# tabahi/WebSpeechAnalyzer

Measured on AMD Instinct MI355X. Metric: 53-feat frames/sec, higher is better.
Workload: dtype f32 front end / f64 tracker; 1 GPU; 1024 clips x 10 s @16 kHz mono per GPU, 1024-pt FFT, 25 ms hop, Segment Features (level 5); parallelism=1 GPU, batches_in_flight=6, streams=3

## Files before the change

webspeechanalyzer_amd/csrc/api.hip:

```cpp
#include <algorithm>
#include <cmath>
#include <cstdio>
#include <cstdlib>
#include <cstring>
#include <string>
#include <vector>
#include <map>
#include <mutex>
#include <system_error>
#include <thread>
#include "host_plan.hpp"

using namespace wsa;

thread_local std::string wsa_api::g_create_error;
using wsa_api::fail;

struct wsa_batch {
    wsa_ctx* ctx = nullptr;
    uint32_t n_clips = 0;
    double fs = 0;
    std::vector<uint32_t> n_samples, n_frames, frame_off;
    uint32_t total_frames = 0, max_frames = 0, max_samples = 0;
    DevArena mem;
    FeDev fe;
    Derived D;
    BackEnd be;
    int n_waves = 0;
    uint32_t *d_n_frames = nullptr, *d_frame_off = nullptr, *d_spec = nullptr;
    uint2* d_order = nullptr;
    uint2* d_redo = nullptr;
    char* d_pool = nullptr; double* d_span_hdr = nullptr; bool split = false; size_t pool_bpf = 0;
    hipStream_t up_stream[8] = {}; hipEvent_t up_event[8] = {}, up_start = nullptr; bool up_ready = false;
    int16_t* d_i16 = nullptr; uint64_t i16_cap = 0; uint64_t* d_i16_off = nullptr; uint32_t *d_i16_ch = nullptr, *d_i16_ns = nullptr;
    std::vector<uint64_t> h_i16_off; std::vector<uint32_t> h_i16_ch;
    bool pair = false;
    bool published = false;
    Tuning tune;
    uint32_t* d_span_hist = nullptr; uint2* d_span_key = nullptr;
    float* d_pcm_own = nullptr;
    bool rs_on = false; double fs_in = 0; std::vector<uint32_t> n_samples_in; uint32_t max_samples_in = 0;
    uint32_t *d_rs_n_in = nullptr, *d_rs_n_out = nullptr; float *d_rs_table = nullptr, *d_rs_pcm = nullptr; uint64_t rs_stride = 0;
    bool rs_mixed = false; RsMixedPlan rs_plan; RsClass* d_rs_cls = nullptr; uint32_t* d_rs_clip_class = nullptr; RsWork* d_rs_work = nullptr;
    bool counters_clean = false, end_clears = false, capturing = false, ever_captured = false;
    TrackGather trk;
    std::vector<int32_t> h_trk_seg; std::vector<uint32_t> h_seg_count;
    uint32_t res_utt = 0;
    double* d_trace = nullptr;
    uint32_t* h_totals = nullptr;
    uint32_t* h_totals_dev = nullptr;
    hipEvent_t ev[5] = {nullptr, nullptr, nullptr, nullptr, nullptr};
    bool timing = true, ran = false, full_table = false;
    uint32_t reruns = 0;
    uint32_t res_rows = 0, res_segs = 0, res_flags = 0;
    const uint32_t* spec_in_use = nullptr;
    wsa_cls* cls = nullptr;
    wsa_ecls* ecls = nullptr;
    int cls_last = 0;
};

namespace wsa {
Tuning Tuning::from_env() {
    Tuning t;
    { const char* on = std::getenv("WSA_TUNING_ENV"); if (!on || on[0] != '1') return t; }
    auto num = [](const char* name, int dflt) { const char* e = std::getenv(name); return e && *e ? std::atoi(e) : dflt; };
    t.dbg = num("WSA_DBG", 0);
    t.no_pair = std::getenv("WSA_NO_PAIR") != nullptr; t.no_split = std::getenv("WSA_NO_SPLIT") != nullptr; t.no_quad = std::getenv("WSA_NO_QUAD") != nullptr; t.quad = std::getenv("WSA_QUAD") != nullptr; t.no_fuse = std::getenv("WSA_NO_FUSE") != nullptr;
    t.fe_fat = std::getenv("WSA_FE_FAT") != nullptr; t.peaks_lanes = std::getenv("WSA_PEAKS_LANES") != nullptr;
    t.full_table = num("WSA_FULL_TABLE", -1);
    t.tracker_wpc = num("WSA_TRACKER_WPC", 0); t.fin_wpc = num("WSA_FIN_WPC", 0); t.fpw = num("WSA_FPW", 0);
    t.fe_wg_per_cu = num("WSA_FE_WGS", 0); t.fe_no_queue = std::getenv("WSA_FE_NO_QUEUE") != nullptr; t.peaks_wpc = num("WSA_PEAKS_WPC", 0); t.peaks_w = num("WSA_PEAKS_W", 0); t.upload_threads = num("WSA_UPLOAD_THREADS", 0);
    t.rs_s = num("WSA_RS_S", 0); t.rs_j = num("WSA_RS_J", 0); t.rs_c = num("WSA_RS_C", 0); t.rs_one_launch = std::getenv("WSA_RS_ONE_LAUNCH") != nullptr;
    return t;
}
__global__ void pcm_i16_to_f32_kernel(const int16_t* in, const uint64_t* off, const uint32_t* ch, const uint32_t* ns, float* out, uint64_t stride) {
    const uint32_t c = blockIdx.y;
    const uint32_t n = ns[c], k = ch[c];
    const int16_t* src = in + off[c];
    float* dst = out + (uint64_t)c * stride;
    for (uint32_t i = blockIdx.x * blockDim.x + threadIdx.x; i < n; i += gridDim.x * blockDim.x) dst[i] = (float)src[(uint64_t)i * k] * (1.0f / 32768.0f);
}
__global__ void batch_publish_kernel(const uint32_t* totals, const uint32_t* counters, uint32_t* host) {
    if (threadIdx.x == 0) {
        host[0] = totals[0]; host[1] = totals[1]; host[2] = counters[1]; host[3] = totals[3];
        __threadfence_system();
    }
}
__global__ void batch_clear_kernel(uint32_t* counters, uint32_t* totals, uint32_t* span_hist) {
    if (threadIdx.x < 16) counters[threadIdx.x] = 0;
    if (threadIdx.x < 4) totals[threadIdx.x] = 0;
    if (span_hist) for (int b = threadIdx.x; b < SPAN_BUCKETS; b += blockDim.x) span_hist[b] = 0;
}
}

extern "C" {

int wsa_abi_version(void) { return WSA_ABI_VERSION; }

void wsa_config_default(wsa_config* c) {
    c->spec_type = 1; c->output_level = 4; c->f_min = 50; c->f_max = 4000; c->N_fft_bins = 256; c->N_mel_bins = 128;
    c->window_width = 25; c->window_step = 25; c->pause_length = 200; c->min_seg_length = 50; c->auto_noise_gate = 1;
    c->voiced_max_dB = 100; c->voiced_min_dB = 10; c->pre_norm_gain = 1000; c->high_f_emph = 0;
}

const char* wsa_last_error(const wsa_ctx* ctx) { return ctx ? ctx->err.c_str() : wsa_api::g_create_error.c_str(); }

wsa_status wsa_create(const wsa_config* cfg, int32_t device, wsa_ctx** out) {
    if (!cfg || !out) return fail(nullptr, WSA_ERR_INVALID, "null argument");
    *out = nullptr;
    int n = 0;
    if (hipGetDeviceCount(&n) != hipSuccess || n <= 0) return fail(nullptr, WSA_ERR_NO_DEVICE, "no HIP device visible (libwsa has no CPU path)");
    if (device < 0 || device >= n) return fail(nullptr, WSA_ERR_INVALID, "device ordinal out of range");
    hipDeviceProp_t prop;
    if (hipGetDeviceProperties(&prop, device) != hipSuccess) return fail(nullptr, WSA_ERR_NO_DEVICE, "hipGetDeviceProperties failed");
    if (std::strncmp(prop.gcnArchName, "gfx950", 6) != 0)
        return fail(nullptr, WSA_ERR_NO_DEVICE, std::string("libwsa is built for gfx950 only; device is ") + prop.gcnArchName);
    const int lv = cfg->output_level;
    if (!(lv == 1 || lv == 2 || lv == 3 || lv == 4 || lv == 5 || lv == 10 || lv == 11 || lv == 12 || lv == 13))
        return fail(nullptr, WSA_ERR_INVALID, "output_level must be 1, 2 (spectrum frames only), 3, 4, 5, 10, 11, 12 or 13");
    if (!(cfg->window_step > 0) || !(cfg->window_width > 0)) return fail(nullptr, WSA_ERR_INVALID, "window_width / window_step must be positive");
    wsa_ctx* c = new wsa_ctx();
    c->cfg = *cfg; c->device = device; c->n_cu = prop.multiProcessorCount;
    *out = c;
    return WSA_OK;
}

void wsa_destroy(wsa_ctx* ctx) { delete ctx; }

wsa_status wsa_geometry_for(const wsa_ctx* ctx, double fs, wsa_geometry* out) {
    if (!ctx || !out) return WSA_ERR_INVALID;
    FePlanHost p; std::string err;
    if (!build_fe_plan(ctx->cfg, fs, p, err)) return fail(const_cast<wsa_ctx*>(ctx), WSA_ERR_INVALID, err);
    out->nfft = p.nfft; out->win = p.win; out->hop = p.hop; out->bands = p.bands; out->kmax = p.kmax;
    return WSA_OK;
}

wsa_status wsa_bins_hz(const wsa_ctx* ctx, double fs, double* out, int32_t n) {
    if (!ctx || !out) return WSA_ERR_INVALID;
    FePlanHost p; std::string err;
    if (!build_fe_plan(ctx->cfg, fs, p, err)) return fail(const_cast<wsa_ctx*>(ctx), WSA_ERR_INVALID, err);
    if (n < p.bands) return fail(const_cast<wsa_ctx*>(ctx), WSA_ERR_INVALID, "bins_hz buffer too small");
    for (int i = 0; i < p.bands; i++) out[i] = p.bins_hz[i];
    return WSA_OK;
}

void wsa_batch_destroy(wsa_batch* b) {
    if (!b) return;
    (void)hipSetDevice(b->ctx->device);
    if (b->d_i16) (void)hipFree(b->d_i16);
    for (auto& st : b->up_stream) if (st) (void)hipStreamDestroy(st);
    for (auto& e : b->up_event) if (e) (void)hipEventDestroy(e);
    if (b->up_start) (void)hipEventDestroy(b->up_start);
    for (auto& e : b->ev) if (e) (void)hipEventDestroy(e);
    wsa_cls_free(b->cls);
    wsa_ecls_free(b->ecls);
    delete b;
}

static wsa_status batch_create_impl(wsa_ctx* ctx, uint32_t n_clips, const uint32_t* n_samples, double fs, const uint32_t* n_samples_in, double fs_in, wsa_batch** out, const double* fs_in_each = nullptr) {
    if (!ctx || !out || (n_clips && !n_samples)) return fail(ctx, WSA_ERR_INVALID, "null argument");
    *out = nullptr;
    HIP_TRY(ctx, hipSetDevice(ctx->device));
    wsa_batch* b = new wsa_batch();
    b->ctx = ctx; b->n_clips = n_clips; b->fs = fs;
    b->tune = Tuning::from_env();
    std::string err;
    const FeDev::Refusal refused = b->fe.build(ctx->cfg, fs, b->tune.fe_fat, err);
    if (refused == FeDev::BAD_FFT) err = "unsupported FFT length: NFFT = the smallest of {2^k, 3 * 2^k} >= max(window, fs * N_fft_bins / f_max) must lie in 256 .. 8192 or be 3 * 2^k up to 12288";
    if (refused == FeDev::LDS) err += ": shorten the window or lower f_max / N_fft_bins";
    if (refused != FeDev::OK) { delete b; return fail(ctx, WSA_ERR_INVALID, err); }
    const FePlanHost& P = b->fe.plan;
    b->n_samples.assign(n_samples, n_samples + n_clips);
    b->n_frames.resize(n_clips); b->frame_off.resize(n_clips + 1);
    uint64_t tot = 0;
    for (uint32_t i = 0; i < n_clips; i++) {
        const uint32_t ns = n_samples[i];
        const uint32_t nf = ns < (uint32_t)P.win ? 0u : (ns - (uint32_t)P.win) / (uint32_t)P.hop + 1u;
        b->n_frames[i] = nf; b->frame_off[i] = (uint32_t)tot; tot += nf;
        if (nf > b->max_frames) b->max_frames = nf;
        if (ns > b->max_samples) b->max_samples = ns;
    }
    if (tot * CAND_CAP > 0xfffffff0ull) { delete b; return fail(ctx, WSA_ERR_INVALID, "batch has too many frames"); }
    b->frame_off[n_clips] = (uint32_t)tot; b->total_frames = (uint32_t)tot;

    const Derived& D = b->D = Derived(ctx->cfg, P.bands);
    BackEnd& B = b->be;
    B.n = n_clips;
    B.set_caps(D, P.bands, b->max_frames);
    B.seg_cap = (int)b->max_frames / D.period + 2;
    B.row_cap = D.syllable_rows ? (int)b->max_frames / 2 + 2 : B.seg_cap;
    b->pair = !D.raw_tracks && P.bands <= 128 && !b->tune.no_pair;
    b->pool_bpf = tracker_pool_bpf();
    b->split = b->pair && !b->tune.no_split && (size_t)b->total_frames * b->pool_bpf <= ((size_t)48 << 30);
    const size_t budget = (size_t)(b->pair ? 16 : 8) << 30;
    size_t waves = budget / ((b->be.ws_stride ? b->be.ws_stride : 1) * (b->pair ? 2 : 1));
    size_t wpc = 16;
    if (b->tune.tracker_wpc >= 1 && b->tune.tracker_wpc <= 32) wpc = (size_t)b->tune.tracker_wpc;
    const size_t want = (size_t)ctx->n_cu * wpc;
    if (waves > want) waves = want;
    if (waves > (size_t)n_clips * (size_t)b->be.seg_cap) waves = (size_t)n_clips * (size_t)b->be.seg_cap;
    if (b->pair && waves > ((size_t)n_clips * (size_t)b->be.seg_cap + 1) / 2 && n_clips * (size_t)b->be.seg_cap > 256) waves = ((size_t)n_clips * (size_t)b->be.seg_cap + 1) / 2;
    if (waves < 1) waves = 1;
    b->n_waves = (int)waves;

    DevArena& A = b->mem;
    const size_t spans = (size_t)n_clips * B.seg_cap;
    bool ok = b->fe.upload(A) && A.upload(&b->d_n_frames, b->n_frames) && A.upload(&b->d_frame_off, b->frame_off) && A.alloc(&b->d_spec, (size_t)b->total_frames * P.bands);
    if (ok && D.level > 2 && b->split) {
        size_t free_b = 0, total_b = 0;
        const size_t pool_bytes = (size_t)b->total_frames * b->pool_bpf;
        const bool room = hipMemGetInfo(&free_b, &total_b) != hipSuccess || free_b > pool_bytes + ((size_t)2 << 30);
        if (!(room && A.alloc(&b->d_pool, pool_bytes) && A.alloc(&b->d_span_hdr, spans * 8))) {
            (void)hipGetLastError();
            b->split = false; b->d_pool = nullptr; b->d_span_hdr = nullptr;
        }
    }
    ok = ok && B.alloc(A, D, b->total_frames, false) && A.alloc(&B.d_counters, 16);
    if (D.level > 2)
        ok = ok && A.alloc(&B.d_ws, B.ws_stride * (size_t)b->n_waves * (b->pair && !b->split ? 2 : 1)) && A.alloc(&b->d_redo, spans) && A.alloc(&b->d_order, spans)
                && A.alloc(&b->d_span_hist, (size_t)SPAN_BUCKETS) && A.alloc(&b->d_span_key, spans)
                && (!D.raw_tracks || (A.alloc(&B.d_trk_pts, ((size_t)b->total_frames + 1) * 64 * 2) && A.alloc(&B.d_trk_rank, ((size_t)b->total_frames + 1) * 64)))
                && (D.level != 12 || A.alloc(&B.d_coef_ws, (size_t)b->total_frames * 8));
    ok = ok && A.pin(&b->h_totals, &b->h_totals_dev, 8);
    for (auto& e : b->ev) if (ok) ok = hipEventCreate(&e) == hipSuccess;
    if (b->tune.full_table >= 0) b->full_table = b->tune.full_table != 0;
    if (ok && n_samples_in) {
        b->rs_on = true; b->fs_in = fs_in; b->n_samples_in.assign(n_samples_in, n_samples_in + n_clips);
        for (uint32_t i = 0; i < n_clips; i++) if (n_samples_in[i] > b->max_samples_in) b->max_samples_in = n_samples_in[i];
        b->rs_stride = ((uint64_t)b->max_samples + 3u) & ~3ull;
        ok = A.upload(&b->d_rs_n_in, b->n_samples_in) && A.upload(&b->d_rs_n_out, b->n_samples) && b->mem.alloc(&b->d_rs_pcm, (size_t)n_clips * b->rs_stride + 4);
        if (ok && fs_in_each) {
            b->rs_mixed = true;
            if (!plan_resample_mixed(n_clips, b->n_samples.data(), fs_in_each, fs, b->rs_plan, err)) { wsa_batch_destroy(b); return fail(ctx, WSA_ERR_INVALID, err); }
            RsMixedPlan& M = b->rs_plan;
            ok = A.upload(&b->d_rs_table, M.tables) && A.upload(&b->d_rs_cls, M.cls) && A.upload(&b->d_rs_clip_class, M.clip_class) && A.upload(&b->d_rs_work, M.work);
            std::vector<float>().swap(M.tables); std::vector<RsWork>().swap(M.work);
        } else if (ok) {
            std::vector<float> K0, K; build_resample_table(fs_in, fs, K0); resample_table_image(K0, K);
            ok = A.upload(&b->d_rs_table, K);
        }
    }
    if (!ok) {
        const std::string m = std::string("device allocation failed: ") + hipGetErrorString(hipGetLastError());
        wsa_batch_destroy(b);
        return fail(ctx, WSA_ERR_HIP, m);
    }
    *out = b;
    return WSA_OK;
}

wsa_status wsa_batch_create(wsa_ctx* ctx, uint32_t n_clips, const uint32_t* n_samples, double fs, wsa_batch** out) {
    return batch_create_impl(ctx, n_clips, n_samples, fs, nullptr, 0, out);
}

uint64_t wsa_resample_length(uint64_t n_in, double fs_in, double fs_out) { return fs_in > 0 && fs_out > 0 ? resample_length(n_in, fs_in, fs_out) : 0; }

wsa_status wsa_batch_create_resampled(wsa_ctx* ctx, uint32_t n_clips, const uint32_t* n_samples_in, double fs_in, double fs_out, wsa_batch** out) {
    if (!ctx || !out || (n_clips && !n_samples_in)) return fail(ctx, WSA_ERR_INVALID, "null argument");
    if (const wsa_status st = check_rates(ctx, &fs_in, 1, fs_out, nullptr); st != WSA_OK) return st;
    std::vector<uint32_t> n_out(n_clips);
    for (uint32_t i = 0; i < n_clips; i++) {
        const uint64_t n = resample_length(n_samples_in[i], fs_in, fs_out);
        if (n > 0xfffffff0ull) return fail(ctx, WSA_ERR_INVALID, "a converted clip would exceed 2^32 samples");
        n_out[i] = (uint32_t)n;
    }
    return batch_create_impl(ctx, n_clips, n_out.data(), fs_out, n_samples_in, fs_in, out);
}

wsa_status wsa_batch_create_mixed(wsa_ctx* ctx, uint32_t n_clips, const uint32_t* n_samples_in, const double* fs_in, double fs_out, wsa_batch** out) {
    if (!ctx || !out || (n_clips && (!n_samples_in || !fs_in))) return fail(ctx, WSA_ERR_INVALID, n_clips && ctx && out && !fs_in ? "null argument: fs_in holds one rate per clip (clip 0 has none)" : "null argument");
    if (const wsa_status st = check_rates(ctx, fs_in, n_clips, fs_out, "clip"); st != WSA_OK) return st;
    std::vector<uint32_t> n_out(n_clips);
    for (uint32_t i = 0; i < n_clips; i++) {
        const uint64_t n = resample_length(n_samples_in[i], fs_in[i], fs_out);
        if (n > 0xfffffff0ull) return fail(ctx, WSA_ERR_INVALID, "a converted clip would exceed 2^32 samples (clip " + std::to_string(i) + ")");
        n_out[i] = (uint32_t)n;
    }
    return batch_create_impl(ctx, n_clips, n_out.data(), fs_out, n_samples_in, 0, out, fs_in);
}

wsa_status wsa_batch_get_info(const wsa_batch* b, wsa_batch_info* o) {
    if (!b || !o) return WSA_ERR_INVALID;
    o->n_clips = b->n_clips; o->n_frames_total = b->total_frames; o->max_frames_per_clip = b->max_frames; o->bands = (uint32_t)b->fe.plan.bands;
    o->rows_cap = b->n_clips * (uint32_t)b->be.row_cap; o->segments_cap = b->n_clips * (uint32_t)b->be.seg_cap; o->workspace_bytes = b->mem.dev_bytes;
    return WSA_OK;
}

static wsa_status run_backend_stages(wsa_batch* b, const uint32_t* d_spec, bool skip_peaks, hipStream_t s) {
    wsa_ctx* ctx = b->ctx;
    const Derived& D = b->D;
    const BackEnd& B = b->be;
    b->published = false;
    if (D.level <= 2) return WSA_OK;
    const int dbg = b->tune.dbg;
    {
        hipStream_t cs = s;
        uint32_t* counters = B.d_counters + 4;
        PkParams pk; pk.spec = d_spec; pk.rec = B.rec; pk.total_frames = b->total_frames; pk.bands = b->fe.plan.bands;
        pk.flags = B.d_counters + 1; pk.dbg = (b->tune.dbg >> 20) & 0xff; pk.lanes_only = b->tune.peaks_lanes ? 1 : 0;
        pk.wpc = b->tune.peaks_wpc; pk.round_bins = b->tune.peaks_w;
        if (!skip_peaks) launch_peaks(pk, cs);
        GateParams g;
        B.fill(g, D);
        g.n_frames = b->d_n_frames; g.frame_off = b->d_frame_off; g.trace = b->d_trace; g.dbg = dbg; g.prio = 1;
        const bool ordered = !(dbg & 8192);
        g.span_hist = ordered ? b->d_span_hist : nullptr; g.span_key = b->d_span_key;
        launch_gate(g, cs);
        TrParams t;
        B.fill(t, D);
        t.frame_off = b->d_frame_off; t.trace = b->d_trace; t.dbg = dbg;
        t.order = ordered ? b->d_order : nullptr; t.redo = b->d_redo; t.redo_count = counters + 2;
        t.fin_waves = b->tune.fin_wpc >= 1 && b->tune.fin_wpc <= 32 ? ctx->n_cu * b->tune.fin_wpc : 0;
        t.quad = b->split && !b->tune.no_quad && (b->tune.quad || b->total_frames >= 1200000u) ? 1 : 0;
        t.quad_waves = (int)std::min<size_t>((size_t)b->n_waves, ((size_t)b->n_clips * (size_t)B.seg_cap + 3) / 4 + 1);
        t.pool = b->split ? b->d_pool : nullptr; t.pool_bpf = (uint32_t)b->pool_bpf; t.span_hdr = b->split ? b->d_span_hdr : nullptr;
        if (t.order) launch_span_order(t, b->d_span_hist, b->d_span_key, b->d_order, counters, cs);
        if (b->timing) HIP_TRY(ctx, hipEventRecord(b->ev[2], s));
        launch_tracker(t, b->n_waves, b->full_table, b->pair, cs);
    }
    if (b->timing) HIP_TRY(ctx, hipEventRecord(b->ev[3], s));
    CompactParams cp;
    B.fill(cp, D);
    cp.clip_rows = B.d_clip_rows; cp.flags = B.d_counters + 1; cp.fused = b->tune.no_fuse ? 0 : 1;
    cp.host = D.tail_kernel ? nullptr : b->h_totals_dev;
    b->published = compact_is_fused(cp) && cp.host != nullptr;
    const bool self_clear = b->published && !b->capturing;
    cp.clr_counters = self_clear ? B.d_counters : nullptr; cp.clr_hist = self_clear ? b->d_span_hist : nullptr;
    b->end_clears = self_clear;
    launch_compact(cp, s);
    if (D.level == 11) {
        UttParams u;
        B.fill(u, b->d_frame_off);
        launch_utterance(u, s);
    }
    if (D.level == 12) {
        CoefParams q;
        B.fill(q, b->d_frame_off);
        q.total_frames = b->total_frames;
        launch_coeffs(q, b->n_clips * (uint32_t)B.row_cap, s);
    }
    HIP_TRY(ctx, hipGetLastError());
    return WSA_OK;
}

static wsa_status run_impl(wsa_batch* b, const float* d_pcm, uint64_t stride, const uint32_t* d_spec_in, bool fe, bool be, hipStream_t s) {
    wsa_ctx* ctx = b->ctx;
    HIP_TRY(ctx, hipSetDevice(ctx->device));
    {
        hipStreamCaptureStatus cap = hipStreamCaptureStatusNone;
        if (s && hipStreamIsCapturing(s, &cap) != hipSuccess) { (void)hipGetLastError(); cap = hipStreamCaptureStatusNone; }
        b->capturing = cap != hipStreamCaptureStatusNone;
        if (b->capturing) b->ever_captured = true;
    }
    if (!b->counters_clean || b->ever_captured) hipLaunchKernelGGL(batch_clear_kernel, dim3(1), dim3(256), 0, s, b->be.d_counters, b->be.d_totals, b->d_span_hist);
    b->counters_clean = false; b->end_clears = false;
    if (b->timing) HIP_TRY(ctx, hipEventRecord(b->ev[0], s));
    const uint32_t* spec = d_spec_in ? d_spec_in : b->d_spec;
    if (fe) {
        if (!d_pcm && b->total_frames) return fail(ctx, WSA_ERR_INVALID, "null PCM pointer");
        if (stride < (b->rs_on ? b->max_samples_in : b->max_samples) && b->n_clips > 1) return fail(ctx, WSA_ERR_INVALID, "clip_stride smaller than the longest clip");
        if (b->rs_mixed) {
            RsMixedParams r; r.in = d_pcm; r.stride_in = stride; r.out = b->d_rs_pcm; r.stride_out = b->rs_stride; r.n_in = b->d_rs_n_in; r.n_out = b->d_rs_n_out;
            r.tables = b->d_rs_table; r.cls = b->d_rs_cls; r.clip_class = b->d_rs_clip_class; r.work = b->d_rs_work;
            launch_resample_mixed(r, b->rs_plan, !b->tune.rs_one_launch, s);
            HIP_TRY(ctx, hipGetLastError());
            d_pcm = b->d_rs_pcm; stride = b->rs_stride;
        } else if (b->rs_on) {
            RsParams r; r.in = d_pcm; r.stride_in = stride; r.out = b->d_rs_pcm; r.stride_out = b->rs_stride;
            r.n_in = b->d_rs_n_in; r.n_out = b->d_rs_n_out; r.table = b->d_rs_table; r.ratio = b->fs_in / b->fs; r.S = b->tune.rs_s > 0 ? b->tune.rs_s : resample_stride(b->fs_in, b->fs);
            r.J = b->tune.rs_j > 0 ? b->tune.rs_j : resample_outputs_per_lane(r.S, r.ratio); r.span = resample_span(r.ratio, r.S, r.J); r.chunks = b->tune.rs_c > 0 ? b->tune.rs_c : 1;
            launch_resample(r, b->n_clips, b->max_samples, s);
            HIP_TRY(ctx, hipGetLastError());
            d_pcm = b->d_rs_pcm; stride = b->rs_stride;
        }
        FeParams p;
        b->fe.fill(p, b->tune.fe_fat);
        p.pcm = d_pcm; p.clip_stride = stride; p.n_frames = b->d_n_frames; p.frame_off = b->d_frame_off; p.spec = b->d_spec;
        p.frames_per_wave = b->tune.fpw > 0 ? b->tune.fpw : 25; p.wg_per_cu = b->tune.fe_wg_per_cu;
        p.queue = b->tune.fe_no_queue ? nullptr : b->be.d_counters + 8; p.n_cu = b->ctx->n_cu;
        launch_frontend(p, (int)b->n_clips, (int)b->max_frames, b->fe.plan.R, b->fe.plan.three, s);
        HIP_TRY(ctx, hipGetLastError());
    }
    if (b->timing) HIP_TRY(ctx, hipEventRecord(b->ev[1], s));
    if (be) {
        const wsa_status st = run_backend_stages(b, spec, false, s);
        if (st != WSA_OK) return st;
    } else if (b->timing) { HIP_TRY(ctx, hipEventRecord(b->ev[2], s)); HIP_TRY(ctx, hipEventRecord(b->ev[3], s)); }
    if (!(be && b->published)) hipLaunchKernelGGL(batch_publish_kernel, dim3(1), dim3(64), 0, s, b->be.d_totals, b->be.d_counters, b->h_totals_dev);
    if (b->timing) HIP_TRY(ctx, hipEventRecord(b->ev[4], s));
    b->ran = true; b->spec_in_use = spec;
    b->counters_clean = be && b->end_clears && !b->capturing;
    return WSA_OK;
}

int wsa_debug_batch_counters(wsa_batch* b, uint32_t* out16) {
    if (!b || !out16) return WSA_ERR_INVALID;
    return hipMemcpy(out16, b->be.d_counters, 16 * sizeof(uint32_t), hipMemcpyDeviceToHost) == hipSuccess ? WSA_OK : WSA_ERR_HIP;
}

wsa_status wsa_batch_run(wsa_batch* b, const float* d_pcm, uint64_t clip_stride, void* stream) {
    if (!b) return WSA_ERR_INVALID;
    return run_impl(b, d_pcm, clip_stride, nullptr, true, true, reinterpret_cast<hipStream_t>(stream));
}
wsa_status wsa_batch_run_frontend(wsa_batch* b, const float* d_pcm, uint64_t clip_stride, void* stream) {
    if (!b) return WSA_ERR_INVALID;
    return run_impl(b, d_pcm, clip_stride, nullptr, true, false, reinterpret_cast<hipStream_t>(stream));
}
wsa_status wsa_batch_run_backend(wsa_batch* b, const uint32_t* d_spectra, void* stream) {
    if (!b || !d_spectra) return WSA_ERR_INVALID;
    return run_impl(b, nullptr, 0, d_spectra, false, true, reinterpret_cast<hipStream_t>(stream));
}

}
static std::mutex g_slab_mu;
static std::map<uintptr_t, size_t> g_slabs;
static bool slab_of(const void* p, uintptr_t* base, size_t* size) {
    std::lock_guard<std::mutex> lk(g_slab_mu);
    auto it = g_slabs.upper_bound(reinterpret_cast<uintptr_t>(p));
    if (it == g_slabs.begin()) return false;
    --it;
    if (reinterpret_cast<uintptr_t>(p) >= it->first + it->second) return false;
    *base = it->first; *size = it->second;
    return true;
}
template <typename DST, typename SRC, typename LEN>
static wsa_status upload_clips(wsa_batch* b, uint32_t n, DST dst, SRC src, LEN bytes, hipStream_t s) {
    wsa_ctx* ctx = b->ctx;
    uint64_t total = 0;
    for (uint32_t i = 0; i < n; i++) total += bytes(i);
    constexpr int UP_MAX = 8;
    int UP_THREADS = 3;
    if (b->tune.upload_threads >= 1 && b->tune.upload_threads <= UP_MAX) UP_THREADS = b->tune.upload_threads;
    {
        bool pinned = n > 0;
        std::vector<uintptr_t> slab_end(n, 0);
        for (uint32_t i = 0; i < n && pinned; i++) {
            if (!bytes(i)) continue;
            uintptr_t base = 0; size_t size = 0;
            if (slab_of(src(i), &base, &size)) { slab_end[i] = base + size; continue; }
            hipPointerAttribute_t at;
            if (hipPointerGetAttributes(&at, src(i)) != hipSuccess) { (void)hipGetLastError(); pinned = false; }
            else pinned = at.type == hipMemoryTypeHost;
        }
        if (pinned) {
            uint32_t i = 0;
            while (i < n) {
                const char* s0 = reinterpret_cast<const char*>(src(i)); char* d0 = reinterpret_cast<char*>(dst(i));
                size_t len = bytes(i); uint32_t j = i + 1;
                while (slab_end[i] && j < n && reinterpret_cast<const char*>(src(j)) == s0 + len && reinterpret_cast<char*>(dst(j)) == d0 + len
                       && reinterpret_cast<uintptr_t>(s0) + len + bytes(j) <= slab_end[i]) { len += bytes(j); j++; }
                if (len) HIP_TRY(ctx, hipMemcpyAsync(d0, s0, len, hipMemcpyHostToDevice, s));
                i = j;
            }
            return WSA_OK;
        }
    }
    if (n < 16 || total < ((uint64_t)32 << 20) || UP_THREADS == 1) {
        for (uint32_t i = 0; i < n; i++) if (bytes(i)) HIP_TRY(ctx, hipMemcpyAsync(dst(i), src(i), bytes(i), hipMemcpyHostToDevice, s));
        return WSA_OK;
    }
    if (!b->up_ready) {
        for (int t = 0; t < UP_MAX; t++) { HIP_TRY(ctx, hipStreamCreateWithFlags(&b->up_stream[t], hipStreamNonBlocking)); HIP_TRY(ctx, hipEventCreateWithFlags(&b->up_event[t], hipEventDisableTiming)); }
        HIP_TRY(ctx, hipEventCreateWithFlags(&b->up_start, hipEventDisableTiming));
        b->up_ready = true;
    }
    HIP_TRY(ctx, hipEventRecord(b->up_start, s));
    hipError_t err[UP_MAX];
    std::thread th[UP_MAX];
    uint32_t first_[UP_MAX + 1]; first_[0] = 0;
    { uint64_t acc = 0; int t = 1; for (uint32_t i = 0; i < n && t < UP_THREADS; i++) { acc += bytes(i); if (acc >= total * t / UP_THREADS) first_[t++] = i + 1; } while (t <= UP_THREADS) first_[t++] = n; }
    first_[UP_THREADS] = n;
    int started = 0;
    for (int t = 0; t < UP_THREADS; t++) {
        err[t] = hipSuccess;
        try {
        th[t] = std::thread([&, t]() {
            hipError_t e = hipSetDevice(ctx->device);
            if (e == hipSuccess) e = hipStreamWaitEvent(b->up_stream[t], b->up_start, 0);
            for (uint32_t i = first_[t]; i < first_[t + 1] && e == hipSuccess; i++) if (bytes(i)) e = hipMemcpyAsync(dst(i), src(i), bytes(i), hipMemcpyHostToDevice, b->up_stream[t]);
            if (e == hipSuccess) e = hipEventRecord(b->up_event[t], b->up_stream[t]);
            err[t] = e;
        });
        } catch (const std::system_error&) { break; }
        started++;
    }
    for (int t = 0; t < started; t++) th[t].join();
    hipError_t first = hipSuccess;
    for (int t = started; t < UP_THREADS && first == hipSuccess; t++)
        for (uint32_t i = first_[t]; i < first_[t + 1] && first == hipSuccess; i++) if (bytes(i)) first = hipMemcpyAsync(dst(i), src(i), bytes(i), hipMemcpyHostToDevice, s);
    for (int t = 0; t < started; t++) {
        if (err[t] != hipSuccess) { if (first == hipSuccess) first = err[t]; (void)hipStreamSynchronize(b->up_stream[t]); }
        else { const hipError_t e = hipStreamWaitEvent(s, b->up_event[t], 0); if (e != hipSuccess && first == hipSuccess) first = e; }
    }
    HIP_TRY(ctx, first);
    return WSA_OK;
}

extern "C" {
wsa_status wsa_batch_run_host(wsa_batch* b, const float* const* pcm, void* stream) {
    if (!b || (!pcm && b->n_clips)) return WSA_ERR_INVALID;
    wsa_ctx* ctx = b->ctx;
    hipStream_t s = reinterpret_cast<hipStream_t>(stream);
    HIP_TRY(ctx, hipSetDevice(ctx->device));
    const std::vector<uint32_t>& ns_host = b->rs_on ? b->n_samples_in : b->n_samples;
    const uint64_t stride = ((b->rs_on ? b->max_samples_in : b->max_samples) + 3u) & ~3ull;
    if (!b->d_pcm_own && !b->mem.alloc(&b->d_pcm_own, (size_t)b->n_clips * stride)) return fail(ctx, WSA_ERR_HIP, "PCM staging allocation failed");
    {
        const wsa_status st = upload_clips(b, b->n_clips, [&](uint32_t i) { return b->d_pcm_own + (size_t)i * stride; }, [&](uint32_t i) { return pcm[i]; },
                                           [&](uint32_t i) { return (size_t)ns_host[i] * sizeof(float); }, s);
        if (st != WSA_OK) return st;
    }
    return run_impl(b, b->d_pcm_own, stride, nullptr, true, true, s);
}

wsa_status wsa_batch_run_host_i16(wsa_batch* b, const int16_t* const* pcm, const uint32_t* channels, void* stream) {
    if (!b || (!pcm && b->n_clips)) return WSA_ERR_INVALID;
    wsa_ctx* ctx = b->ctx;
    hipStream_t s = reinterpret_cast<hipStream_t>(stream);
    HIP_TRY(ctx, hipSetDevice(ctx->device));
    const std::vector<uint32_t>& ns_host = b->rs_on ? b->n_samples_in : b->n_samples;
    const uint64_t stride = ((b->rs_on ? b->max_samples_in : b->max_samples) + 3u) & ~3ull;
    if (!b->d_pcm_own && !b->mem.alloc(&b->d_pcm_own, (size_t)b->n_clips * stride)) return fail(ctx, WSA_ERR_HIP, "PCM staging allocation failed");
    std::vector<uint64_t> off(b->n_clips + 1, 0); std::vector<uint32_t> ch(b->n_clips ? b->n_clips : 1, 1u);
    for (uint32_t i = 0; i < b->n_clips; i++) {
        ch[i] = channels ? channels[i] : 1u;
        if (ch[i] < 1 || ch[i] > 64) return fail(ctx, WSA_ERR_INVALID, "channels must be 1 .. 64");
        off[i + 1] = off[i] + (((uint64_t)ns_host[i] * ch[i] + 3u) & ~3ull);
    }
    if (off[b->n_clips] > b->i16_cap) {
        if (b->d_i16) { (void)hipFree(b->d_i16); b->d_i16 = nullptr; b->i16_cap = 0; }
        HIP_TRY(ctx, hipMalloc(reinterpret_cast<void**>(&b->d_i16), (size_t)off[b->n_clips] * sizeof(int16_t) + 16));
        b->i16_cap = off[b->n_clips];
    }
    if (!b->d_i16_off) {
        if (!b->mem.alloc(&b->d_i16_off, (size_t)b->n_clips + 1) || !b->mem.alloc(&b->d_i16_ch, (size_t)b->n_clips + 1) || !b->mem.alloc(&b->d_i16_ns, (size_t)b->n_clips + 1))
            return fail(ctx, WSA_ERR_HIP, "int16 staging allocation failed");
    }
    b->h_i16_off = off; b->h_i16_ch = ch;
    HIP_TRY(ctx, hipMemcpyAsync(b->d_i16_off, b->h_i16_off.data(), ((size_t)b->n_clips + 1) * sizeof(uint64_t), hipMemcpyHostToDevice, s));
    HIP_TRY(ctx, hipMemcpyAsync(b->d_i16_ch, b->h_i16_ch.data(), (size_t)(b->n_clips ? b->n_clips : 1) * sizeof(uint32_t), hipMemcpyHostToDevice, s));
    HIP_TRY(ctx, hipMemcpyAsync(b->d_i16_ns, ns_host.data(), (size_t)b->n_clips * sizeof(uint32_t), hipMemcpyHostToDevice, s));
    {
        const wsa_status st = upload_clips(b, b->n_clips, [&](uint32_t i) { return b->d_i16 + off[i]; }, [&](uint32_t i) { return pcm[i]; },
                                           [&](uint32_t i) { return (size_t)ns_host[i] * ch[i] * sizeof(int16_t); }, s);
        if (st != WSA_OK) return st;
    }
    if (b->n_clips) {
        const uint32_t mx = b->rs_on ? b->max_samples_in : b->max_samples;
        hipLaunchKernelGGL(pcm_i16_to_f32_kernel, dim3((mx + 1023) / 1024 ? (mx + 1023) / 1024 : 1, b->n_clips), dim3(256), 0, s, b->d_i16, b->d_i16_off, b->d_i16_ch, b->d_i16_ns, b->d_pcm_own, stride);
        HIP_TRY(ctx, hipGetLastError());
    }
    return run_impl(b, b->d_pcm_own, stride, nullptr, true, true, s);
}

static wsa_status fetch_totals(wsa_batch* b, hipStream_t s) {
    wsa_ctx* ctx = b->ctx;
    if (!b->ran) return fail(ctx, WSA_ERR_INVALID, "no run on this batch yet");
    {
        HIP_TRY(ctx, hipSetDevice(ctx->device));
        HIP_TRY(ctx, hipStreamSynchronize(s));
        const volatile uint32_t* ht = b->h_totals;
        b->res_rows = ht[0]; b->res_segs = ht[1]; b->res_flags = ht[2]; b->res_utt = ht[3];
        if (b->res_flags & 2u) {
            b->full_table = true; b->reruns++;
            hipLaunchKernelGGL(batch_clear_kernel, dim3(1), dim3(256), 0, s, b->be.d_counters, b->be.d_totals, b->d_span_hist);
            const bool tm = b->timing; b->timing = false;
            const wsa_status st = run_backend_stages(b, b->spec_in_use, true, s);
            b->timing = tm;
            if (st != WSA_OK) return st;
            if (!b->published) hipLaunchKernelGGL(batch_publish_kernel, dim3(1), dim3(64), 0, s, b->be.d_totals, b->be.d_counters, b->h_totals_dev);
            HIP_TRY(ctx, hipStreamSynchronize(s));
            b->res_rows = ht[0]; b->res_segs = ht[1]; b->res_flags = ht[2]; b->res_utt = ht[3];
        }
    }
    if (b->res_flags & 1u) return fail(ctx, WSA_ERR_CAPACITY, "a device-side arena overflowed; results are invalid");
    return WSA_OK;
}

wsa_status wsa_host_alloc(wsa_ctx* ctx, uint64_t bytes, void** out) {
    if (!ctx || !out) return WSA_ERR_INVALID;
    *out = nullptr;
    HIP_TRY(ctx, hipSetDevice(ctx->device));
    HIP_TRY(ctx, hipHostMalloc(out, bytes ? (size_t)bytes : 1, hipHostMallocPortable));
    { std::lock_guard<std::mutex> lk(g_slab_mu); g_slabs[reinterpret_cast<uintptr_t>(*out)] = bytes ? (size_t)bytes : 1; }
    return WSA_OK;
}
void wsa_host_free(void* p) {
    if (!p) return;
    { std::lock_guard<std::mutex> lk(g_slab_mu); g_slabs.erase(reinterpret_cast<uintptr_t>(p)); }
    (void)hipHostFree(p);
}

wsa_status wsa_queue_create(wsa_ctx* ctx, void** stream) {
    if (!ctx || !stream) return WSA_ERR_INVALID;
    *stream = nullptr;
    HIP_TRY(ctx, hipSetDevice(ctx->device));
    hipStream_t s = nullptr;
    HIP_TRY(ctx, hipStreamCreateWithFlags(&s, hipStreamNonBlocking));
    *stream = s;
    return WSA_OK;
}
wsa_status wsa_queue_synchronize(wsa_ctx* ctx, void* stream) {
    if (!ctx) return WSA_ERR_INVALID;
    HIP_TRY(ctx, hipSetDevice(ctx->device));
    HIP_TRY(ctx, hipStreamSynchronize(reinterpret_cast<hipStream_t>(stream)));
    return WSA_OK;
}
void wsa_queue_destroy(wsa_ctx* ctx, void* stream) {
    if (!stream) return;
    if (ctx) (void)hipSetDevice(ctx->device);
    (void)hipStreamDestroy(reinterpret_cast<hipStream_t>(stream));
}

void wsa_batch_view_internal(wsa_batch* b, wsa_batch_view* v) {
    v->ctx = b->ctx; v->level = b->ctx->cfg.output_level; v->n_clips = b->n_clips; v->rows_cap = b->n_clips * (uint32_t)b->be.row_cap;
    v->d_meta = b->be.d_meta; v->d_feat = b->be.d_feat; v->d_row_off = b->be.d_row_off; v->reruns = b->reruns; v->cls = &b->cls; v->ecls = &b->ecls; v->cls_last = &b->cls_last;
}
wsa_status wsa_batch_fetch_internal(wsa_batch* b, hipStream_t s) { return fetch_totals(b, s); }

wsa_ctx* wsa_batch_ctx_internal(const wsa_batch* b) { return b ? b->ctx : nullptr; }

wsa_status wsa_batch_result(wsa_batch* b, void* stream, wsa_device_result* o) {
    if (!b || !o) return WSA_ERR_INVALID;
    const wsa_status st = fetch_totals(b, reinterpret_cast<hipStream_t>(stream));
    o->n_clips = b->n_clips; o->n_rows = b->res_rows; o->n_segments = b->res_segs; o->n_frames_total = b->total_frames;
    o->status_flags = b->res_flags;
    o->d_row_meta = b->be.d_meta; o->d_row_feat = b->be.d_feat; o->d_segments = b->be.d_seg; o->d_clip_row_off = b->be.d_row_off; o->d_clip_seg_off = b->be.d_seg_off;
    o->d_spectra = b->spec_in_use; o->d_clip_frame_off = b->d_frame_off; o->d_formants = b->be.d_formants;
    o->n_utterance_rows = b->be.d_utt_feat ? b->res_utt : 0; o->d_utt_meta = b->be.d_utt_meta; o->d_utt_feat = b->be.d_utt_feat; o->d_clip_utt_off = b->be.d_utt_off;
    return st;
}

wsa_status wsa_batch_copy_rows(wsa_batch* b, void* stream, int32_t* row_meta, double* row_feat, uint32_t rows_cap,
                               int32_t* segments, uint32_t seg_cap, uint32_t* clip_row_off, uint32_t* clip_seg_off) {
    if (!b) return WSA_ERR_INVALID;
    wsa_ctx* ctx = b->ctx;
    hipStream_t s = reinterpret_cast<hipStream_t>(stream);
    const wsa_status st = fetch_totals(b, s);
    if (st != WSA_OK) return st;
    if ((row_meta || row_feat) && rows_cap < b->res_rows) return fail(ctx, WSA_ERR_INVALID, "row buffer too small");
    if (segments && seg_cap < b->res_segs) return fail(ctx, WSA_ERR_INVALID, "segment buffer too small");
    if (row_meta && b->res_rows) HIP_TRY(ctx, hipMemcpyAsync(row_meta, b->be.d_meta, (size_t)b->res_rows * 8 * sizeof(int32_t), hipMemcpyDefault, s));
    if (row_feat && b->res_rows) HIP_TRY(ctx, hipMemcpyAsync(row_feat, b->be.d_feat, (size_t)b->res_rows * WSA_NFEAT * sizeof(double), hipMemcpyDefault, s));
    if (segments && b->res_segs) HIP_TRY(ctx, hipMemcpyAsync(segments, b->be.d_seg, (size_t)b->res_segs * 4 * sizeof(int32_t), hipMemcpyDefault, s));
    if (clip_row_off) HIP_TRY(ctx, hipMemcpyAsync(clip_row_off, b->be.d_row_off, ((size_t)b->n_clips + 1) * sizeof(uint32_t), hipMemcpyDefault, s));
    if (clip_seg_off) HIP_TRY(ctx, hipMemcpyAsync(clip_seg_off, b->be.d_seg_off, ((size_t)b->n_clips + 1) * sizeof(uint32_t), hipMemcpyDefault, s));
    HIP_TRY(ctx, hipStreamSynchronize(s));
    return WSA_OK;
}

wsa_status wsa_batch_copy_spectra(wsa_batch* b, void* stream, uint32_t* spectra, uint64_t cap_words, uint32_t* clip_frame_off) {
    if (!b) return WSA_ERR_INVALID;
    wsa_ctx* ctx = b->ctx;
    hipStream_t s = reinterpret_cast<hipStream_t>(stream);
    if (!b->ran) return fail(ctx, WSA_ERR_INVALID, "no run on this batch yet");
    if (spectra && !b->spec_in_use) return fail(ctx, WSA_ERR_INVALID, "the u32 frames of this run were not stored: call wsa_batch_keep_spectra(batch, 1) before the run");
    const uint64_t words = (uint64_t)b->total_frames * (uint32_t)b->fe.plan.bands;
    if (spectra && cap_words < words) return fail(ctx, WSA_ERR_INVALID, "spectra buffer too small");
    HIP_TRY(ctx, hipSetDevice(ctx->device));
    if (spectra && words) HIP_TRY(ctx, hipMemcpyAsync(spectra, b->spec_in_use, words * sizeof(uint32_t), hipMemcpyDefault, s));
    if (clip_frame_off) std::memcpy(clip_frame_off, b->frame_off.data(), ((size_t)b->n_clips + 1) * sizeof(uint32_t));
    HIP_TRY(ctx, hipStreamSynchronize(s));
    return WSA_OK;
}

wsa_status wsa_batch_copy_utterance(wsa_batch* b, void* stream, int32_t* utt_meta, double* utt_feat, uint32_t cap_rows, uint32_t* clip_utt_off) {
    if (!b) return WSA_ERR_INVALID;
    wsa_ctx* ctx = b->ctx;
    hipStream_t s = reinterpret_cast<hipStream_t>(stream);
    if (!b->be.d_utt_feat) return fail(ctx, WSA_ERR_INVALID, "no utterance features: output_level must be 11");
    const wsa_status st = fetch_totals(b, s);
    if (st != WSA_OK) return st;
    if ((utt_meta || utt_feat) && cap_rows < b->res_utt) return fail(ctx, WSA_ERR_INVALID, "utterance buffer too small");
    if (utt_meta && b->res_utt) HIP_TRY(ctx, hipMemcpyAsync(utt_meta, b->be.d_utt_meta, (size_t)b->res_utt * 4 * sizeof(int32_t), hipMemcpyDefault, s));
    if (utt_feat && b->res_utt) HIP_TRY(ctx, hipMemcpyAsync(utt_feat, b->be.d_utt_feat, (size_t)b->res_utt * WSA_NUTT * sizeof(double), hipMemcpyDefault, s));
    if (clip_utt_off) HIP_TRY(ctx, hipMemcpyAsync(clip_utt_off, b->be.d_utt_off, ((size_t)b->n_clips + 1) * sizeof(uint32_t), hipMemcpyDefault, s));
    HIP_TRY(ctx, hipStreamSynchronize(s));
    return WSA_OK;
}

wsa_status wsa_batch_copy_formants(wsa_batch* b, void* stream, float* formants, uint64_t cap_frames) {
    if (!b || !formants) return WSA_ERR_INVALID;
    wsa_ctx* ctx = b->ctx;
    hipStream_t s = reinterpret_cast<hipStream_t>(stream);
    if (!b->ran || !b->be.d_formants) return fail(ctx, WSA_ERR_INVALID, "no formant frames: output_level must be 4, 10, 11 or 12 and the batch must have run");
    if (cap_frames < b->total_frames) return fail(ctx, WSA_ERR_INVALID, "formant buffer too small");
    HIP_TRY(ctx, hipSetDevice(ctx->device));
    if (b->total_frames) HIP_TRY(ctx, hipMemcpyAsync(formants, b->be.d_formants, (size_t)b->total_frames * 9 * sizeof(float), hipMemcpyDefault, s));
    HIP_TRY(ctx, hipStreamSynchronize(s));
    return WSA_OK;
}


static wsa_status fetch_track_tables(wsa_batch* b, hipStream_t s) {
    wsa_ctx* ctx = b->ctx;
    if (!b->be.d_trk_seg) return fail(ctx, WSA_ERR_INVALID, "no raw tracks: output_level must be 3");
    const wsa_status st = fetch_totals(b, s);
    if (st != WSA_OK) return st;
    b->h_trk_seg.resize((size_t)b->n_clips * b->be.seg_cap * 4); b->h_seg_count.resize(b->n_clips);
    if (b->n_clips) {
        HIP_TRY(ctx, hipMemcpyAsync(b->h_trk_seg.data(), b->be.d_trk_seg, b->h_trk_seg.size() * sizeof(int32_t), hipMemcpyDefault, s));
        HIP_TRY(ctx, hipMemcpyAsync(b->h_seg_count.data(), b->be.d_seg_count, b->h_seg_count.size() * sizeof(uint32_t), hipMemcpyDefault, s));
        HIP_TRY(ctx, hipStreamSynchronize(s));
    }
    return WSA_OK;
}

static void batch_track_list(wsa_batch* b) {
    b->trk.begin();
    for (uint32_t c = 0; c < b->n_clips; c++)
        for (uint32_t k = 0; k < b->h_seg_count[c]; k++) b->trk.add(&b->h_trk_seg[((size_t)c * b->be.seg_cap + k) * 4], 0);
}

wsa_status wsa_batch_tracks_info(wsa_batch* b, void* stream, wsa_tracks_info* out) {
    if (!b || !out) return WSA_ERR_INVALID;
    const wsa_status st = fetch_track_tables(b, reinterpret_cast<hipStream_t>(stream));
    if (st != WSA_OK) return st;
    batch_track_list(b);
    out->n_segments = b->trk.segments(); out->n_points = b->trk.n_points; out->n_ranked = b->trk.n_ranked;
    return WSA_OK;
}

wsa_status wsa_batch_copy_tracks(wsa_batch* b, void* stream, uint64_t* seg_off, int32_t* points, uint64_t cap_points, int32_t* ranked, uint64_t cap_ranked) {
    if (!b || !seg_off || !points || !ranked) return WSA_ERR_INVALID;
    wsa_ctx* ctx = b->ctx;
    hipStream_t s = reinterpret_cast<hipStream_t>(stream);
    const wsa_status st = fetch_track_tables(b, s);
    if (st != WSA_OK) return st;
    TrackGather& G = b->trk;
    batch_track_list(b);
    if (G.n_points > cap_points || G.n_ranked > cap_ranked) return fail(ctx, WSA_ERR_INVALID, "track buffers too small");
    G.offsets(seg_off);
    if (const wsa_status gs = G.run(ctx, 1ull << 63, b->be.d_trk_pts, b->be.d_trk_rank, points, ranked, s); gs != WSA_OK) return gs;
    HIP_TRY(ctx, hipStreamSynchronize(s));
    return WSA_OK;
}

wsa_status wsa_batch_copy_pcm(wsa_batch* b, void* stream, float* pcm, uint64_t stride) {
    if (!b || !pcm) return WSA_ERR_INVALID;
    wsa_ctx* ctx = b->ctx;
    hipStream_t s = reinterpret_cast<hipStream_t>(stream);
    if (!b->rs_on || !b->ran) return fail(ctx, WSA_ERR_INVALID, "no converted PCM: the batch must come from wsa_batch_create_resampled / wsa_batch_create_mixed and must have run");
    if (stride < b->max_samples) return fail(ctx, WSA_ERR_INVALID, "stride smaller than the longest converted clip");
    HIP_TRY(ctx, hipSetDevice(ctx->device));
    for (uint32_t i = 0; i < b->n_clips; i++)
        if (b->n_samples[i]) HIP_TRY(ctx, hipMemcpyAsync(pcm + (size_t)i * stride, b->d_rs_pcm + (size_t)i * b->rs_stride, (size_t)b->n_samples[i] * sizeof(float), hipMemcpyDefault, s));
    HIP_TRY(ctx, hipStreamSynchronize(s));
    return WSA_OK;
}

wsa_status wsa_batch_stage_ms(wsa_batch* b, float out[4]) {
    if (!b || !out) return WSA_ERR_INVALID;
    wsa_ctx* ctx = b->ctx;
    if (!b->ran || !b->timing) return fail(ctx, WSA_ERR_INVALID, "no timed run on this batch");
    HIP_TRY(ctx, hipEventSynchronize(b->ev[4]));
    for (int i = 0; i < 4; i++) HIP_TRY(ctx, hipEventElapsedTime(&out[i], b->ev[i], b->ev[i + 1]));
    return WSA_OK;
}

wsa_status wsa_batch_enable_trace(wsa_batch* b, int32_t on) {
    if (!b) return WSA_ERR_INVALID;
    if (on && !b->d_trace) {
        HIP_TRY(b->ctx, hipSetDevice(b->ctx->device));
        const size_t rows = b->total_frames ? b->total_frames : 1;
        if (!b->mem.alloc(&b->d_trace, rows * 12)) return fail(b->ctx, WSA_ERR_HIP, "trace allocation failed");
        HIP_TRY(b->ctx, hipMemset(b->d_trace, 0, rows * 12 * sizeof(double)));
    }
    if (!on) b->d_trace = nullptr;
    return WSA_OK;
}

wsa_status wsa_batch_copy_trace(wsa_batch* b, void* stream, double* out, uint64_t cap_rows) {
    if (!b || !out) return WSA_ERR_INVALID;
    wsa_ctx* ctx = b->ctx;
    hipStream_t s = reinterpret_cast<hipStream_t>(stream);
    if (!b->d_trace || !b->ran) return fail(ctx, WSA_ERR_INVALID, "trace not enabled or no run yet");
    if (cap_rows < b->total_frames) return fail(ctx, WSA_ERR_INVALID, "trace buffer too small");
    if (b->total_frames) HIP_TRY(ctx, hipMemcpyAsync(out, b->d_trace, (size_t)b->total_frames * 12 * sizeof(double), hipMemcpyDefault, s));
    HIP_TRY(ctx, hipStreamSynchronize(s));
    return WSA_OK;
}

wsa_status wsa_batch_keep_spectra(wsa_batch* b, int32_t on) {
    if (!b) return WSA_ERR_INVALID;
    (void)on;
    return WSA_OK;
}

wsa_status wsa_batch_backend_reruns(const wsa_batch* b, uint32_t* out) {
    if (!b || !out) return WSA_ERR_INVALID;
    *out = b->reruns;
    return WSA_OK;
}

wsa_status wsa_batch_enable_timing(wsa_batch* b, int32_t on) {
    if (!b) return WSA_ERR_INVALID;
    b->timing = on != 0;
    return WSA_OK;
}

}
```

webspeechanalyzer_amd/csrc/gate.hip:

```cpp
#include "wsa_internal.hpp"
#include "wave_ops.hpp"
#include "jsmath_device.hpp"
#include "gate_floor.hpp"

#pragma clang diagnostic ignored "-Winline-asm"

namespace wsa {


template <bool ST>
__global__ __launch_bounds__(64) void gate_kernel_t(GateParams p) {
    const int lane = threadIdx.x;
    for (uint32_t clip = p.clip0 + blockIdx.x; clip < p.clip0 + p.n_clips; clip += gridDim.x) {
        const uint32_t nfr = p.n_frames[clip];
        const uint32_t foff = ST ? clip * p.ring : p.frame_off[clip];
        const uint32_t fmask = ST ? p.ring - 1 : 0xffffffffu;
        int32_t* seg_i = p.seg_i + (uint64_t)clip * p.seg_cap * 8;
        double* seg_d = p.seg_d + (uint64_t)clip * p.seg_cap * 2;

        int cur_frame = 0, no_fm = 0, c_ci = 0, c_started = -1;
        double ctx_max = p.ctx_max0, floor_ = p.floor0, last_max = p.ctx_max0, last_floor = p.floor0;
        double gw = 0, gT = 0, gk = 0;
        int nseg = 0, span_begin = 0, cuts = 0;
        bool overflow = false;
        double* st = ST ? p.state + (uint64_t)clip * GATE_STATE : nullptr;
        if (ST) {
            cur_frame = (int)st[0]; no_fm = (int)st[1]; c_ci = (int)st[2]; c_started = (int)st[3];
            ctx_max = st[4]; floor_ = st[5]; last_max = st[6]; last_floor = st[7]; gw = st[8]; gT = st[9]; gk = st[10];
            span_begin = (int)st[11]; cuts = (int)st[12];
        }
        const uint32_t fbase = (uint32_t)cur_frame;

        auto finalize = [&](int e_arg, int f_end) __attribute__((always_inline)) {
            const int len = e_arg - no_fm;
            if (!((double)len > p.min_frames && c_started >= 2)) return;
            if (nseg >= p.seg_cap) { overflow = true; return; }
            if (lane == 0) {
                int32_t* sg = seg_i + 8 * nseg;
                sg[SEG_START] = cur_frame - len; sg[SEG_LEN] = len; sg[SEG_FBEGIN] = span_begin; sg[SEG_FEND] = f_end;
                sg[SEG_CCI] = c_ci; sg[SEG_FLAG] = p.level == 3 ? 1 : 0; sg[SEG_NROWS] = 0; sg[SEG_ROW0] = 0;
                seg_d[2 * nseg] = ctx_max; seg_d[2 * nseg + 1] = floor_;
                if (!ST && p.span_hist) {
                    const uint32_t bkt = (uint32_t)(SPAN_BUCKETS - 1) - min((uint32_t)(f_end - span_begin), (uint32_t)(SPAN_BUCKETS - 1));
                    p.span_key[(uint64_t)clip * p.seg_cap + nseg] = make_uint2(bkt, atomicAdd(&p.span_hist[bkt], 1u));
                }
            }
            nseg++;
        };
        bool gate_reset = false;
        auto noise_gate = [&](double h) __attribute__((always_inline)) {
            gw++;
            if (h > ctx_max || (gw > 40 && h > 2 * floor_)) {
                if (h >= ctx_max) { gw = 0; last_max = ctx_max = h; }
                else if (h > last_max / 100) { ctx_max -= trunc(ctx_max / 8); gw = 35; }
                const double y = ctx_max, t = jsm::log10(y);
                double v;
                if (t > 7) v = trunc(jsm::pow_pos(10, t - 3) / 20);
                else if (t > 6) v = trunc(jsm::pow_pos(10, t - 3) / 2);
                else if (t > 4) v = trunc(jsm::pow_pos(10, t - 2) / 2);
                else if (t > 2) v = trunc(jsm::pow_pos(10, t / 3));
                else if (t > 1) v = trunc(y / 10);
                else v = 1;
                floor_ = v; last_floor = v;
                if (gk > 0 && gT / gk < 30 * v) { c_ci = 0; c_started = 0; no_fm = 0; gate_reset = true; gk = 0; gT = 0; }
                gT += ctx_max; gk += 1;
            } else if (floor_ > 10 && floor_ > last_floor / 10 && gw > 20) {
                floor_ -= trunc(last_floor / 20);
                if (floor_ < 10) floor_ = 10;
            }
        };

        constexpr int GF = 4;
        const uint32_t fend = fbase + nfr;
        auto load_hdr_blk = [&](uint32_t blk, uint4& h) __attribute__((always_inline)) {
            const uint32_t f = min(blk + (uint32_t)lane, fend - 1);
            h = p.rec.hdr[foff + (f & fmask)];
        };
        auto load_ent = [&](uint32_t f, int n, uint32_t cbase, uint32_t& w) __attribute__((always_inline)) {
            w = 0u;
            if (f < fend && lane < n) w = p.rec.amp[cbase + (uint32_t)lane];
        };
        uint4 hd = make_uint4(0u, 0u, 0u, 0u), hd2 = hd;
        uint32_t e_ent[GF], x_ent[GF];
        if (nfr > 0) {
            load_hdr_blk(fbase, hd);
#pragma unroll
            for (int k = 0; k < GF; k++) load_ent(fbase + k, (read_lane_i32((int)hd.y, k) >> 8) & 0xff, (uint32_t)read_lane_i32((int)hd.w, k), e_ent[k]);
        }
        for (uint32_t blk = fbase; blk < fend; blk += 64) {
          if (blk + 64 < fend) load_hdr_blk(blk + 64, hd2);
          int o_info = -1, o_span = 0; double o_v = 0, o_fl = 0;
          const int nblk = (int)min(64u, fend - blk);
          for (int j0 = 0; j0 < nblk; j0 += GF) {
#pragma unroll
            for (int k = 0; k < GF; k++) {
                const int jn = j0 + GF + k;
                const int ny = jn < 64 ? read_lane_i32((int)hd.y, jn & 63) : read_lane_i32((int)hd2.y, jn & 63);
                const uint32_t nb = (uint32_t)(jn < 64 ? read_lane_i32((int)hd.w, jn & 63) : read_lane_i32((int)hd2.w, jn & 63));
                load_ent(blk + (uint32_t)jn, (ny >> 8) & 0xff, nb, x_ent[k]);
            }
#pragma unroll
            for (int k = 0; k < GF; k++) {
            const int jf = j0 + k;
            if (jf >= nblk) break;
            const uint32_t f = blk + (uint32_t)jf;
            const int hnw = read_lane_i32((int)hd.y, jf);
            const int ncand = (hnw >> 8) & 0xff;
            const double g = (double)(hnw & 0xff) * 4294967296.0 + (double)(uint32_t)read_lane_i32((int)hd.x, jf);
            const uint32_t amp = e_ent[k];

            cur_frame++;
            const int t_idx = c_ci;
            const double v = floor_;
            const bool acc = lane < ncand && (double)amp > v;
            const int n = __popcll(__ballot(acc));
            const double d = wave_sum_int40(acc ? (uint64_t)amp : 0ull);
            const uint32_t mx = (uint32_t)read_lane_i32((int)hd.z, jf);
            double h = 2 * v; int pbin = 0;
            if (n > 0 && (double)mx > h) { h = mx; pbin = (hnw >> 16) & 0xff; }
            bool reset_before_acc = false;
            if (c_started < 0) {
                const bool r_gt4 = p.auto_gate ? (d > h && h * (n - 1) > 4 * (d - h)) : ((d > h ? h * (n - 1) / (d - h) : 0) > 4);
                if (n > 0 && pbin > 7 && pbin < p.max_voiced_bin && n > 4 && r_gt4) {
                    c_ci = 0; c_started = 0; no_fm = 0; reset_before_acc = true; span_begin = (int)f;
                } else no_fm++;
            }
            bool do_reset = false;
            int info = -1;
            if (c_started >= 0) {
                if (n == 0 || pbin < 7 || pbin >= p.max_voiced_bin || (n > 3 && g - d > 0 && 10 * d < g - d)) {
                    no_fm++;
                    if (c_started < 2) c_started--;
                    else if ((double)no_fm >= p.breaker) { finalize(c_ci + 1, (int)f + 1); do_reset = true; }
                    else if (p.auto_gate) { gate_reset = false; noise_gate(h); if (gate_reset) span_begin = (int)f + 1; }
                } else {
                    if (p.auto_gate) { gate_reset = false; noise_gate(h); if (gate_reset) { reset_before_acc = true; span_begin = (int)f; } }
                    info = t_idx | (reset_before_acc ? (1 << 30) : 0);
                    if (c_started < 2) c_started++; else no_fm = 0;
                }
            }
            if (lane == jf) { o_info = info; o_v = v; o_fl = floor_; o_span = span_begin; }
            if (lane == 0) {
                if (!ST && p.trace && !(p.dbg & 16)) {
                    double* tr = p.trace + ((uint64_t)foff + f) * 12;
                    tr[0] = c_ci; tr[1] = c_started; tr[2] = no_fm; tr[3] = ctx_max; tr[4] = floor_; tr[5] = n; tr[6] = pbin;
                    tr[7] = h; tr[8] = d; tr[9] = g; tr[10] = 0; tr[11] = 0;
                }
            }
            c_ci++;
            if (do_reset) { c_ci = 0; c_started = -1; no_fm = 0; span_begin = (int)f + 1; }
            if (ST && c_started >= 0 && f + 1 - (uint32_t)span_begin + p.step_frames > p.ring) {
                finalize(c_ci, (int)f + 1);
                c_ci = 0; c_started = 1; no_fm = 0; span_begin = (int)f + 1; cuts++;
            }
            }
#pragma unroll
            for (int k = 0; k < GF; k++) e_ent[k] = x_ent[k];
          }
          if (lane < nblk) {
              const uint32_t fi = foff + ((blk + (uint32_t)lane) & fmask);
              p.fr_info[fi] = o_info; p.fr_v[fi] = o_v; p.fr_fl[fi] = o_fl;
              if (ST && p.fr_span) p.fr_span[fi] = o_span;
          }
          hd = hd2;
        }
        if (!ST || (p.ctl[clip] & 2u)) {
            finalize(c_ci, (int)fend);
            c_ci = 0; c_started = 1; no_fm = 0; span_begin = (int)fend;
        }
        if (ST && lane == 0) {
            st[0] = cur_frame; st[1] = no_fm; st[2] = c_ci; st[3] = c_started; st[4] = ctx_max; st[5] = floor_; st[6] = last_max;
            st[7] = last_floor; st[8] = gw; st[9] = gT; st[10] = gk; st[11] = span_begin; st[12] = cuts;
        }
        if (lane == 0) {
            p.seg_count[clip] = (uint32_t)nseg; p.clip_rows[clip] = 0;
            if (nseg > 0) atomicMax(&p.counters[0], (uint32_t)nseg);
            if (overflow) atomicOr(&p.shared[1], 1u);
        }
    }
}

template <bool TRACE>
__global__ __launch_bounds__(64) void gate_kernel_auto(GateParams p) {
    constexpr int GS = 16;
    __shared__ uint32_t s_amp[64 * GS];
    static_assert(CAND_CAP == 64 && GS % 4 == 0, "one LDS row per frame, one lane per candidate");
    if (p.prio) __builtin_amdgcn_s_setprio(3);
    const int lane = threadIdx.x;
    const int br_i = p.breaker >= 2147483647.0 ? 2147483647 : (int)ceil(p.breaker);
    const int maxvb = p.max_voiced_bin;
    const bool want_trace = TRACE && p.trace && !(p.dbg & 16);
    const uint64_t lt_l = lanemask_lt(lane);
    for (uint32_t clip = p.clip0 + blockIdx.x; clip < p.clip0 + p.n_clips; clip += gridDim.x) {
        const uint32_t nfr = p.n_frames[clip];
        const uint32_t foff = p.frame_off[clip];
        int32_t* seg_i = p.seg_i + (uint64_t)clip * p.seg_cap * 8;
        double* seg_d = p.seg_d + (uint64_t)clip * p.seg_cap * 2;
        int no_fm = 0, c_ci = 0, c_started = -1, gw = 0;
        uint32_t ctx_max = (uint32_t)p.ctx_max0, floor_ = (uint32_t)p.floor0, last_max = ctx_max;
        uint32_t dec20 = floor_ / 20u, thr_b = max(10u, floor_ / 10u);
        uint64_t gT = 0; uint32_t gk = 0;
        int nseg = 0, span_begin = 0;
        bool overflow = false;

        auto finalize = [&](int e_arg, int f_end, int cur_frame) __attribute__((always_inline)) {
            const int len = e_arg - no_fm;
            if (!((double)len > p.min_frames && c_started >= 2)) return;
            if (nseg >= p.seg_cap) { overflow = true; return; }
            if (lane == 0) {
                int32_t* sg = seg_i + 8 * nseg;
                sg[SEG_START] = cur_frame - len; sg[SEG_LEN] = len; sg[SEG_FBEGIN] = span_begin; sg[SEG_FEND] = f_end;
                sg[SEG_CCI] = c_ci; sg[SEG_FLAG] = p.level == 3 ? 1 : 0; sg[SEG_NROWS] = 0; sg[SEG_ROW0] = 0;
                seg_d[2 * nseg] = (double)ctx_max; seg_d[2 * nseg + 1] = (double)floor_;
                if (p.span_hist) {
                    const uint32_t bkt = (uint32_t)(SPAN_BUCKETS - 1) - min((uint32_t)(f_end - span_begin), (uint32_t)(SPAN_BUCKETS - 1));
                    p.span_key[(uint64_t)clip * p.seg_cap + nseg] = make_uint2(bkt, atomicAdd(&p.span_hist[bkt], 1u));
                }
            }
            nseg++;
        };
        uint4 stg[GS / 4];
        auto stage_load = [&](uint32_t blk, const uint4& hdr_of_lane) __attribute__((always_inline)) {
            const int c0 = 4 * (lane & (GS / 4 - 1));
#pragma unroll
            for (int i = 0; i < GS / 4; i++) {
                const int row = (256 / GS) * i + (lane / (GS / 4));
                const int nc = (__builtin_amdgcn_ds_bpermute(row << 2, (int)hdr_of_lane.y) >> 8) & 0xff;
                uint4 w = make_uint4(0u, 0u, 0u, 0u);
                if (blk + (uint32_t)row < nfr && c0 < nc) w = *reinterpret_cast<const uint4*>(p.rec.amp + ((uint64_t)(foff + blk + (uint32_t)row)) * CAND_CAP + c0);
                if (c0 + 1 >= nc) w.y = 0u;
                if (c0 + 2 >= nc) w.z = 0u;
                if (c0 + 3 >= nc) w.w = 0u;
                stg[i] = w;
            }
        };
        auto stage_store = [&]() __attribute__((always_inline)) {
#pragma unroll
            for (int i = 0; i < GS / 4; i++) *reinterpret_cast<uint4*>(&s_amp[((256 / GS) * i + (lane / (GS / 4))) * GS + 4 * (lane & (GS / 4 - 1))]) = stg[i];
        };
        uint4 hd = make_uint4(0u, 0u, 0u, 0u), hd2 = hd;
        if (nfr > 0) {
            hd = p.rec.hdr[foff + min((uint32_t)lane, nfr - 1)];
            stage_load(0, hd);
            stage_store();
        }
        for (uint32_t blk = 0; blk < nfr; blk += 64) {
            wsync();
            if (blk + 64 < nfr) { hd2 = p.rec.hdr[foff + min(blk + 64 + (uint32_t)lane, nfr - 1)]; stage_load(blk + 64, hd2); }
            const int mxbin_l = (int)((hd.y >> 16) & 0xffu);
            const uint32_t flags_l = ((mxbin_l < 7 || mxbin_l >= maxvb) ? 1u : 0u)
                                   | (11ull * (uint64_t)hd.z < (((uint64_t)(hd.y & 0xffu) << 32) | hd.x) ? 2u : 0u)
                                   | ((mxbin_l > 7 && mxbin_l < maxvb) ? 4u : 0u);
            int o_info = -1; uint32_t o_fl = 0;
            const uint32_t floor_in = floor_;
            const int nblk = (int)min(64u, nfr - blk);
#pragma clang diagnostic push
#pragma clang diagnostic ignored "-Winline-asm"
            auto put = [&](int j_, int info_) __attribute__((always_inline)) {
                asm volatile("s_mov_b32 m0, %2\n\tv_writelane_b32 %0, %3, m0\n\tv_writelane_b32 %1, %4, m0" : "+v"(o_info), "+v"(o_fl) : "s"(j_), "s"(info_), "s"(floor_) : "m0");
            };
#pragma clang diagnostic pop
            auto amp_row = [&](int j_) __attribute__((always_inline)) -> uint32_t {
                uint32_t a = lane < GS ? s_amp[j_ * GS + lane] : 0u;
                const int nc = (read_lane_i32((int)hd.y, j_) >> 8) & 0xff;
                if (nc > GS) a = lane < nc ? p.rec.amp[((uint64_t)(foff + blk) + (uint32_t)j_) * CAND_CAP + (uint32_t)lane] : 0u;
                return a;
            };
            auto count_accepted = [&](int j_) __attribute__((always_inline)) -> int {
                return __popcll(__ballot(amp_row(j_) > floor_));
            };
            for (int j = 0; j < nblk; j++) {
                if (!TRACE) {
                    if (c_started >= 2) {
                        for (; j < nblk; j++) {
                            {
                                const int k = lane - j;
                                const int d0 = max(20 - gw, 0);
                                const uint32_t room = floor_ > thr_b ? floor_ - thr_b : 0u;
                                const int S = __popcll(__ballot((uint64_t)(uint32_t)lane * (uint64_t)dec20 < (uint64_t)room));
                                const uint32_t lo10 = S > 0 ? 10u : 0u;
                                const int sk = min(max(k - d0, 0), S), sk1 = min(max(k + 1 - d0, 0), S);
                                const uint32_t fk = max(floor_ - (uint32_t)sk * dec20, lo10), fk1 = max(floor_ - (uint32_t)sk1 * dec20, lo10);
                                const uint32_t mxl = hd.z, v2 = fk << 1;
                                const bool strong = mxl > v2, voiced = strong && !(flags_l & 1u);
                                const uint64_t run_m = ~0ull << j;
                                const uint64_t prev = __ballot(voiced) & run_m & lt_l;
                                const int nofm_b = prev ? lane - 64 + __clzll((long long)prev) : no_fm + k;
                                const bool ex = max(mxl, v2) > ctx_max
                                             || (strong && gw + k >= 40)
                                             || (voiced && (flags_l & 2u))
                                             || (!voiced && nofm_b >= br_i - 1);
                                const uint64_t exm = __ballot(ex) & run_m;
                                const int E = min(exm ? __ffsll((long long)exm) - 1 : 64, nblk);
                                if (E > j) {
                                    if (k >= 0 && lane < E) { o_info = voiced ? c_ci + k : -1; o_fl = fk1; }
                                    floor_ = (uint32_t)read_lane_i32((int)fk1, E - 1);
                                    no_fm = read_lane_i32(voiced ? 0 : nofm_b + 1, E - 1);
                                    c_ci += E - j; gw += E - j; j = E;
                                }
                                if (j >= nblk) break;
                            }
                            const uint32_t mx_ = (uint32_t)read_lane_i32((int)hd.z, j), fl_ = (uint32_t)read_lane_i32((int)flags_l, j);
                            const bool strong_ = mx_ > 2u * floor_;
                            const uint32_t h_ = max(mx_, 2u * floor_);
                            bool unv_;
                            if (strong_ && !(fl_ & 1u)) {
                                if ((fl_ & 2u) && count_accepted(j) > 3) break;
                                unv_ = false;
                            } else {
                                if (no_fm + 1 >= br_i) break;
                                unv_ = true;
                            }
                            if (h_ > ctx_max || (gw >= 40 && strong_)) {
                                uint32_t nctx = ctx_max, nlast = last_max; int ngw = gw + 1;
                                if (h_ >= ctx_max) { ngw = 0; nlast = nctx = h_; }
                                else if (100ull * (uint64_t)h_ > (uint64_t)last_max) { nctx -= nctx >> 3; ngw = 35; }
                                const uint32_t nv = (uint32_t)__builtin_amdgcn_readfirstlane((int)floor_law(nctx));
                                if (gk >= (1u << 20) || (gk > 0 && gT < 30ull * (uint64_t)nv * (uint64_t)gk)) break;
                                ctx_max = nctx; last_max = nlast; gw = ngw;
                                floor_ = nv; dec20 = nv / 20u; thr_b = max(10u, nv / 10u);
                                gT += nctx; gk += 1;
                            } else {
                                gw++;
                                if (gw > 20 && floor_ > thr_b) floor_ = max(floor_ - dec20, 10u);
                            }
                            put(j, unv_ ? -1 : c_ci);
                            no_fm = unv_ ? no_fm + 1 : 0;
                            c_ci++;
                        }
                    } else if (c_started < 0) {
                        for (; j < nblk; j++) {
                            {
                                const uint64_t exm = __ballot(hd.z > 2u * floor_ && (flags_l & 4u)) & (~0ull << j);
                                const int E = min(exm ? __ffsll((long long)exm) - 1 : 64, nblk);
                                if (E > j) {
                                    if (lane >= j && lane < E) { o_info = -1; o_fl = floor_; }
                                    no_fm += E - j; c_ci += E - j; j = E;
                                }
                                if (j >= nblk) break;
                            }
                            const uint32_t mx_ = (uint32_t)read_lane_i32((int)hd.z, j), fl_ = (uint32_t)read_lane_i32((int)flags_l, j);
                            if (mx_ > 2u * floor_ && (fl_ & 4u) && count_accepted(j) > 4) break;
                            put(j, -1);
                            no_fm++; c_ci++;
                        }
                    }
                    if (j >= nblk) break;
                }
                const uint32_t f = blk + (uint32_t)j;
                const uint32_t amp = amp_row(j);
                const uint32_t mx = (uint32_t)read_lane_i32((int)hd.z, j);
                const uint32_t v = floor_;
                const int n = __popcll(__ballot(amp > v));
                const bool strong = mx > 2u * v;
                const uint32_t h = strong ? mx : 2u * v;
                int info = -1;
                {
                    const uint32_t hx = (uint32_t)read_lane_i32((int)hd.x, j), hy = (uint32_t)read_lane_i32((int)hd.y, j);
                    const uint64_t g = ((uint64_t)(hy & 0xffu) << 32) | hx;
                    const int pbin = strong ? (int)((hy >> 16) & 0xffu) : 0;
                    const int t_idx = c_ci;
                    uint64_t d = 0; bool have_d = false;
                    auto exact_d = [&]() __attribute__((always_inline)) {
                        if (have_d) return;
                        const uint32_t a = amp > v ? amp : 0u;
                        d = ((uint64_t)wave_sum_u32(a >> 20) << 20) + (uint64_t)wave_sum_u32(a & 0xfffffu);
                        have_d = true;
                    };
                    if (want_trace) exact_d();
                    bool reset_before_acc = false;
                    if (c_started < 0) {
                        bool start = false;
                        if (n > 4 && pbin > 7 && pbin < maxvb) { exact_d(); start = d > (uint64_t)h && (uint64_t)h * (uint64_t)(n - 1) > 4ull * (d - (uint64_t)h); }
                        if (start) { c_ci = 0; c_started = 0; no_fm = 0; reset_before_acc = true; span_begin = (int)f; }
                        else no_fm++;
                    }
                    bool do_reset = false, gate_reset = false;
                    auto noise_gate = [&]() __attribute__((always_inline)) {
                        gw++;
                        if (h > ctx_max || (gw > 40 && h > 2u * floor_)) {
                            if (h >= ctx_max) { gw = 0; last_max = ctx_max = h; }
                            else if (100ull * (uint64_t)h > (uint64_t)last_max) { ctx_max -= ctx_max >> 3; gw = 35; }
                            const uint32_t nv = (uint32_t)__builtin_amdgcn_readfirstlane((int)floor_law(ctx_max));
                            floor_ = nv; dec20 = nv / 20u; thr_b = max(10u, nv / 10u);
                            const bool below = gk < (1u << 20) ? gT < 30ull * (uint64_t)nv * (uint64_t)gk : (double)gT / (double)gk < 30.0 * (double)nv;
                            if (gk > 0 && below) { c_ci = 0; c_started = 0; no_fm = 0; gate_reset = true; gk = 0; gT = 0; }
                            gT += ctx_max; gk += 1;
                        } else if (floor_ > thr_b && gw > 20) {
                            floor_ = max(floor_ - dec20, 10u);
                        }
                    };
                    if (c_started >= 0) {
                        bool unv = n == 0 || pbin < 7 || pbin >= maxvb;
                        if (!unv && n > 3 && 11ull * (uint64_t)mx < g) { exact_d(); unv = 11ull * d < g; }
                        if (unv) {
                            no_fm++;
                            if (c_started < 2) c_started--;
                            else if (no_fm >= br_i) { finalize(c_ci + 1, (int)f + 1, (int)f + 1); do_reset = true; }
                            else { noise_gate(); if (gate_reset) span_begin = (int)f + 1; }
                        } else {
                            noise_gate();
                            if (gate_reset) { reset_before_acc = true; span_begin = (int)f; }
                            info = t_idx | (reset_before_acc ? (1 << 30) : 0);
                            if (c_started < 2) c_started++; else no_fm = 0;
                        }
                    }
                    if (want_trace && lane == 0) {
                        double* tr = p.trace + ((uint64_t)foff + f) * 12;
                        tr[0] = c_ci; tr[1] = c_started; tr[2] = no_fm; tr[3] = (double)ctx_max; tr[4] = (double)floor_; tr[5] = n; tr[6] = pbin;
                        tr[7] = (double)h; tr[8] = (double)d; tr[9] = (double)g; tr[10] = 0; tr[11] = 0;
                    }
                    c_ci++;
                    if (do_reset) { c_ci = 0; c_started = -1; no_fm = 0; span_begin = (int)f + 1; }
                }
                put(j, info);
            }
            const uint32_t o_sh = (uint32_t)__builtin_amdgcn_ds_bpermute(((lane - 1) & 63) << 2, (int)o_fl);
            if (lane < nblk) {
                const uint32_t fi = foff + blk + (uint32_t)lane;
                const uint32_t o_v = lane == 0 ? floor_in : o_sh;
                p.fr_info[fi] = o_info; p.fr_v[fi] = (double)o_v; p.fr_fl[fi] = (double)o_fl;
            }
            wsync();
            if (blk + 64 < nfr) stage_store();
            hd = hd2;
        }
        finalize(c_ci, (int)nfr, (int)nfr);
        if (lane == 0) {
            p.seg_count[clip] = (uint32_t)nseg; p.clip_rows[clip] = 0;
            if (nseg > 0) atomicMax(&p.counters[0], (uint32_t)nseg);
            if (overflow) atomicOr(&p.shared[1], 1u);
        }
        wsync();
    }
}

__global__ void stream_prepare_kernel(double* state, int32_t* carry, int32_t* tr_state, const uint32_t* ctl, uint32_t n, double ctx_max0, double floor0) {
    const uint32_t s = blockIdx.x * blockDim.x + threadIdx.x;
    if (s >= n || !(ctl[s] & 1u)) return;
    double* st = state + (uint64_t)s * GATE_STATE;
    st[0] = 0; st[1] = 0; st[2] = 0; st[3] = -1; st[4] = ctx_max0; st[5] = floor0; st[6] = ctx_max0; st[7] = floor0;
    st[8] = 0; st[9] = 0; st[10] = 0; st[11] = 0; st[12] = 0;
    for (int i = 0; i < CARRY_WORDS; i++) carry[(uint64_t)s * CARRY_WORDS + i] = 0;
    if (tr_state) {
        int32_t* t = tr_state + (uint64_t)s * TR_STATE_WORDS;
        t[0] = 0; t[1] = 0; t[2] = 0; t[3] = -1; t[4] = 0; t[5] = -2; t[8] = 0; t[9] = 0; t[10] = 0; t[11] = 0;
    }
}

void launch_gate(const GateParams& p, hipStream_t s) {
    if (p.n_clips == 0) return;
    if (p.auto_gate && p.strided && !(p.dbg & 2048)) {
        if ((p.trace && !(p.dbg & 16)) || (p.dbg & 4096)) hipLaunchKernelGGL(gate_kernel_auto<true>, dim3(p.n_clips), dim3(64), 0, s, p);
        else hipLaunchKernelGGL(gate_kernel_auto<false>, dim3(p.n_clips), dim3(64), 0, s, p);
    }
    else hipLaunchKernelGGL(gate_kernel_t<false>, dim3(p.n_clips), dim3(64), 0, s, p);
}

void launch_stream_prepare(double* state, int32_t* carry, int32_t* tr_state, const uint32_t* ctl, uint32_t n, double ctx_max0, double floor0, hipStream_t s) {
    if (n == 0) return;
    hipLaunchKernelGGL(stream_prepare_kernel, dim3((n + 255) / 256), dim3(256), 0, s, state, carry, tr_state, ctl, n, ctx_max0, floor0);
}

void launch_gate_stream(const GateParams& p, hipStream_t s) {
    if (p.n_clips == 0) return;
    hipLaunchKernelGGL(gate_kernel_t<true>, dim3(p.n_clips), dim3(64), 0, s, p);
}

}
```

webspeechanalyzer_amd/csrc/tracker.hip:

```cpp
#include <type_traits>
#include "wsa_internal.hpp"
#include "jsmath_device.hpp"
#include "wave_ops.hpp"
#include "tracker_score.hpp"
#include "tracker_features.hpp"

#ifdef WSA_TUNING
#define WSA_TUNE(bits_) (p.dbg & (bits_))
#else
#define WSA_TUNE(bits_) false
#endif

namespace wsa {

constexpr int MAXC = 64;
constexpr int AC_MAX = 320;
constexpr int PAIR_AC = 64;
constexpr int PAIR_GSZ = 4384;
constexpr int QUAD_AC = 38;
constexpr int QUAD_GSZ = 2496;
constexpr int AC_FAST = 140;

struct Ws {
    int32_t *tr_len, *tr_slot, *tr_rank;
    double *tr_sumE, *tr_sumEbin;
    int4* pt;
    int4* ptx;
    int32_t* pt_key;
    int32_t *d_p0, *d_p1, *d_gen;
    float *fr, *sm1;
    double *dB, *Aev;
    int32_t *q_idx, *sorted; double* q_mb;
};

__host__ __device__ inline size_t align16(size_t x) { return (x + 15) & ~(size_t)15; }

__host__ __device__ __forceinline__ Ws carve_ws(char* base, int T, int P, int F, int PX, size_t* bytes) {
    Ws w;
    size_t o = 0;
#define WSA_CARVE(field, type, count) do { w.field = reinterpret_cast<type*>(base + o); \
        o = align16(o + sizeof(type) * (size_t)(count)); } while (0)
    WSA_CARVE(tr_len, int32_t, T); WSA_CARVE(tr_slot, int32_t, T); WSA_CARVE(tr_rank, int32_t, T);
    WSA_CARVE(tr_sumE, double, T); WSA_CARVE(tr_sumEbin, double, T);
    WSA_CARVE(pt, int4, P); WSA_CARVE(ptx, int4, PX); WSA_CARVE(pt_key, int32_t, P);
    WSA_CARVE(d_p0, int32_t, F + 2); WSA_CARVE(d_p1, int32_t, F + 2); WSA_CARVE(d_gen, int32_t, F + 2);
    WSA_CARVE(fr, float, (size_t)(F + 2) * 9); WSA_CARVE(sm1, float, F + 2);
    WSA_CARVE(dB, double, (size_t)3 * (F + 2)); WSA_CARVE(Aev, double, (size_t)3 * (F + 2));
    WSA_CARVE(q_idx, int32_t, T); WSA_CARVE(sorted, int32_t, T); WSA_CARVE(q_mb, double, T);
#undef WSA_CARVE
    if (bytes) *bytes = o;
    return w;
}

constexpr int GW_MAX = 32;
static_assert(GW_MAX <= MAXC, "a frame's new tracks / points (one per lane of its span's group) fit the MAXC per frame that tracker_pool_bpf gives a span region");
size_t tracker_pool_bpf() { size_t b = 0; (void)carve_ws(nullptr, MAXC, MAXC, 1, 0, &b); return align16(b) + 256; }
size_t tracker_ws_bytes(int tcap, int pcap, int fcap, bool raw_tracks) { size_t b = 0; (void)carve_ws(nullptr, tcap, pcap, fcap, raw_tracks ? pcap : 0, &b); return align16(b) + 256; }

template <int AC, bool RAW, bool ST, bool PAIR = false, int SPLIT = 0, int GW = 32>
__device__ __forceinline__ void tracker_body(const TrParams& p) {
    constexpr int SCRATCH = MAXC * (4 + 4 + 8 + 8) + 64 * 8 + MAXC * 8 + MAXC * 4;
    constexpr int LDS_ONE = AC * 52 + SCRATCH;
    constexpr int LDS_ALL = (PAIR && GW == 16 && 4 * QUAD_GSZ > LDS_ONE) ? 4 * QUAD_GSZ : LDS_ONE;
    __shared__ __attribute__((aligned(16))) unsigned char s_big[LDS_ALL];
    static_assert((AC * 52) % 16 == 0, "the scratch arrays start 16-byte aligned");
    double* const s_plo = reinterpret_cast<double*>(s_big + AC * 52);
    double* const s_phi = s_plo + MAXC;
    unsigned long long* const s_best = reinterpret_cast<unsigned long long*>(s_phi + MAXC);
    uint32_t* const s_pk = reinterpret_cast<uint32_t*>(s_best + MAXC);
    uint32_t* const s_amp = s_pk + MAXC;
    int32_t* const s_pr_j = reinterpret_cast<int32_t*>(s_amp + MAXC);
    int32_t* const s_pr_o = s_pr_j + 64;
    int32_t* const s_asg = s_pr_o + 64;
    double* const a_vel = reinterpret_cast<double*>(s_big);
    double* const a_sumE = a_vel + AC;
    double* const a_sumEbin = a_sumE + AC;
    unsigned long long* const a_mmask = reinterpret_cast<unsigned long long*>(a_sumEbin + AC);
    int32_t* const a_last_frame = reinterpret_cast<int32_t*>(a_mmask + AC);
    int32_t* const a_len = a_last_frame + AC;
    int32_t* const a_gid = a_len + AC;
    uint32_t* const a_bins = reinterpret_cast<uint32_t*>(a_gid + AC);
    uint32_t* const a_amp = a_bins + AC;
    constexpr int FRCAP = (AC * 52 - AC * 16) / 40;
    static_assert(FRCAP <= FEAT_LDS_MAX, "finalize_fast hands formant_features_lds every span that fits the block");
    double* const f_qmb = reinterpret_cast<double*>(s_big);
    int32_t* const f_qidx = reinterpret_cast<int32_t*>(f_qmb + AC);
    int32_t* const f_sorted = f_qidx + AC;
    float* const f_fr = reinterpret_cast<float*>(f_sorted + AC);
    float* const f_sm = f_fr + FRCAP * 9;

    const int lane = threadIdx.x;
    Ws W = carve_ws(SPLIT ? p.pool : p.ws + (uint64_t)blockIdx.x * (PAIR ? 2 : 1) * p.ws_stride, p.tcap, p.pcap, p.fcap, RAW ? p.pcap : 0, nullptr);
    int gen = 0;
    int vz; asm volatile("v_mov_b32 %0, 0" : "=v"(vz));
    int aev_stride = p.fcap + 2;
    if (!ST && !SPLIT) { for (int d = lane; d < p.fcap + 2; d += 64) W.d_gen[d] = 0; }
    if (PAIR && !SPLIT) { const Ws W1 = carve_ws(p.ws + ((uint64_t)blockIdx.x * 2 + 1) * p.ws_stride, p.tcap, p.pcap, p.fcap, 0, nullptr); for (int d = lane; d < p.fcap + 2; d += 64) W1.d_gen[d] = 0; }
    wsync();

    uint32_t item = (!ST && p.order) ? 0u : blockIdx.x;
    bool gen_once = false;
    for (;;) {
        uint32_t k_seg = 0, clip = 0;
        uint64_t pair_idx = 0; uint32_t pair_total = 0;
        if (ST) { if (gen_once) break; gen_once = true; clip = blockIdx.x; k_seg = 0; }
        else if (SPLIT == 2) {
            const uint32_t total = p.counters[p.order_cnt];
            const uint64_t idx = (uint64_t)item * gridDim.x + blockIdx.x;
            if (idx >= total) break;
            item++;
            const uint2 e = p.order[idx];
            clip = e.x; k_seg = e.y;
        }
        else if (PAIR) {
            pair_total = p.counters[p.order_cnt];
            const uint32_t npairs = (pair_total + (uint32_t)(64 / GW) - 1u) / (uint32_t)(64 / GW), W_ = gridDim.x, r = item;
            if ((uint64_t)r * W_ >= npairs) break;
            item++;
            pair_idx = (uint64_t)r * W_ + ((r & 1u) ? W_ - 1u - blockIdx.x : blockIdx.x);
            if (pair_idx >= npairs) continue;
        }
        else if (p.order) {
            const uint32_t total = p.counters[p.order_cnt], W_ = gridDim.x, r = item;
            if ((uint64_t)r * W_ >= total) break;
            item++;
            const uint64_t idx = (uint64_t)r * W_ + ((r & 1u) ? W_ - 1u - blockIdx.x : blockIdx.x);
            if (idx >= total) continue;
            const uint2 e = p.order[idx];
            clip = e.x; k_seg = e.y;
        } else {
            k_seg = item / p.n_clips; clip = item - k_seg * p.n_clips;
            if (k_seg >= p.counters[0]) break;
            item += gridDim.x;
            if (k_seg >= p.seg_count[clip]) continue;
        }
        int my_seg = (int)k_seg;
        int32_t* sg = p.seg_i + ((uint64_t)clip * p.seg_cap + my_seg) * 8;
        int start = 0, len = 0, c_ci = 0; uint32_t f_begin = 0, f_end = 0; double ctx_max = 0, floor_ = 0;
        if (!ST && !PAIR) {
            start = sg[SEG_START]; len = sg[SEG_LEN]; c_ci = sg[SEG_CCI];
            f_begin = (uint32_t)sg[SEG_FBEGIN]; f_end = (uint32_t)sg[SEG_FEND];
            ctx_max = p.seg_d[((uint64_t)clip * p.seg_cap + my_seg) * 2];
            floor_ = p.seg_d[((uint64_t)clip * p.seg_cap + my_seg) * 2 + 1];
        }
        uint32_t foff = p.frame_off[clip];

        const unsigned long long tk0 = (WSA_TUNE(16)) ? __builtin_readcyclecounter() : 0ull;
        unsigned long long tk1 = tk0;
        double accG = 0, accL = 0;
        auto acc_totals = [&](double& S, double& C) __attribute__((always_inline)) { C = wave_sum_f64(accL); S = accG - C; };
        int n_tr = 0, n_pt = 0, n_act = 0, stale_d = -1, stale_p1 = 0;
        bool overflow = false, act_overflow = false;
        if (!ST) gen++;

        unsigned long long ph[4] = {0, 0, 0, 0};
        unsigned long long acp[5] = {0, 0, 0, 0, 0}, act = 0;
#define WSA_ACP(k_) do { if (WSA_TUNE(512)) { const unsigned long long now_ = __builtin_readcyclecounter(); acp[k_] += now_ - act; act = now_; } } while (0)

        auto take_rows = [&](int n) __attribute__((always_inline)) -> long long {
            uint32_t r0 = 0;
            if (lane == 0) r0 = atomicAdd(&p.clip_rows[clip], (uint32_t)n);
            r0 = (uint32_t)read_lane_i32((int)r0, 0);
            if ((uint64_t)r0 + (uint32_t)n > p.row_cap) { overflow = true; return -1; }
            return (long long)clip * p.row_cap + r0;
        };

        constexpr int BIG = LDS_ALL;
        auto finalize_fast_impl = [&](auto GFR) __attribute__((always_inline)) -> bool {
            constexpr bool G = decltype(GFR)::value;
            const int off_u = (int)align16((size_t)2 * n_tr);
            const int rank_bytes = 16 * n_tr, fr_bytes = G ? 0 : (int)align16((size_t)40 * len);
            const int off_pt = off_u + fr_bytes;
            const bool pe_lds = !G && off_pt + 12 * n_pt <= BIG;
            const int ppb = pe_lds ? 12 : 4;
            if (n_tr > 8000 || n_pt > 60000 || off_u + rank_bytes > BIG || off_pt + ppb * n_pt > BIG || off_pt + FEAT_SCRATCH * 8 > BIG) return false;
            int16_t* const trk_key = reinterpret_cast<int16_t*>(s_big);
            double* const qmb = reinterpret_cast<double*>(s_big + off_u);
            int32_t* const qt = reinterpret_cast<int32_t*>(s_big + off_u + 8 * n_tr);
            int32_t* const srt = qt + n_tr;
            float* const fr = G ? W.fr : reinterpret_cast<float*>(s_big + off_u);
            float* const smv = G ? W.sm1 : fr + 9 * len;
            double* const pE = reinterpret_cast<double*>(s_big + off_pt);
            uint32_t* const pkb = reinterpret_cast<uint32_t*>(s_big + off_pt + (pe_lds ? 8 * n_pt : 0));
            auto energy_of = [&](int q) __attribute__((always_inline)) -> double { return pe_lds ? pE[q] : reinterpret_cast<const double*>(W.pt + q)[1]; };
            if (WSA_TUNE(16)) ph[0] = ph[1] = ph[2] = ph[3] = __builtin_readcyclecounter();
            int nq = 0;
            for (int base = 0; base < n_tr; base += 64) {
                const int t = base + lane;
                bool q = false; double mb = 0;
                if (t < n_tr) {
                    trk_key[t] = -1;
                    const int tl = W.tr_len[t]; const double sb = W.tr_sumEbin[t], se = W.tr_sumE[t];
                    if (tl >= 2) { mb = sb / se; q = mb >= 7; }
                }
                const uint64_t mask = __ballot(q);
                if (q) { const int pos = nq + __popcll(mask & lanemask_lt(lane)); qmb[pos] = mb; qt[pos] = t; }
                nq += __popcll(mask);
            }
            wsync();
            for (int base = 0; base < nq; base += 64) {
                const int qi = base + lane;
                if (qi < nq) {
                    const double mb = qmb[qi];
                    int rank = 0;
                    for (int u = 0; u < nq; u++) { const double o = qmb[u]; rank += (o < mb || (o == mb && u < qi)) ? 1 : 0; }
                    srt[rank] = qi;
                }
            }
            wsync();
            int n_part = 0;
            {
                double last = 0; int slot = 0; bool stopped = false;
                for (int base = 0; base < nq && !stopped; base += 64) {
                    const int r = base + lane;
                    double mb = 0; int t = 0;
                    if (r < nq) { const int qi = srt[r]; mb = qmb[qi]; t = qt[qi]; }
                    uint64_t todo = __ballot(r < nq);
                    int myslot = -1;
                    while (todo) {
                        const uint64_t jm = __ballot(((todo >> lane) & 1ull) && fabs(mb - last) > 20);
                        if (jm == 0ull) { if ((todo >> lane) & 1ull) myslot = slot; break; }
                        const int j = __ffsll((long long)jm) - 1;
                        if (((todo >> lane) & 1ull) && lane < j) myslot = slot;
                        last = __hiloint2double(__builtin_amdgcn_readlane(__double2hiint(mb), j), __builtin_amdgcn_readlane(__double2loint(mb), j));
                        slot++;
                        if (slot >= 3) { stopped = true; break; }
                        todo &= ~lanemask_lt(j);
                    }
                    if (myslot >= 0) trk_key[t] = (int16_t)((r << 2) | myslot);
                    n_part += __popcll(__ballot(myslot >= 0));
                }
            }
            wsync();
            const int off_tbl = (int)align16((size_t)off_pt + (size_t)ppb * (size_t)n_pt);
            const int tbl_bytes = 4 * (len + 1) + 2 * (len + 1) * n_part;
            const bool use_tbl = !G && n_part <= 32 && c_ci + 1 < 0x7fff && stale_d < 0x7fff && off_tbl + tbl_bytes <= BIG && !(p.dbg & 32768);
            uint32_t* const tblm = reinterpret_cast<uint32_t*>(s_big + off_tbl);
            uint16_t* const tbl = reinterpret_cast<uint16_t*>(tblm + len + 1);
            if (use_tbl) for (int q = lane; q <= len; q += 64) tblm[q] = 0u;
            wsync();
            bool bad = false;
            {
                int4 nxt4 = lane < n_pt ? W.pt[lane] : make_int4(0, 0, 0, 0);
                for (int q = lane; q < n_pt; q += 64) {
                    const int4 rec4 = nxt4;
                    if (q + 64 < n_pt) nxt4 = W.pt[q + 64];
                    const int key = trk_key[rec4.x];
                    if (pe_lds) pE[q] = __hiloint2double(rec4.w, rec4.z);
                    pkb[q] = ((uint32_t)rec4.y & 0x1ffffu) | ((key < 0 ? 0x7fffu : (uint32_t)key) << 17);
                    if (use_tbl && key >= 0) {
                        const int d = (int)((uint32_t)rec4.y >> 17);
                        if (d >= len) bad = true;
                        else {
                            const int row = (q < stale_p1 && stale_d >= 0) ? len : d;
                            tbl[row * n_part + (key >> 2)] = (uint16_t)(q + 1);
                            atomicOr(&tblm[row], 1u << (key >> 2));
                        }
                    }
                }
            }
            wsync();
            if (WSA_TUNE(16)) ph[0] = __builtin_readcyclecounter();
            if (!use_tbl) bad = false;
            for (int base = len; base <= (use_tbl ? -1 : c_ci + 1); base += 64) {
                const int d = base + lane;
                if (d <= c_ci + 1 && W.d_gen[d] == gen)
                    for (int q = W.d_p0[d]; q < W.d_p1[d]; q++) if ((pkb[q] >> 17) != 0x7fffu) bad = true;
            }
            if (stale_d >= len && lane == 0)
                for (int q = 0; q < stale_p1; q++) if ((pkb[q] >> 17) != 0x7fffu) bad = true;
            if (__ballot(bad) != 0ull) { if (lane == 0) { sg[SEG_FLAG] = -1; sg[SEG_NROWS] = 0; } return true; }
            if (use_tbl) {
                const uint32_t stale_m = tblm[len];
                float thr_f;
                { const double t0 = floor_ < 0 ? 0.0 : floor(floor_) + 1.0; thr_f = (float)(t0 > 256.0 ? 256.0 : t0); }
                for (int base = 0; base < ((WSA_TUNE(8)) ? 0 : len); base += 64) {
                    const int d = base + lane;
                    float* const row = fr + 9 * (d < len ? d : 0);
                    if (d < len) {
#pragma unroll
                        for (int q = 0; q < 9; q++) row[q] = 0.f;
                    }
                    float sm = 0.f;
                    auto apply = [&](int q) __attribute__((always_inline)) {
                        const uint32_t w = pkb[q];
                        int l = (int)((w >> 17) & 3u);
                        const double E = energy_of(q);
                        const float ff = (float)(w & 0xffu), cur = row[3 * l];
                        if (cur >= thr_f && cur < ff && l < 2) l++;
                        row[3 * l] = ff; row[3 * l + 1] = (float)E; row[3 * l + 2] = (float)((w >> 8) & 0x1ffu);
                        sm = (float)((double)sm + E);
                    };
                    const uint32_t m_main = d < len ? tblm[d] : 0u, m_st = (d < len && d == stale_d) ? stale_m : 0u;
                    uint32_t mm = m_main | m_st;
                    while (mm) {
                        const int r = __ffs((int)mm) - 1; mm &= mm - 1u;
                        if ((m_st >> r) & 1u) apply((int)tbl[len * n_part + r] - 1);
                        if ((m_main >> r) & 1u) apply((int)tbl[d * n_part + r] - 1);
                    }
                    if (d < len) smv[d] = sm;
                }
            } else
            for (int base = 0; base < ((WSA_TUNE(8)) ? 0 : len); base += 64) {
                const int d = base + lane;
                if (d < len) {
                    float f9[9];
#pragma unroll
                    for (int q = 0; q < 9; q++) f9[q] = 0.f;
                    float sm = 0.f;
                    const int a1 = (stale_d == d) ? stale_p1 : 0;
                    const int dg = W.d_gen[d], dp0 = W.d_p0[d], dp1 = W.d_p1[d];
                    const bool has_main = dg == gen;
                    const int b0 = has_main ? dp0 : 0, b1 = has_main ? dp1 : 0;
                    int last_key = -1;
                    for (;;) {
                        int best_key = 0x7fffffff, best_q = -1;
                        for (int q = 0; q < a1; q++) {
                            const uint32_t w = pkb[q];
                            const int key = (int)(((w >> 19) << 16) | (uint32_t)q);
                            if ((w >> 17) != 0x7fffu && key > last_key && key < best_key) { best_key = key; best_q = q; }
                        }
                        for (int q = b0; q < b1; q++) {
                            const uint32_t w = pkb[q];
                            const int key = (int)(((w >> 19) << 16) | (uint32_t)q);
                            if ((w >> 17) != 0x7fffu && key > last_key && key < best_key) { best_key = key; best_q = q; }
                        }
                        if (best_q < 0) break;
                        last_key = best_key;
                        const uint32_t w = pkb[best_q];
                        int l = (int)((w >> 17) & 3u);
                        const double f = w & 0xffu, wd = (w >> 8) & 0x1ffu, E = energy_of(best_q);
                        const float cur = l == 0 ? f9[0] : (l == 1 ? f9[3] : f9[6]);
                        if ((double)cur > floor_ && (double)cur < f && l < 2) l++;
                        const float ff = (float)f, Ef = (float)E, wf = (float)wd;
                        if (l == 0) { f9[0] = ff; f9[1] = Ef; f9[2] = wf; }
                        else if (l == 1) { f9[3] = ff; f9[4] = Ef; f9[5] = wf; }
                        else { f9[6] = ff; f9[7] = Ef; f9[8] = wf; }
                        sm = (float)((double)sm + E);
                    }
#pragma unroll
                    for (int q = 0; q < 9; q++) fr[9 * d + q] = f9[q];
                    smv[d] = sm;
                }
            }
            wsync();
            if (WSA_TUNE(16)) ph[1] = __builtin_readcyclecounter();
            if (p.formants && (p.level == 4 || p.level == 10)) {
                for (int q = lane; q < 9 * len; q += 64) { const int d = q / 9; p.formants[((uint64_t)foff + (((uint32_t)start + (uint32_t)d) & p.ring_mask)) * 9 + (uint32_t)(q - 9 * d)] = fr[q]; }
                if (p.sums) { for (int q = lane; q < len; q += 64) p.sums[(uint64_t)foff + (((uint32_t)start + (uint32_t)q) & p.ring_mask)] = smv[q]; }
            }
            double accS, accC; acc_totals(accS, accC);
            const double cs = accC / accS;
            const double lg_ctx = jsm::log10(ctx_max);
            double* const red = reinterpret_cast<double*>(s_big + off_pt);
            if (p.level == 4 || p.level == 5) {
                const long long r0 = take_rows(1);
                if (r0 < 0) return true;
                double* x = p.row_feat + (uint64_t)r0 * WSA_NFEAT;
                if (WSA_TUNE(16)) ph[2] = __builtin_readcyclecounter();
                if (p.level == 5) {
                    if (!(WSA_TUNE(4))) formant_features_lds(fr, len, ctx_max, x, lane, red, !G && len <= 15 && !(p.dbg & 65536), G || (p.dbg & 131072) != 0);
                    if (WSA_TUNE(16)) ph[3] = __builtin_readcyclecounter();
                    if (lane == 0) { x[0] = len; x[1] = sqrt((double)len); x[2] = cs; x[3] = lg_ctx; x[4] = floor_; }
                } else if (lane < WSA_NFEAT) x[lane] = 0;
                if (lane == 0) {
                    int32_t* m = p.row_meta + (uint64_t)r0 * 8;
                    m[0] = (int32_t)clip; m[1] = 0; m[2] = 0; m[3] = 0; m[4] = my_seg; m[5] = 0; m[6] = start; m[7] = len;
                    sg[SEG_FLAG] = 1; sg[SEG_NROWS] = 1; sg[SEG_ROW0] = (int32_t)r0;
                }
                return true;
            }
            int nsyl = 0, my_si = 0, my_sl = 0;
            {
                int si = -1, cc = 0, uu = 0;
                for (int base = 0; base < len; base += 64) {
                    const int dd = base + lane;
                    const float smq = dd < len ? smv[dd] : 0.f;
                    const int lim = min(64, len - base);
                    for (int j = 0; j < lim; j++) {
                        const int e2 = base + j;
                        const double v = __builtin_bit_cast(float, read_lane_i32(__builtin_bit_cast(int, smq), j));
                        if (v > floor_) { cc = 0; uu++; if (si < 0) si = e2; } else cc++;
                        if ((uu > 20 && cc > 0) || (uu > 10 && cc > 1) || (uu > 0 && cc > 4) || (e2 >= len - 1 && uu > 4)) {
                            const int t = e2 - cc;
                            if (t - si > 1) {
                                if (nsyl < 64) { if (lane == nsyl) { my_si = si; my_sl = t - si; } }
                                else if (lane == 0) { W.q_idx[2 * nsyl] = si; W.q_idx[2 * nsyl + 1] = t - si; }
                                nsyl++;
                                si = -1; uu = 0;
                            }
                        }
                    }
                }
            }
            wsync();
            long long r0 = 0;
            if (nsyl > 0) { r0 = take_rows(nsyl); if (r0 < 0) return true; }
            for (int k = 0; k < nsyl; k++) {
                const int si = k < 64 ? read_lane_i32(my_si, k) : W.q_idx[2 * k], sl = k < 64 ? read_lane_i32(my_sl, k) : W.q_idx[2 * k + 1];
                double* x = p.row_feat + (uint64_t)(r0 + k) * WSA_NFEAT;
                if (p.level == 13) {
                    if (!(WSA_TUNE(4))) formant_features_lds(fr + 9 * si, sl, ctx_max, x, lane, red, !G && sl <= 15 && !(p.dbg & 65536), G || (p.dbg & 131072) != 0);
                    if (lane == 0) { x[0] = sl; x[1] = sqrt((double)sl); x[2] = cs; x[3] = lg_ctx; x[4] = floor_; }
                } else if (lane < WSA_NFEAT) x[lane] = 0;
                if (lane == 0) {
                    int32_t* m = p.row_meta + (uint64_t)(r0 + k) * 8;
                    m[0] = (int32_t)clip; m[1] = 0; m[2] = si; m[3] = sl; m[4] = my_seg; m[5] = k; m[6] = start + si; m[7] = sl;
                }
            }
            if (lane == 0) { sg[SEG_FLAG] = nsyl > 0 ? 1 : 0; sg[SEG_NROWS] = nsyl; sg[SEG_ROW0] = (int32_t)r0; }
            return true;
        };
        auto finalize_fast = [&]() __attribute__((always_inline)) -> bool {
            if (finalize_fast_impl(std::false_type{})) return true;
            if constexpr (SPLIT == 2) { if (!(p.dbg & 262144)) return finalize_fast_impl(std::true_type{}); }
            return false;
        };
        auto finalize_slow = [&]() __attribute__((always_inline)) {
            if (WSA_TUNE(16)) ph[0] = ph[1] = ph[2] = ph[3] = __builtin_readcyclecounter();
            int nq = 0;
            for (int base = 0; base < n_tr; base += 64) {
                const int t = base + lane;
                bool q = false; double mb = 0;
                if (t < n_tr) {
                    W.tr_slot[t] = -1;
                    if (W.tr_len[t] >= 2) { mb = W.tr_sumEbin[t] / W.tr_sumE[t]; q = mb >= 7; }
                }
                const uint64_t mask = __ballot(q);
                if (q) { const int pos = nq + __popcll(mask & lanemask_lt(lane)); W.q_idx[pos] = t; W.q_mb[pos] = mb; }
                nq += __popcll(mask);
            }
            wsync();
            const bool q_lds = nq <= AC;
            double* qmb = W.q_mb; int32_t* qidx = W.q_idx; int32_t* sorted = W.sorted;
            if (q_lds) {
                for (int qi = lane; qi < nq; qi += 64) { f_qmb[qi] = W.q_mb[qi]; f_qidx[qi] = W.q_idx[qi]; }
                qmb = f_qmb; qidx = f_qidx; sorted = f_sorted;
                wsync();
            }
            for (int base = 0; base < nq; base += 64) {
                const int qi = base + lane;
                if (qi < nq) {
                    const double mb = qmb[qi];
                    int rank = 0;
                    for (int u = 0; u < nq; u++) { const double o = qmb[u]; rank += (o < mb || (o == mb && u < qi)) ? 1 : 0; }
                    sorted[rank] = qi;
                }
            }
            wsync();
            {
                double last = 0; int slot = 0; bool stopped = false;
                for (int base = 0; base < nq && !stopped; base += 64) {
                    const int r = base + lane;
                    double mb = 0; int t = 0;
                    if (r < nq) { const int qi = sorted[r]; mb = qmb[qi]; t = qidx[qi]; }
                    uint64_t todo = __ballot(r < nq);
                    int myslot = -1;
                    while (todo) {
                        const uint64_t jm = __ballot(((todo >> lane) & 1ull) && fabs(mb - last) > 20);
                        if (jm == 0ull) { if ((todo >> lane) & 1ull) myslot = slot; break; }
                        const int j = __ffsll((long long)jm) - 1;
                        if (((todo >> lane) & 1ull) && lane < j) myslot = slot;
                        last = __hiloint2double(__builtin_amdgcn_readlane(__double2hiint(mb), j), __builtin_amdgcn_readlane(__double2loint(mb), j));
                        slot++;
                        if (slot >= 3) { stopped = true; break; }
                        todo &= ~lanemask_lt(j);
                    }
                    if (myslot >= 0) W.tr_slot[t] = (r << 2) | myslot;
                }
            }
            wsync();
            {
                int t_nxt = lane < n_pt ? W.pt[lane].x : 0;
                for (int q = lane; q < n_pt; q += 64) {
                    const int t = t_nxt;
                    if (q + 64 < n_pt) t_nxt = W.pt[q + 64].x;
                    W.pt_key[q] = W.tr_slot[t];
                }
            }
            wsync();
            if (WSA_TUNE(16)) ph[0] = __builtin_readcyclecounter();
            bool bad = false;
            for (int base = len; base <= c_ci + 1; base += 64) {
                const int d = base + lane;
                if (d <= c_ci + 1 && W.d_gen[d] == gen)
                    for (int q = W.d_p0[d]; q < W.d_p1[d]; q++) if (W.pt_key[q] >= 0) bad = true;
            }
            if (stale_d >= len && lane == 0)
                for (int q = 0; q < stale_p1; q++) if (W.pt_key[q] >= 0) bad = true;
            if (__ballot(bad) != 0ull) { if (lane == 0) { sg[SEG_FLAG] = -1; sg[SEG_NROWS] = 0; } return; }
            float* const fr = len <= FRCAP ? f_fr : W.fr;
            float* const smv_ = len <= FRCAP ? f_sm : W.sm1;
            auto slow_features = [&](const float* f, int a, double* x) __attribute__((always_inline)) {
                if (len > FRCAP && a <= FEAT_LDS_MAX) formant_features_lds(f, a, ctx_max, x, lane, reinterpret_cast<double*>(s_big), false, true);
                else formant_features_wave(f, a, ctx_max, x, W.Aev, aev_stride, lane);
            };
            for (int base = 0; base < ((WSA_TUNE(8)) ? 0 : len); base += 64) {
                const int d = base + lane;
                if (d < len) {
                    float f9[9];
#pragma unroll
                    for (int q = 0; q < 9; q++) f9[q] = 0.f;
                    float sm = 0.f;
                    const int a0 = 0, a1 = (stale_d == d) ? stale_p1 : 0;
                    const bool has_main = W.d_gen[d] == gen;
                    const int b0 = has_main ? W.d_p0[d] : 0, b1 = has_main ? W.d_p1[d] : 0;
                    long long last_key = -1;
                    for (;;) {
                        long long best_key = 0x7fffffffffffffffLL; int best_q = -1;
                        for (int part = 0; part < 2; part++) {
                            const int q0 = part ? b0 : a0, q1 = part ? b1 : a1;
                            for (int q = q0; q < q1; q++) {
                                const int pk = W.pt_key[q];
                                if (pk < 0) continue;
                                const long long key = (long long)(pk >> 2) * (long long)(p.pcap + 1) + q;
                                if (key > last_key && key < best_key) { best_key = key; best_q = q; }
                            }
                        }
                        if (best_q < 0) break;
                        last_key = best_key;
                        int l = W.pt_key[best_q] & 3;
                        const int4 rec4 = W.pt[best_q];
                        const int bw = rec4.y;
                        const double f = bw & 0xff, wd = (bw >> 8) & 0x1ff, E = __hiloint2double(rec4.w, rec4.z);
                        const float cur = l == 0 ? f9[0] : (l == 1 ? f9[3] : f9[6]);
                        if ((double)cur > floor_ && (double)cur < f && l < 2) l++;
                        const float ff = (float)f, Ef = (float)E, wf = (float)wd;
                        if (l == 0) { f9[0] = ff; f9[1] = Ef; f9[2] = wf; }
                        else if (l == 1) { f9[3] = ff; f9[4] = Ef; f9[5] = wf; }
                        else { f9[6] = ff; f9[7] = Ef; f9[8] = wf; }
                        sm = (float)((double)sm + E);
                    }
#pragma unroll
                    for (int q = 0; q < 9; q++) fr[9 * d + q] = f9[q];
                    smv_[d] = sm;
                }
            }
            wsync();
            if (WSA_TUNE(16)) ph[1] = __builtin_readcyclecounter();
            if (p.formants && (p.level == 4 || p.level == 10)) {
                for (int q = lane; q < 9 * len; q += 64) { const int d = q / 9; p.formants[((uint64_t)foff + (((uint32_t)start + (uint32_t)d) & p.ring_mask)) * 9 + (uint32_t)(q - 9 * d)] = fr[q]; }
                if (p.sums) { for (int q = lane; q < len; q += 64) p.sums[(uint64_t)foff + (((uint32_t)start + (uint32_t)q) & p.ring_mask)] = smv_[q]; }
            }
            double accS, accC; acc_totals(accS, accC);
            const double cs = accC / accS;
            const double lg_ctx = jsm::log10(ctx_max);
            if (p.level == 4 || p.level == 5) {
                const long long r0 = take_rows(1);
                if (r0 < 0) return;
                double* x = p.row_feat + (uint64_t)r0 * WSA_NFEAT;
                if (WSA_TUNE(16)) ph[2] = __builtin_readcyclecounter();
                if (p.level == 5) {
                    if (!(WSA_TUNE(4))) slow_features(fr, len, x);
                    if (WSA_TUNE(16)) ph[3] = __builtin_readcyclecounter();
                    if (lane == 0) { x[0] = len; x[1] = sqrt((double)len); x[2] = cs; x[3] = lg_ctx; x[4] = floor_; }
                } else if (lane < WSA_NFEAT) x[lane] = 0;
                if (lane == 0) {
                    int32_t* m = p.row_meta + (uint64_t)r0 * 8;
                    m[0] = (int32_t)clip; m[1] = 0; m[2] = 0; m[3] = 0; m[4] = my_seg; m[5] = 0; m[6] = start; m[7] = len;
                    sg[SEG_FLAG] = 1; sg[SEG_NROWS] = 1; sg[SEG_ROW0] = (int32_t)r0;
                }
                return;
            }
            int nsyl = 0;
            {
                int si = -1, cc = 0, uu = 0;
                for (int base = 0; base < len; base += 64) {
                    const int dd = base + lane;
                    const float smv = dd < len ? smv_[dd] : 0.f;
                    const int lim = min(64, len - base);
                    for (int j = 0; j < lim; j++) {
                        const int e2 = base + j;
                        const double v = __builtin_bit_cast(float, read_lane_i32(__builtin_bit_cast(int, smv), j));
                        if (v > floor_) { cc = 0; uu++; if (si < 0) si = e2; } else cc++;
                        if ((uu > 20 && cc > 0) || (uu > 10 && cc > 1) || (uu > 0 && cc > 4) || (e2 >= len - 1 && uu > 4)) {
                            const int t = e2 - cc;
                            if (t - si > 1) {
                                if (lane == 0) { W.q_idx[2 * nsyl] = si; W.q_idx[2 * nsyl + 1] = t - si; }
                                nsyl++;
                                si = -1; uu = 0;
                            }
                        }
                    }
                }
            }
            wsync();
            long long r0 = 0;
            if (nsyl > 0) { r0 = take_rows(nsyl); if (r0 < 0) return; }
            for (int k = 0; k < nsyl; k++) {
                const int si = W.q_idx[2 * k], sl = W.q_idx[2 * k + 1];
                double* x = p.row_feat + (uint64_t)(r0 + k) * WSA_NFEAT;
                if (p.level == 13) {
                    if (!(WSA_TUNE(4))) slow_features(fr + 9 * si, sl, x);
                    if (lane == 0) { x[0] = sl; x[1] = sqrt((double)sl); x[2] = cs; x[3] = lg_ctx; x[4] = floor_; }
                } else if (lane < WSA_NFEAT) x[lane] = 0;
                if (lane == 0) {
                    int32_t* m = p.row_meta + (uint64_t)(r0 + k) * 8;
                    m[0] = (int32_t)clip; m[1] = 0; m[2] = si; m[3] = sl; m[4] = my_seg; m[5] = k; m[6] = start + si; m[7] = sl;
                }
            }
            if (lane == 0) { sg[SEG_FLAG] = nsyl > 0 ? 1 : 0; sg[SEG_NROWS] = nsyl; sg[SEG_ROW0] = (int32_t)r0; }
        };

        struct Hdr { int info; double v, fl; uint4 h; };
        struct Pre { int info; double v, fl, g; int n; uint32_t pk, amp, plo, phi, hi; };
        auto uni_i = [](int x) __attribute__((always_inline)) { return __builtin_amdgcn_readfirstlane(x); };
        auto uni_d = [](double x) __attribute__((always_inline)) {
            return __hiloint2double(__builtin_amdgcn_readfirstlane(__double2hiint(x)), __builtin_amdgcn_readfirstlane(__double2loint(x)));
        };
        auto load_hdr = [&](uint32_t f, Hdr& q) __attribute__((always_inline)) {
            const uint32_t fi = (min(f, f_end - 1) & p.ring_mask) + (uint32_t)vz;
            q.info = p.fr_info[foff + fi]; q.v = p.fr_v[foff + fi]; q.fl = p.fr_fl[foff + fi];
            q.h = p.rec.hdr[foff + fi];
        };
        auto load_ent = [&](uint32_t f, const Hdr& h, Pre& q) __attribute__((always_inline)) {
            const int hy = uni_i((int)h.h.y);
            q.info = f < f_end ? uni_i(h.info) : -1; q.v = uni_d(h.v); q.fl = uni_d(h.fl);
            q.g = (double)(hy & 0xff) * 4294967296.0 + (double)(uint32_t)uni_i((int)h.h.x);
            q.n = (hy >> 8) & 0xff; q.pk = q.amp = q.plo = q.phi = q.hi = 0;
            if (q.info >= 0 && lane < q.n && !(WSA_TUNE(32))) {
                const uint32_t c = (uint32_t)uni_i((int)h.h.w) + (uint32_t)lane;
                const uint4 e4 = p.rec.ent[c];
                q.amp = p.rec.amp[c]; q.pk = e4.x; q.plo = e4.y; q.phi = e4.z; q.hi = e4.w;
            }
        };
        auto accumulate = [&](const Pre& cur, auto&& refill) __attribute__((always_inline)) {
            const int info = cur.info;
            if (!(info >= 0 && !(WSA_TUNE(2)))) refill();
            else {
                {
                    const int ncand = cur.n;
                    const double g = cur.g, v = cur.v;
                    const uint32_t pkw = cur.pk, amp = cur.amp;
                    const double plo = (double)(cur.hi & 0xffu) * 4294967296.0 + (double)cur.plo, phi = (double)((cur.hi >> 8) & 0xffu) * 4294967296.0 + (double)cur.phi;
                    const bool reset_this_frame = (info >> 30) & 1;
                    const int t_idx = info & 0x3fffffff;
                    const bool acc = lane < ncand && (double)amp > v;
                    const uint64_t amask = __ballot(acc);
                    const int n = __popcll(amask);
                    if (n < 1) refill();
                    if (n >= 1) {
                        if (WSA_TUNE(512)) act = __builtin_readcyclecounter();
                        const int nfile = t_idx;
                        const double fl = cur.fl;
                        accG += g;
                        const int my_o = __popcll(amask & lanemask_lt(lane));
                        if (acc) { s_pk[my_o] = pkw; s_amp[my_o] = amp; s_plo[my_o] = plo; s_phi[my_o] = phi; }
                        refill();
                        wsync();
                        int pk_i = 0, pk_s = 0, pk_l = -1000; uint32_t pk_amp = 0; double pk_plo = 0, pk_phi = 0;
                        if (lane < n) {
                            const uint32_t w = s_pk[lane];
                            pk_i = w & 0xff; pk_s = (w >> 8) & 0xff; pk_l = (w >> 16) & 0xff;
                            pk_amp = s_amp[lane]; pk_plo = s_plo[lane]; pk_phi = s_phi[lane];
                        }
                        WSA_ACP(0);
                        {
                            int kept = 0;
                            for (int base = 0; base < n_act; base += 64) {
                                const int j = base + lane;
                                const bool valid = j < n_act;
                                const int lf = valid ? a_last_frame[j] : 0;
                                const bool keep = valid && (nfile - lf) < 4;
                                const uint64_t km = __ballot(keep);
                                if (kept == base && km == __ballot(valid)) { kept += __popcll(km); continue; }
                                int ln = 0, gi = 0; uint32_t bn = 0, am = 0; double ve = 0, se = 0, sb = 0;
                                if (valid) { ln = a_len[j]; gi = a_gid[j]; bn = a_bins[j]; am = a_amp[j]; ve = a_vel[j]; se = a_sumE[j]; sb = a_sumEbin[j]; }
                                if (valid && !keep) { W.tr_len[gi] = ln; W.tr_sumE[gi] = se; W.tr_sumEbin[gi] = sb; }
                                wsync();
                                if (keep) {
                                    const int q = kept + __popcll(km & lanemask_lt(lane));
                                    a_last_frame[q] = lf; a_len[q] = ln; a_gid[q] = gi; a_bins[q] = bn; a_amp[q] = am; a_vel[q] = ve; a_sumE[q] = se; a_sumEbin[q] = sb;
                                }
                                kept += __popcll(km);
                                wsync();
                            }
                            n_act = kept;
                        }
                        WSA_ACP(1);
                        int asg = -1; double best = 0;
                        for (int tbase = 0; tbase < n_act; tbase += 64) {
                            const int j = tbase + lane;
                            const bool valid = j < n_act;
                            int gap = -1, bin = 0;
                            if (valid) { gap = nfile - a_last_frame[j]; bin = (int)(a_bins[j] & 0xff); a_mmask[j] = 0ull; }
                            const bool live = valid && gap >= 0 && gap < 4;
                            const int win = gap == 0 ? 3 : (gap == 1 ? 4 : (gap == 2 ? 6 : 9));
                            int o_lo = 0, o_hi = 0;
                            for (int o = 0; o < n; o++) {
                                const int lo = __builtin_amdgcn_readlane(pk_l, o);
                                o_lo += (lo <= bin - win) ? 1 : 0;
                                o_hi += (lo < bin + win) ? 1 : 0;
                            }
                            const int cnt = live ? o_hi - o_lo : 0;
                            const int incl = (int)wave_incl_scan_u32((uint32_t)cnt);
                            const int off = incl - cnt;
                            const int M = __builtin_amdgcn_readlane(incl, 63);
                            const int maxc = (int)wave_max_u32((uint32_t)cnt);
                            for (int base = 0; base < M; base += 64) {
                                if (lane < MAXC) { s_best[lane] = 0ull; s_asg[lane] = 0x7fffffff; }
                                for (int c = 0; c < maxc; c++) {
                                    const int slot = off + c - base;
                                    if (c < cnt && slot >= 0 && slot < 64) { s_pr_j[slot] = j; s_pr_o[slot] = o_lo + c; }
                                }
                                wsync();
                                const bool pv = base + lane < M;
                                int jj = 0, oo = 0; double sc = 0;
                                if (pv) {
                                    jj = s_pr_j[lane]; oo = s_pr_o[lane];
                                    const int tb = (int)(a_bins[jj] & 0xff), tg = nfile - a_last_frame[jj];
                                    const int pl = (int)((s_pk[oo] >> 16) & 0xff);
                                    sc = match_score(tg, (double)abs(tb - pl), (double)a_len[jj], (double)tb, (double)pl,
                                                     (double)a_amp[jj], (double)s_amp[oo], a_vel[jj]);
                                    if (sc > 1) atomicMax(&s_best[oo], (unsigned long long)__double_as_longlong(sc));
                                }
                                wsync();
                                if (pv && sc > 1 && (unsigned long long)__double_as_longlong(sc) == s_best[oo]) atomicMin(&s_asg[oo], jj);
                                wsync();
                                if (lane < n) {
                                    const int cj = s_asg[lane];
                                    if (cj != 0x7fffffff) {
                                        const double cs = __longlong_as_double((long long)s_best[lane]);
                                        if (cs > best) { best = cs; asg = cj; }
                                    }
                                }
                                wsync();
                            }
                        }
                        WSA_ACP(2);
                        if (lane < n && asg >= 0) atomicOr(&a_mmask[asg], 1ull << lane);
                        wsync();
                        const int p_begin = n_pt;
                        for (int tbase = 0; tbase < n_act; tbase += 64) {
                            const int j = tbase + lane;
                            const unsigned long long mm = j < n_act ? a_mmask[j] : 0ull;
                            bool upd = false; int pb = 0, st = 0, en = 0; uint32_t a0 = 0; double be = 0;
                            if (mm) {
                                const int first = __ffsll((long long)mm) - 1;
                                const uint32_t w0 = s_pk[first];
                                pb = (w0 >> 16) & 0xff;
                                a0 = s_amp[first];
                                if ((double)a0 > fl) {
                                    upd = true;
                                    st = w0 & 0xff; en = (w0 >> 8) & 0xff;
                                    double lo_sum = s_plo[first], hi_sum = s_phi[first];
                                    uint32_t pb_amp = a0;
                                    unsigned long long rest = mm & (mm - 1ull);
                                    while (rest) {
                                        const int o = __ffsll((long long)rest) - 1; rest &= rest - 1;
                                        const uint32_t w = s_pk[o];
                                        const int oi = w & 0xff, os = (w >> 8) & 0xff, ol = (w >> 16) & 0xff;
                                        if (os > en) { en = os; hi_sum = s_phi[o]; }
                                        if (oi < st) { st = oi; lo_sum = s_plo[o]; }
                                        if (s_amp[o] > pb_amp) { pb = ol; pb_amp = s_amp[o]; }
                                    }
                                    be = hi_sum - lo_sum;
                                }
                            }
                            const uint64_t um = __ballot(upd);
                            const int nu = __popcll(um);
                            if (n_pt + nu > p.pcap) { overflow = true; }
                            else if (upd) {
                                const int q = n_pt + __popcll(um & lanemask_lt(lane));
                                const int hlen = a_len[j];
                                const uint32_t bn = a_bins[j];
                                const int P1 = bn & 0xff, P2 = (bn >> 8) & 0xff, P3 = (bn >> 16) & 0xff;
                                double vel = a_vel[j];
                                if (hlen >= 3) {
                                    const double xv = (double)((pb - P1) + (P2 - P1) + (P3 - P2)), third = 1.0 / 3.0;
                                    const double q0 = xv * third;
                                    vel = __builtin_fma(__builtin_fma(-3.0, q0, xv), third, q0);
                                }
                                else if (hlen == 2) vel = (double)((pb - P1) + (P2 - P1)) / 2;
                                else if (hlen == 1) vel = (double)(pb - P1);
                                const double se = a_sumE[j] + be, sb = a_sumEbin[j] + be * pb;
                                a_vel[j] = vel; a_bins[j] = (uint32_t)pb | ((uint32_t)P1 << 8) | ((uint32_t)P2 << 16);
                                a_amp[j] = a0; a_last_frame[j] = nfile; a_len[j] = hlen + 1; a_sumE[j] = se; a_sumEbin[j] = sb;
                                const int t = a_gid[j];
                                W.pt[q] = make_int4(t, pb | ((en - st + 1) << 8) | (min(nfile, 0x7fff) << 17), __double2loint(be), __double2hiint(be));
                                if (RAW) W.ptx[q] = make_int4(st, (int)a0, nfile, en);
                            }
                            if (upd) accL += be;
                            if (!overflow) n_pt += nu;
                        }
                        WSA_ACP(3);
                        const bool mk = lane < n && asg == -1 && (double)pk_amp > fl;
                        const uint64_t nm = __ballot(mk);
                        const int nnew = __popcll(nm);
                        if (n_act + nnew > ((p.dbg & 1024) && AC < AC_MAX ? 12 : AC)) { act_overflow = true; overflow = true; }
                        if (n_tr + nnew > p.tcap || n_pt + nnew > p.pcap) overflow = true;
                        if (overflow) {}
                        else if (mk) {
                            const int r = __popcll(nm & lanemask_lt(lane));
                            const int t = n_tr + r, q = n_pt + r, j = n_act + r;
                            const double be = pk_phi - pk_plo;
                            a_last_frame[j] = nfile; a_len[j] = 1; a_gid[j] = t; a_bins[j] = (uint32_t)pk_l; a_amp[j] = pk_amp;
                            a_vel[j] = 0; a_sumE[j] = be; a_sumEbin[j] = be * pk_l;
                            W.pt[q] = make_int4(t, pk_l | ((pk_s - pk_i + 1) << 8) | (min(nfile, 0x7fff) << 17), __double2loint(be), __double2hiint(be));
                            if (RAW) W.ptx[q] = make_int4(pk_i, (int)pk_amp, nfile, pk_s);
                        }
                        if (!overflow) { n_tr += nnew; n_pt += nnew; n_act += nnew; }
                        WSA_ACP(4);
                        if (reset_this_frame) { stale_d = nfile; stale_p1 = n_pt; }
                        else if (lane == 0 && nfile < p.fcap + 2) { W.d_p0[nfile] = p_begin; W.d_p1[nfile] = n_pt; W.d_gen[nfile] = gen; }
                        wsync();
                    }
                }
            }
        };
        auto finish_span = [&]() __attribute__((always_inline)) {
            if constexpr (!PAIR) { for (int j = lane; j < n_act; j += 64) { const int gi = a_gid[j]; W.tr_len[gi] = a_len[j]; W.tr_sumE[gi] = a_sumE[j]; W.tr_sumEbin[gi] = a_sumEbin[j]; } }
            wsync();
            if constexpr (RAW) {
                int nq = 0;
                for (int base = 0; base < n_tr; base += 64) {
                    const int t = base + lane;
                    bool q = false; double mb = 0;
                    if (t < n_tr && W.tr_len[t] >= 2) { mb = W.tr_sumEbin[t] / W.tr_sumE[t]; q = mb >= 7; }
                    const uint64_t mask = __ballot(q);
                    if (q) { const int pos = nq + __popcll(mask & lanemask_lt(lane)); W.q_idx[pos] = t; W.q_mb[pos] = mb; }
                    nq += __popcll(mask);
                }
                wsync();
                const uint64_t pbase = (uint64_t)foff * MAXC;
                const uint64_t pmask = ST ? (uint64_t)(p.ring_mask + 1u) * MAXC - 1ull : ~0ull;
                const uint64_t poff = (ST ? (uint64_t)((uint32_t)sg[SEG_FBEGIN] & p.ring_mask) : (uint64_t)f_begin) * MAXC;
                const uint64_t pool0 = pbase + poff;
                auto slot = [&](uint64_t q) __attribute__((always_inline)) -> uint64_t { return pbase + ((poff + q) & pmask); };
                for (int qi = lane; qi < nq; qi += 64) {
                    const double mb = W.q_mb[qi];
                    int rank = 0;
                    for (int u = 0; u < nq; u++) { const double o = W.q_mb[u]; rank += (o < mb || (o == mb && u < qi)) ? 1 : 0; }
                    p.trk_rank[slot((uint64_t)rank)] = W.q_idx[qi];
                }
                for (int q = lane; q < n_pt; q += 64) { int4 v = W.pt[q]; v.y &= 0x1ffff; p.trk_pts[2 * slot((uint64_t)q)] = v; p.trk_pts[2 * slot((uint64_t)q) + 1] = W.ptx[q]; }
                if (lane == 0) {
                    int32_t* ts = p.trk_seg + ((uint64_t)clip * p.seg_cap + my_seg) * 4;
                    ts[0] = (int32_t)(pool0 & 0xffffffffu); ts[1] = n_pt; ts[2] = nq; ts[3] = (int32_t)(pool0 >> 32);
                }
            } else
            if (!(WSA_TUNE(1))) { if ((p.dbg & 256) || !finalize_fast()) finalize_slow(); }
        };
        if constexpr (SPLIT == 2) {
            const double* hd = p.span_hdr + ((uint64_t)clip * p.seg_cap + k_seg) * 8;
            const double h0 = hd[0], h1 = hd[1], h2 = hd[2], h3 = hd[3], h4 = hd[4], h5 = hd[5], h6 = hd[6];
            const int flag = (int)h6;
            if (flag == 0) continue;
            if (flag & 2) { if (lane == 0) atomicOr(&p.shared[1], 1u); continue; }
            const int F = (int)(f_end - f_begin);
            W = carve_ws(p.pool + (uint64_t)(foff + f_begin) * p.pool_bpf, MAXC * F, MAXC * F, F, 0, nullptr);
            aev_stride = F + 2;
            n_tr = (int)h0; n_pt = (int)h1; n_act = 0; stale_d = (int)h2; stale_p1 = (int)h3;
            accG = h4; accL = lane == 0 ? h5 : 0.0;
            gen = 1;
            const unsigned long long tf0 = WSA_TUNE(16) ? __builtin_readcyclecounter() : 0ull;
            finish_span();
            if (WSA_TUNE(16) && lane == 0 && p.trace) {
                double* tr = p.trace + (uint64_t)atomicAdd(&p.shared[0], 1u) * 12;
                tr[0] = 0; tr[1] = (double)(__builtin_readcyclecounter() - tf0); tr[2] = len; tr[3] = F; tr[4] = n_tr; tr[5] = n_pt; tr[6] = blockIdx.x;
                tr[7] = (double)(ph[0] - tf0); tr[8] = (double)(ph[1] - ph[0]); tr[9] = (double)(ph[2] - ph[1]); tr[10] = (double)(ph[3] - ph[2]);
            }
            if (overflow && lane == 0) atomicOr(&p.shared[1], 1u);
            wsync();
            continue;
        } else
        if constexpr (PAIR) {
            static_assert(GW == 32 || (GW == 16 && SPLIT == 1), "four spans per wave only as the accumulate half of the split tracker");
            static_assert(GW <= GW_MAX, "the SPLIT kernels' span regions are sized for at most GW_MAX new tracks / points per frame (see tracker_pool_bpf)");
            constexpr int ACG = GW == 32 ? PAIR_AC : QUAD_AC, NGR = 64 / GW, GSZ = GW == 32 ? PAIR_GSZ : QUAD_GSZ;
            const int g = lane / GW, gl = lane % GW;
            const uint32_t below = (1u << gl) - 1u;
            unsigned char* const gb = s_big + g * GSZ;
            double* const t_vel = reinterpret_cast<double*>(gb);
            double* const t_sumE = t_vel + ACG;
            double* const t_sumEbin = t_sumE + ACG;
            uint32_t* const t_mmask = reinterpret_cast<uint32_t*>(t_sumEbin + ACG);
            int32_t* const t_lf = reinterpret_cast<int32_t*>(t_mmask + ACG);
            int32_t* const t_len = t_lf + ACG;
            int32_t* const t_gid = t_len + ACG;
            uint32_t* const t_bins = reinterpret_cast<uint32_t*>(t_gid + ACG);
            uint32_t* const t_amp = t_bins + ACG;
            uint32_t* const q_pk = t_amp + ACG;
            uint32_t* const q_amp = q_pk + GW;
            uint32_t* const q_plo = q_amp + GW;
            uint32_t* const q_phi = q_plo + GW;
            uint32_t* const q_hi = q_phi + GW;
            unsigned long long* const q_best = reinterpret_cast<unsigned long long*>(q_hi + GW);
            int32_t* const q_asg = reinterpret_cast<int32_t*>(q_best + GW);
            int32_t* const q_prj = q_asg + GW;
            int32_t* const q_pro = q_prj + GW;
            uint32_t* const q_map = reinterpret_cast<uint32_t*>(q_pro + GW);
            static_assert(NGR * GSZ <= LDS_ALL && GSZ % 16 == 0 && GSZ >= ACG * 48 + GW * 40 + 24 && (ACG * 24) % 8 == 0 && (ACG * 48 + GW * 20) % 8 == 0, "group layout fits the block");
            const uint32_t e_idx = (uint32_t)(NGR * pair_idx) + (uint32_t)g;
            const bool has = e_idx < pair_total;
            const uint2 oe = has ? p.order[e_idx] : make_uint2(0u, 0u);
            const uint32_t g_clip = oe.x, g_seg = oe.y;
            const int32_t* gsg = p.seg_i + ((uint64_t)g_clip * p.seg_cap + g_seg) * 8;
            const uint32_t g_fb = has ? (uint32_t)gsg[SEG_FBEGIN] : 0u, g_fe = has ? (uint32_t)gsg[SEG_FEND] : 0u;
            const uint32_t g_foff = p.frame_off[g_clip];
            const int g_F = (int)(g_fe - g_fb);
            const int g_tcap = SPLIT ? MAXC * g_F : p.tcap, g_fcap = SPLIT ? g_F : p.fcap;
            const Ws Wg = SPLIT ? carve_ws(p.pool + (uint64_t)(g_foff + g_fb) * p.pool_bpf, g_tcap, g_tcap, g_fcap, 0, nullptr)
                                : carve_ws(p.ws + ((uint64_t)blockIdx.x * 2 + (uint32_t)g) * p.ws_stride, p.tcap, p.pcap, p.fcap, 0, nullptr);
            if (SPLIT) { if (has) for (int d = gl; d < g_F + 2; d += GW) Wg.d_gen[d] = 0; }
            int g_ntr = 0, g_npt = 0, g_nact = 0, g_stale_d = -1, g_stale_p1 = 0;
            double g_accG = 0, g_accL = 0;
            bool g_ovf = false, g_redo = SPLIT && has && g_F < 1;
            if (gl == 0) { q_map[0] = 0u; q_map[5] = 0u; }
            auto dbl40 = [](uint32_t lo, uint32_t hi8) __attribute__((always_inline)) { return (double)(hi8 & 0xffu) * 4294967296.0 + (double)lo; };
            struct FH { int info; double v, fl; uint4 h; };
            struct FC { uint4 e; uint32_t amp; };
            auto load_fh = [&](uint32_t k, FH& q) __attribute__((always_inline)) {
                const uint32_t f = g_fb + k, fi = g_foff + (g_fe > g_fb ? min(f, g_fe - 1u) : 0u);
                auto at = [](const auto* base, uint32_t byte_off) __attribute__((always_inline)) { return *reinterpret_cast<decltype(base)>(reinterpret_cast<const char*>(base) + byte_off); };
                q.info = at(p.fr_info, fi << 2); q.v = at(p.fr_v, fi << 3); q.fl = at(p.fr_fl, fi << 3); q.h = at(p.rec.hdr, fi << 4);
                if (f >= g_fe) q.info = -1;
            };
            auto load_fc = [&](const FH& h, FC& q) __attribute__((always_inline)) {
                q.e = make_uint4(0u, 0u, 0u, 0u); q.amp = 0u;
                if (h.info >= 0 && gl < (int)((h.h.y >> 8) & 0xffu)) { const uint32_t c = h.h.w + (uint32_t)gl; q.e = p.rec.ent[c]; q.amp = p.rec.amp[c]; }
            };
            const int nsteps = groups_max_i32<GW>((int)(g_fe - g_fb));
            unsigned long long pcy[5] = {0, 0, 0, 0, 0}, pt0 = 0; int pn_chunk2 = 0, pn_pass = 0, pn_on = 0;
#define WSA_PCY(k_) do { if (WSA_TUNE(16)) { const unsigned long long now_ = __builtin_readcyclecounter(); pcy[k_] += now_ - pt0; pt0 = now_; } } while (0)
            const unsigned long long ptk0 = WSA_TUNE(16) ? __builtin_readcyclecounter() : 0ull;
            FH h0, h1, h2; FC c0, c1;
            load_fh(0u, h0); load_fh(1u, h1); load_fc(h0, c0);
            for (int step = 0; step < nsteps; step++) {
                load_fh((uint32_t)step + 2u, h2);
                load_fc(h1, c1);
                const bool act = h0.info >= 0 && !g_redo && !WSA_TUNE(2);
                if (__ballot(act) != 0ull) {
                    const int info = h0.info, nfile = info & 0x3fffffff;
                    const bool rst = ((info >> 30) & 1) != 0;
                    const int ncand = (int)((h0.h.y >> 8) & 0xffu);
                    const double v = h0.v, fl = h0.fl;
                    if (WSA_TUNE(16)) pt0 = __builtin_readcyclecounter();
                    if (gl < 4) q_map[1 + gl] = 0u;
                    wsync();
                    int n = 0;
                    const int ncmax = groups_max_i32<GW>(act ? ncand : 0);
                    for (int cb = 0; cb < ncmax; cb += GW) {
                        uint4 e4 = c0.e; uint32_t am = c0.amp;
                        const bool hasc = act && cb + gl < ncand;
                        if (cb > 0) { e4 = make_uint4(0u, 0u, 0u, 0u); am = 0u; if (hasc) { const uint32_t c = h0.h.w + (uint32_t)(cb + gl); e4 = p.rec.ent[c]; am = p.rec.amp[c]; } }
                        const bool acc = hasc && (double)am > v;
                        const uint32_t m = group_ballot<GW>(acc, lane);
                        const int pos = n + __popc(m & below);
                        if (acc && pos < GW) {
                            q_pk[pos] = e4.x; q_amp[pos] = am; q_plo[pos] = e4.y; q_phi[pos] = e4.z; q_hi[pos] = e4.w;
                            const uint32_t lb = (e4.x >> 16) & 0x7fu;
                            atomicOr(&q_map[1 + (lb >> 5)], 1u << (lb & 31u));
                        }
                        n += __popc(m);
                    }
                    if (WSA_TUNE(16) && act && n > GW && !g_redo && gl == 0) atomicAdd(&p.shared[10], 1u);
                    if (act && n > GW) g_redo = true;
                    const bool on = act && n >= 1 && n <= GW;
                    if (on) g_accG += (double)(h0.h.y & 0xffu) * 4294967296.0 + (double)h0.h.x;
                    wsync();
                    if (__ballot(on) != 0ull) {
                        const bool ispk = on && gl < n;
                        const uint32_t pkw = q_pk[gl], pamp = q_amp[gl];
                        const int pk_i = pkw & 0xff, pk_s = (pkw >> 8) & 0xff, pk_l = (pkw >> 16) & 0xff;
                        const uint32_t m0 = q_map[1], m1 = q_map[2], m2 = q_map[3], m3 = q_map[4];
                        const int pc1 = __popc(m0), pc2 = pc1 + __popc(m1), pc3 = pc2 + __popc(m2);
                        WSA_PCY(0); pn_on++;
                        const bool compact = on && ((step & 3) == 0 || g_nact + n > ACG);
                        if (__ballot(compact) != 0ull) {
                            int kept = 0;
                            const int na_max = groups_max_i32<GW>(compact ? g_nact : 0);
                            for (int tb = 0; tb < na_max; tb += GW) {
                                const int j = tb + gl;
                                const bool valid = compact && j < g_nact;
                                const int jr = GW == 32 ? j : min(j, ACG - 1);
                                const int lf = t_lf[jr], ln = t_len[jr], gi = t_gid[jr]; const uint32_t bn = t_bins[jr], am = t_amp[jr]; const double ve = t_vel[jr], se = t_sumE[jr], sb = t_sumEbin[jr];
                                const bool keep = valid && (nfile - lf) < 4;
                                const uint32_t km = group_ballot<GW>(keep, lane);
                                if (valid && !keep) { Wg.tr_len[gi] = ln; Wg.tr_sumE[gi] = se; Wg.tr_sumEbin[gi] = sb; }
                                wsync();
                                if (keep) {
                                    const int q = kept + __popc(km & below);
                                    t_lf[q] = lf; t_len[q] = ln; t_gid[q] = gi; t_bins[q] = bn; t_amp[q] = am; t_vel[q] = ve; t_sumE[q] = se; t_sumEbin[q] = sb;
                                }
                                kept += __popc(km);
                                wsync();
                            }
                            if (compact) g_nact = kept;
                        }
                        WSA_PCY(1);
                        int asg = -1; double best = 0;
                        const int na_max = groups_max_i32<GW>(on ? g_nact : 0);
                        if (na_max > GW) pn_chunk2++;
                        for (int tb = 0; tb < na_max; tb += GW) {
                            const int j = tb + gl;
                            const bool valid = on && j < g_nact;
                            const int jr = GW == 32 ? j : min(j, ACG - 1);
                            const int gap = nfile - t_lf[jr], bin = (int)(t_bins[jr] & 0xffu);
                            if (valid) t_mmask[j] = 0u;
                            const bool live = valid && gap >= 0 && gap < 4;
                            const int win = (int)((0x9643u >> (4 * (gap & 3))) & 0xfu);
                            const int lo = max(bin - win + 1, 0), width = bin + win - lo;
                            const int w0 = lo >> 5, sh = lo & 31;
                            const uint32_t wa = w0 == 0 ? m0 : (w0 == 1 ? m1 : (w0 == 2 ? m2 : m3));
                            const uint32_t wb = w0 == 0 ? m1 : (w0 == 1 ? m2 : (w0 == 2 ? m3 : 0u));
                            const uint32_t wnd = (uint32_t)(((((unsigned long long)wb) << 32) | wa) >> sh) & ((1u << width) - 1u);
                            const int o_lo = (w0 == 0 ? 0 : (w0 == 1 ? pc1 : (w0 == 2 ? pc2 : pc3))) + __popc(wa & ((1u << sh) - 1u));
                            const int cnt = live ? __popc(wnd) : 0;
                            const int incl = (int)group_incl_scan_u32<GW>((uint32_t)cnt);
                            const int off = incl - cnt;
                            const int M = (int)group_last_u32<GW>((uint32_t)incl, lane);
                            const int M_max = groups_max_i32<GW>(M);
                            for (int base = 0; base < M_max; base += GW) {
                                pn_pass++;
                                q_best[gl] = 0ull; q_asg[gl] = 0x7fffffff;
                                for (int c = 0; __ballot(c < cnt) != 0ull; c++) {
                                    const int slot = off + c - base;
                                    if (c < cnt && slot >= 0 && slot < GW) { q_prj[slot] = j; q_pro[slot] = o_lo + c; }
                                }
                                wsync();
                                const bool pv = base + gl < M;
                                const int jj = (int)min((uint32_t)q_prj[gl], (uint32_t)(ACG - 1)), oo = (int)min((uint32_t)q_pro[gl], (uint32_t)(GW - 1));
                                const int tbn = (int)(t_bins[jj] & 0xffu), tg = nfile - t_lf[jj];
                                const int pl = (int)((q_pk[oo] >> 16) & 0xffu);
                                const double sc = match_score(tg, (double)abs(tbn - pl), (double)t_len[jj], (double)tbn, (double)pl,
                                                              (double)t_amp[jj], (double)q_amp[oo], t_vel[jj]);
                                const bool cand = pv && sc > 1;
                                if (cand) atomicMax(&q_best[oo], (unsigned long long)__double_as_longlong(sc));
                                wsync();
                                if (cand && (unsigned long long)__double_as_longlong(sc) == q_best[oo]) atomicMin(&q_asg[oo], jj);
                                wsync();
                                {
                                    const int cj = q_asg[gl];
                                    const double cs = __longlong_as_double((long long)q_best[gl]);
                                    if (ispk && cj != 0x7fffffff && cs > best) { best = cs; asg = cj; }
                                }
                                wsync();
                            }
                        }
                        WSA_PCY(2);
                        if (ispk && asg >= 0) atomicOr(&t_mmask[asg], 1u << gl);
                        wsync();
                        const int p_begin = g_npt;
                        for (int tb = 0; tb < na_max; tb += GW) {
                            const int j = tb + gl;
                            const uint32_t mm = (on && j < g_nact) ? t_mmask[j] : 0u;
                            const int first = mm ? __ffs((int)mm) - 1 : 0;
                            const uint32_t w0_ = q_pk[first], a0 = q_amp[first], hb = q_hi[first];
                            const uint32_t plo0 = q_plo[first], phi0 = q_phi[first];
                            const bool upd = mm != 0u && (double)a0 > fl;
                            int pb = (w0_ >> 16) & 0xff, st = w0_ & 0xff, en = (w0_ >> 8) & 0xff;
                            uint32_t lo_l = plo0, lo_h = hb & 0xffu, hi_l = phi0, hi_h = (hb >> 8) & 0xffu;
                            {
                                uint32_t pb_amp = a0;
                                uint32_t rest = upd ? mm & (mm - 1u) : 0u;
                                while (rest) {
                                    const int o = __ffs((int)rest) - 1; rest &= rest - 1u;
                                    const uint32_t w = q_pk[o];
                                    const int oi = w & 0xff, os = (w >> 8) & 0xff, ol = (w >> 16) & 0xff;
                                    const uint32_t hbo = q_hi[o], ao = q_amp[o], plo_o = q_plo[o], phi_o = q_phi[o];
                                    if (os > en) { en = os; hi_l = phi_o; hi_h = (hbo >> 8) & 0xffu; }
                                    if (oi < st) { st = oi; lo_l = plo_o; lo_h = hbo & 0xffu; }
                                    if (ao > pb_amp) { pb = ol; pb_amp = ao; }
                                }
                            }
                            const unsigned long long be_i = (((unsigned long long)hi_h << 32) | hi_l) - (((unsigned long long)lo_h << 32) | lo_l);
                            const double be = upd ? (double)(uint32_t)(be_i >> 32) * 4294967296.0 + (double)(uint32_t)be_i : 0.0;
                            const uint32_t um = group_ballot<GW>(upd, lane);
                            const int nu = __popc(um);
                            if (!SPLIT && g_npt + nu > g_tcap) g_ovf = true;
                            else if (upd) {
                                const int q = g_npt + __popc(um & below);
                                const int hlen = t_len[j];
                                const uint32_t bn = t_bins[j];
                                const int P1 = bn & 0xff, P2 = (bn >> 8) & 0xff, P3 = (bn >> 16) & 0xff;
                                const double xv = (double)((pb - P1) + (P2 - P1) + (P3 - P2)), third = 1.0 / 3.0;
                                const double q0 = xv * third;
                                const double v3 = __builtin_fma(__builtin_fma(-3.0, q0, xv), third, q0);
                                const double v2 = (double)((pb - P1) + (P2 - P1)) * 0.5, v1 = (double)(pb - P1);
                                const double vel = hlen >= 3 ? v3 : (hlen == 2 ? v2 : (hlen == 1 ? v1 : t_vel[j]));
                                const double se = t_sumE[j] + be, sb = t_sumEbin[j] + be * pb;
                                t_vel[j] = vel; t_bins[j] = (uint32_t)pb | ((uint32_t)P1 << 8) | ((uint32_t)P2 << 16);
                                t_amp[j] = a0; t_lf[j] = nfile; t_len[j] = hlen + 1; t_sumE[j] = se; t_sumEbin[j] = sb;
                                Wg.pt[q] = make_int4(t_gid[j], pb | ((en - st + 1) << 8) | (min(nfile, 0x7fff) << 17), __double2loint(be), __double2hiint(be));
                            }
                            if (upd) g_accL += be;
                            if (!g_ovf) g_npt += nu;
                        }
                        WSA_PCY(3);
                        const bool mk = ispk && asg == -1 && (double)pamp > fl;
                        const uint32_t nm = group_ballot<GW>(mk, lane);
                        const int nnew = __popc(nm);
                        if (WSA_TUNE(16) && on && g_nact + nnew > ACG && !g_redo && gl == 0) atomicAdd(&p.shared[11], 1u);
                        if (on && g_nact + nnew > ((p.dbg & (1024 | 16384)) ? 12 : ACG)) g_redo = true;
                        if (!SPLIT && on && (g_ntr + nnew > g_tcap || g_npt + nnew > g_tcap)) g_ovf = true;
                        const bool grow = on && !g_ovf && !g_redo;
                        if (grow && mk) {
                            const int r = __popc(nm & below);
                            const int t = g_ntr + r, q = g_npt + r, j = g_nact + r;
                            const uint32_t hb = q_hi[gl];
                            const double be = dbl40(q_phi[gl], hb >> 8) - dbl40(q_plo[gl], hb);
                            t_lf[j] = nfile; t_len[j] = 1; t_gid[j] = t; t_bins[j] = (uint32_t)pk_l; t_amp[j] = pamp;
                            t_vel[j] = 0; t_sumE[j] = be; t_sumEbin[j] = be * pk_l;
                            Wg.pt[q] = make_int4(t, pk_l | ((pk_s - pk_i + 1) << 8) | (min(nfile, 0x7fff) << 17), __double2loint(be), __double2hiint(be));
                        }
                        if (grow) { g_ntr += nnew; g_npt += nnew; g_nact += nnew; }
                        if (on) {
                            if (rst) { g_stale_d = nfile; g_stale_p1 = g_npt; }
                            else if (gl == 0 && nfile < g_fcap + 2) { Wg.d_p0[nfile] = p_begin; Wg.d_p1[nfile] = g_npt; Wg.d_gen[nfile] = SPLIT ? 1 : gen; }
                        }
                        wsync();
                        WSA_PCY(4);
                    }
                }
                h0 = h1; h1 = h2; c0 = c1;
            }
#undef WSA_PCY
            const unsigned long long ptk1 = WSA_TUNE(16) ? __builtin_readcyclecounter() : 0ull;
            for (int j = gl; j < g_nact; j += GW) { const int gi = t_gid[j]; Wg.tr_len[gi] = t_len[j]; Wg.tr_sumE[gi] = t_sumE[j]; Wg.tr_sumEbin[gi] = t_sumEbin[j]; }
            wsync();
            if constexpr (SPLIT == 1) {
                double cg[NGR];
#pragma unroll
                for (int q = 0; q < NGR; q++) cg[q] = g == q ? g_accL : 0.0;
                wave_sums_f64(cg);
                double c_mine = cg[0];
#pragma unroll
                for (int q = 1; q < NGR; q++) c_mine = g == q ? cg[q] : c_mine;
                if (has && gl == 0) {
                    if (g_redo) { const uint32_t k = atomicAdd(p.redo_count, 1u); p.redo[k] = make_uint2(g_clip, g_seg); }
                    double* hd = p.span_hdr + ((uint64_t)g_clip * p.seg_cap + g_seg) * 8;
                    hd[0] = g_ntr; hd[1] = g_npt; hd[2] = g_stale_d; hd[3] = g_stale_p1; hd[4] = g_accG; hd[5] = c_mine;
                    hd[6] = g_redo ? 0.0 : (g_ovf ? 2.0 : 1.0);
                }
            } else
            for (int gs = 0; gs < (GW == 32 ? 2 : 0); gs++) {
                const int src = gs * 32;
                if (!read_lane_i32((int)has, src)) continue;
                clip = (uint32_t)read_lane_i32((int)g_clip, src); k_seg = (uint32_t)read_lane_i32((int)g_seg, src); my_seg = (int)k_seg;
                if (read_lane_i32((int)g_redo, src)) {
                    if (lane == 0) { const uint32_t k = atomicAdd(p.redo_count, 1u); p.redo[k] = make_uint2(clip, k_seg); }
                    continue;
                }
                sg = p.seg_i + ((uint64_t)clip * p.seg_cap + my_seg) * 8;
                start = sg[SEG_START]; len = sg[SEG_LEN]; c_ci = sg[SEG_CCI];
                f_begin = (uint32_t)sg[SEG_FBEGIN]; f_end = (uint32_t)sg[SEG_FEND];
                ctx_max = p.seg_d[((uint64_t)clip * p.seg_cap + my_seg) * 2];
                floor_ = p.seg_d[((uint64_t)clip * p.seg_cap + my_seg) * 2 + 1];
                foff = p.frame_off[clip];
                n_tr = read_lane_i32(g_ntr, src); n_pt = read_lane_i32(g_npt, src); n_act = 0;
                stale_d = read_lane_i32(g_stale_d, src); stale_p1 = read_lane_i32(g_stale_p1, src);
                accG = __hiloint2double(read_lane_i32(__double2hiint(g_accG), src), read_lane_i32(__double2loint(g_accG), src));
                accL = g == gs ? g_accL : 0.0;
                overflow = read_lane_i32((int)g_ovf, src) != 0; act_overflow = false;
                W = carve_ws(p.ws + ((uint64_t)blockIdx.x * 2 + (uint32_t)gs) * p.ws_stride, p.tcap, p.pcap, p.fcap, 0, nullptr);
                if (!overflow) finish_span();
                if (overflow && lane == 0) atomicOr(&p.shared[1], 1u);
                wsync();
            }
            if (WSA_TUNE(16) && lane == 0 && p.trace) {
                double* tr = p.trace + (uint64_t)atomicAdd(&p.shared[0], 1u) * 12;
                tr[0] = (double)(ptk1 - ptk0); tr[1] = (double)(__builtin_readcyclecounter() - ptk1); tr[2] = nsteps; tr[3] = pn_on; tr[4] = pn_chunk2; tr[5] = pn_pass; tr[6] = blockIdx.x;
                tr[7] = (double)pcy[0]; tr[8] = (double)pcy[1]; tr[9] = (double)pcy[2]; tr[10] = (double)pcy[3]; tr[11] = (double)pcy[4];
            }
            gen++;
            continue;
        } else
        if constexpr (ST) {
            int32_t* stt = p.st_state + (uint64_t)clip * TR_STATE_WORDS;
            double* std_ = reinterpret_cast<double*>(stt + 8);
            n_tr = stt[0]; n_pt = stt[1]; n_act = stt[2]; stale_d = stt[3]; stale_p1 = stt[4]; int my_span = stt[5]; gen = stt[6];
            accG = std_[0] + std_[1]; accL = lane == 0 ? std_[1] : 0.0;
            char* ab = p.st_act + (uint64_t)clip * TR_ACT_BYTES;
            double* const g_vel = reinterpret_cast<double*>(ab); double* const g_sumE = g_vel + AC; double* const g_sumEbin = g_sumE + AC;
            int32_t* const g_lf = reinterpret_cast<int32_t*>(g_sumEbin + AC); int32_t* const g_len = g_lf + AC; int32_t* const g_gid = g_len + AC;
            uint32_t* const g_bins = reinterpret_cast<uint32_t*>(g_gid + AC); uint32_t* const g_amp = g_bins + AC;
            for (int j = lane; j < n_act; j += 64) {
                a_vel[j] = g_vel[j]; a_sumE[j] = g_sumE[j]; a_sumEbin[j] = g_sumEbin[j];
                a_last_frame[j] = g_lf[j]; a_len[j] = g_len[j]; a_gid[j] = g_gid[j]; a_bins[j] = g_bins[j]; a_amp[j] = g_amp[j];
            }
            wsync();
            auto clear_state = [&](int span) __attribute__((always_inline)) { n_tr = n_pt = n_act = 0; stale_d = -1; stale_p1 = 0; accG = accL = 0; gen++; my_span = span; };
            const uint32_t nfr = p.n_frames_step[clip];
            const uint32_t fbase = (uint32_t)p.gate_state[(uint64_t)clip * GATE_STATE] - nfr;
            const int nseg = (int)p.seg_count[clip];
            f_begin = fbase; f_end = fbase + nfr;
            int ks = 0;
            auto close_segments = [&](uint32_t f_next, bool all) __attribute__((always_inline)) {
                while (ks < nseg) {
                    int32_t* sgk = p.seg_i + ((uint64_t)clip * p.seg_cap + ks) * 8;
                    if (!all && (uint32_t)sgk[SEG_FEND] != f_next) break;
                    if (sgk[SEG_FBEGIN] != my_span) clear_state(sgk[SEG_FBEGIN]);
                    my_seg = ks; sg = sgk; start = sg[SEG_START]; len = sg[SEG_LEN]; c_ci = sg[SEG_CCI];
                    ctx_max = p.seg_d[((uint64_t)clip * p.seg_cap + ks) * 2]; floor_ = p.seg_d[((uint64_t)clip * p.seg_cap + ks) * 2 + 1];
                    finish_span();
                    clear_state(-2);
                    ks++;
                }
            };
            for (uint32_t f = fbase; f < fbase + nfr; f++) {
                Hdr h; load_hdr(f, h);
                Pre cur; load_ent(f, h, cur);
                if (cur.info >= 0) {
                    const int sp = p.fr_span[foff + (f & p.ring_mask)];
                    if (sp != my_span) clear_state(sp);
                    accumulate(cur, [] {});
                }
                close_segments(f + 1, false);
            }
            close_segments(0, true);
            double accS, accC; acc_totals(accS, accC);
            if (lane == 0) { stt[0] = n_tr; stt[1] = n_pt; stt[2] = n_act; stt[3] = stale_d; stt[4] = stale_p1; stt[5] = my_span; stt[6] = gen; std_[0] = accS; std_[1] = accC; }
            for (int j = lane; j < n_act; j += 64) {
                g_vel[j] = a_vel[j]; g_sumE[j] = a_sumE[j]; g_sumEbin[j] = a_sumEbin[j];
                g_lf[j] = a_last_frame[j]; g_len[j] = a_len[j]; g_gid[j] = a_gid[j]; g_bins[j] = a_bins[j]; g_amp[j] = a_amp[j];
            }
        } else {
            constexpr int PFD = 4;
            struct Blk { int info; double v, fl; uint4 h; };
            struct Ent { uint32_t pk, amp, plo, phi, hi; };
            auto load_blk = [&](uint32_t fb, Blk& q) __attribute__((always_inline)) {
                const uint32_t f = fb + (uint32_t)lane, fi = foff + min(f, f_end - 1);
                q.info = p.fr_info[fi]; q.v = p.fr_v[fi]; q.fl = p.fr_fl[fi]; q.h = p.rec.hdr[fi];
                if (f >= f_end) q.info = -1;
            };
            Blk bc, bn;
            auto rl = [](int x, int j) __attribute__((always_inline)) { return __builtin_amdgcn_readlane(x, j); };
            auto rl_d = [&](double x, int j) __attribute__((always_inline)) { return __hiloint2double(rl(__double2hiint(x), j), rl(__double2loint(x), j)); };
            auto request = [&](int j, Ent& e) __attribute__((always_inline)) {
                const int info_ = j < 64 ? rl(bc.info, j & 63) : rl(bn.info, j & 63);
                const int hy = j < 64 ? rl((int)bc.h.y, j & 63) : rl((int)bn.h.y, j & 63);
                const uint32_t cb = (uint32_t)(j < 64 ? rl((int)bc.h.w, j & 63) : rl((int)bn.h.w, j & 63));
                e.pk = e.amp = e.plo = e.phi = e.hi = 0u;
                if (info_ >= 0 && lane < ((hy >> 8) & 0xff) && !(WSA_TUNE(32))) {
                    const uint32_t c = cb + (uint32_t)lane;
                    const uint4 e4 = p.rec.ent[c];
                    e.amp = p.rec.amp[c]; e.pk = e4.x; e.plo = e4.y; e.phi = e4.z; e.hi = e4.w;
                }
            };
            load_blk(f_begin, bc);
            bn = bc;
            if (f_begin + 64 < f_end) load_blk(f_begin + 64, bn);
            Ent ring[PFD];
    #pragma unroll
            for (int k = 0; k < PFD; k++) request(k, ring[k]);
            for (uint32_t blk = f_begin; blk < f_end; blk += 64) {
              const int nb = (int)min(64u, f_end - blk);
              for (int j0 = 0; j0 < nb; j0 += PFD) {
    #pragma unroll
                for (int k = 0; k < PFD; k++) {
                  const int j = j0 + k;
                  if (j >= nb) break;
                  Pre cur;
                  const int hy = rl((int)bc.h.y, j);
                  cur.info = rl(bc.info, j); cur.v = rl_d(bc.v, j); cur.fl = rl_d(bc.fl, j);
                  cur.g = (double)(hy & 0xff) * 4294967296.0 + (double)(uint32_t)rl((int)bc.h.x, j);
                  cur.n = (hy >> 8) & 0xff;
                  cur.pk = ring[k].pk; cur.amp = ring[k].amp; cur.plo = ring[k].plo; cur.phi = ring[k].phi; cur.hi = ring[k].hi;
                  accumulate(cur, [&]() __attribute__((always_inline)) { request(j + PFD, ring[k]); });
                  if (p.trace && !(WSA_TUNE(16))) { double accS, accC; acc_totals(accS, accC); if (lane == 0) { double* tr = p.trace + ((uint64_t)foff + blk + (uint32_t)j) * 12; tr[10] = accS; tr[11] = accC; } }
                }
              }
              bc = bn;
              if (blk + 128 < f_end && !(WSA_TUNE(64))) load_blk(blk + 128, bn);
            }
            tk1 = (WSA_TUNE(16)) ? __builtin_readcyclecounter() : 0ull;
            finish_span();
        }
        if ((WSA_TUNE(16)) && lane == 0 && p.trace) {
            double* tr = p.trace + (uint64_t)atomicAdd(&p.shared[0], 1u) * 12;
            tr[0] = (double)(tk1 - tk0); tr[1] = (double)(__builtin_readcyclecounter() - tk1); tr[2] = len; tr[3] = (double)(f_end - f_begin); tr[4] = n_tr; tr[5] = n_pt; tr[6] = blockIdx.x;
            if (WSA_TUNE(512)) { tr[7] = (double)acp[0]; tr[8] = (double)acp[1]; tr[9] = (double)acp[2]; tr[10] = (double)acp[3]; tr[11] = (double)acp[4]; }
            else { tr[7] = (double)(ph[0] - tk1); tr[8] = (double)(ph[1] - ph[0]); tr[9] = (double)(ph[2] - ph[1]); tr[10] = (double)(ph[3] - ph[2]); }
        }
        if (overflow && lane == 0) atomicOr(&p.shared[1], act_overflow && AC < AC_MAX ? 2u : 1u);
        wsync();
    }
}

__global__ __launch_bounds__(64) __attribute__((amdgpu_waves_per_eu(4, 4))) void tracker_kernel_fast(TrParams p) { tracker_body<AC_FAST, false, false>(p); }
__global__ __launch_bounds__(64) __attribute__((amdgpu_waves_per_eu(3, 4))) void tracker_kernel_pair(TrParams p) {
    __builtin_amdgcn_s_setprio(3);
    tracker_body<AC_FAST, false, false, true>(p);
}
__global__ __launch_bounds__(64) __attribute__((amdgpu_waves_per_eu(4, 4))) void tracker_kernel_pair_acc(TrParams p) {
    __builtin_amdgcn_s_setprio(3);
    tracker_body<AC_FAST, false, false, true, 1>(p);
}
__global__ __launch_bounds__(64) __attribute__((amdgpu_waves_per_eu(4, 4))) void tracker_kernel_quad_acc(TrParams p) {
    __builtin_amdgcn_s_setprio(3);
    tracker_body<AC_FAST, false, false, true, 1, 16>(p);
}
__global__ __launch_bounds__(64) __attribute__((amdgpu_waves_per_eu(4, 4))) void tracker_kernel_finalize(TrParams p) {
    __builtin_amdgcn_s_setprio(3);
    tracker_body<AC_FAST, false, false, false, 2>(p);
}
__global__ __launch_bounds__(64) void tracker_kernel_full(TrParams p) { tracker_body<AC_MAX, false, false>(p); }
__global__ __launch_bounds__(64) void tracker_kernel_raw(TrParams p) { tracker_body<AC_MAX, true, false>(p); }
__global__ __launch_bounds__(64) void tracker_kernel_stream(TrParams p) { tracker_body<AC_MAX, false, true>(p); }
__global__ __launch_bounds__(64) void tracker_kernel_stream_raw(TrParams p) { tracker_body<AC_MAX, true, true>(p); }

constexpr int ORDER_T = 256;
__global__ __launch_bounds__(ORDER_T) void span_order_kernel(const uint32_t* hist, const uint2* key, const uint32_t* seg_count, uint32_t n_clips, int seg_cap, uint2* order, uint32_t* counters) {
    __shared__ uint32_t offs[SPAN_BUCKETS], part[ORDER_T];
    const int tid = threadIdx.x;
    constexpr int PER = SPAN_BUCKETS / ORDER_T;
    uint32_t mine[PER], sum = 0;
#pragma unroll
    for (int q = 0; q < PER; q++) { mine[q] = hist[tid * PER + q]; sum += mine[q]; }
    part[tid] = sum;
    __syncthreads();
    for (int d = 1; d < ORDER_T; d <<= 1) {
        const uint32_t add = tid >= d ? part[tid - d] : 0u;
        __syncthreads();
        part[tid] += add;
        __syncthreads();
    }
    uint32_t run = part[tid] - sum;
#pragma unroll
    for (int q = 0; q < PER; q++) { offs[tid * PER + q] = run; run += mine[q]; }
    if (blockIdx.x == 0 && tid == ORDER_T - 1) counters[1] = part[tid];
    __syncthreads();
    const uint32_t clip = blockIdx.x * ORDER_T + tid;
    if (clip >= n_clips) return;
    const uint32_t ns = seg_count[clip];
    for (uint32_t k = 0; k < ns; k++) {
        const uint2 e = key[(uint64_t)clip * seg_cap + k];
        order[offs[e.x] + e.y] = make_uint2(clip, k);
    }
}

void launch_span_order(const TrParams& p, uint32_t* span_hist, const uint2* span_key, uint2* order, uint32_t* counters, hipStream_t s) {
    if (p.n_clips == 0) return;
    hipLaunchKernelGGL(span_order_kernel, dim3((p.n_clips + ORDER_T - 1) / ORDER_T), dim3(ORDER_T), 0, s, span_hist, span_key, p.seg_count, p.n_clips, p.seg_cap, order, counters);
}

void launch_tracker_stream(const TrParams& p, uint32_t n_streams, hipStream_t s) {
    if (n_streams == 0) return;
    static_assert(AC_MAX == TR_ACT_MAX, "the streams' saved active table is sized for the full variant");
    if (p.level == 3) hipLaunchKernelGGL(tracker_kernel_stream_raw, dim3(n_streams), dim3(64), 0, s, p);
    else hipLaunchKernelGGL(tracker_kernel_stream, dim3(n_streams), dim3(64), 0, s, p);
}

void launch_tracker(const TrParams& p, int n_waves, bool full_table, bool pair, hipStream_t s) {
    if (n_waves <= 0) return;
    if (p.level == 3) hipLaunchKernelGGL(tracker_kernel_raw, dim3(n_waves), dim3(64), 0, s, p);
    else if (full_table) hipLaunchKernelGGL(tracker_kernel_full, dim3(n_waves), dim3(64), 0, s, p);
    else if (pair && p.order && p.redo && (!p.trace || (p.dbg & 16))) {
        if (p.pool && p.span_hdr) {
            if (p.quad) hipLaunchKernelGGL(tracker_kernel_quad_acc, dim3(p.quad_waves > 0 ? p.quad_waves : n_waves), dim3(64), 0, s, p);
            else hipLaunchKernelGGL(tracker_kernel_pair_acc, dim3(n_waves), dim3(64), 0, s, p);
            hipLaunchKernelGGL(tracker_kernel_finalize, dim3(p.fin_waves > 0 ? p.fin_waves : 2 * n_waves), dim3(64), 0, s, p);
        }
        else hipLaunchKernelGGL(tracker_kernel_pair, dim3(n_waves), dim3(64), 0, s, p);
        TrParams r = p; r.order = p.redo; r.order_cnt = 2; r.pool = nullptr; r.span_hdr = nullptr;
        const int redo_waves = p.quad ? 1024 : 128;
        hipLaunchKernelGGL(tracker_kernel_fast, dim3(n_waves < redo_waves ? n_waves : redo_waves), dim3(64), 0, s, r);
    }
    else hipLaunchKernelGGL(tracker_kernel_fast, dim3(n_waves), dim3(64), 0, s, p);
}

__global__ void compact_count_kernel(CompactParams p) {
    const uint32_t c = blockIdx.x * blockDim.x + threadIdx.x;
    if (c >= p.n_clips) return;
    const uint32_t ns = p.seg_count[c];
    const int32_t* sg = p.seg_i + (uint64_t)c * p.seg_cap * 8;
    uint32_t r = 0;
    for (uint32_t k = 0; k < ns; k++) if (sg[8 * k + SEG_FLAG] >= 0) r += (uint32_t)sg[8 * k + SEG_NROWS];
    p.clip_row_off[c] = r;
}
constexpr int CSCAN_T = 1024;
template <bool COUNT>
__global__ __launch_bounds__(CSCAN_T) void compact_scan_kernel(CompactParams p) {
    __shared__ uint32_t s_rows[CSCAN_T], s_segs[CSCAN_T];
    const int tid = threadIdx.x;
    const uint32_t per = (p.n_clips + CSCAN_T - 1) / CSCAN_T;
    const uint32_t c0 = min(p.n_clips, tid * per), c1 = min(p.n_clips, c0 + per);
    uint32_t rs = 0, ss = 0;
    for (uint32_t c = c0; c < c1; c++) {
        if (COUNT) {
            const uint32_t ns = p.seg_count[c];
            const int32_t* sg = p.seg_i + (uint64_t)c * p.seg_cap * 8;
            uint32_t r = 0;
            for (uint32_t k = 0; k < ns; k++) if (sg[8 * k + SEG_FLAG] >= 0) r += (uint32_t)sg[8 * k + SEG_NROWS];
            p.clip_row_off[c] = r;
        }
        ss += p.seg_count[c]; rs += p.clip_row_off[c];
    }
    s_rows[tid] = rs; s_segs[tid] = ss;
    __syncthreads();
    for (int d = 1; d < CSCAN_T; d <<= 1) {
        const uint32_t ar_ = tid >= d ? s_rows[tid - d] : 0u, as_ = tid >= d ? s_segs[tid - d] : 0u;
        __syncthreads();
        s_rows[tid] += ar_; s_segs[tid] += as_;
        __syncthreads();
    }
    if (tid == CSCAN_T - 1) {
        p.totals[0] = s_rows[tid]; p.totals[1] = s_segs[tid];
        p.clip_row_off[p.n_clips] = s_rows[tid]; p.clip_seg_off[p.n_clips] = s_segs[tid];
    }
    uint32_t ar = s_rows[tid] - rs, as = s_segs[tid] - ss;
    for (uint32_t c = c0; c < c1; c++) {
        const uint32_t r = p.clip_row_off[c];
        p.clip_row_off[c] = ar; p.clip_seg_off[c] = as; as += p.seg_count[c]; ar += r;
    }
}

template <bool FUSED>
__global__ __launch_bounds__(64) void compact_gather_kernel(CompactParams p) {
    const uint32_t clip = blockIdx.x;
    const int lane = threadIdx.x;
    const uint32_t nseg = p.seg_count[clip];
    if (FUSED) {
        uint32_t rs = 0, ss = 0;
        for (uint32_t i = lane; i < clip; i += 64) { rs += p.clip_rows[i]; ss += p.seg_count[i]; }
        rs = wave_sum_u32(rs); ss = wave_sum_u32(ss);
        if (lane == 0) { p.clip_row_off[clip] = rs; p.clip_seg_off[clip] = ss; }
        if (clip == 0) {
            uint32_t rt = 0, st = 0;
            for (uint32_t i = lane; i < p.n_clips; i += 64) { rt += p.clip_rows[i]; st += p.seg_count[i]; }
            rt = wave_sum_u32(rt); st = wave_sum_u32(st);
            if (lane == 0) {
                p.totals[0] = rt; p.totals[1] = st; p.clip_row_off[p.n_clips] = rt; p.clip_seg_off[p.n_clips] = st;
                if (p.host) { p.host[0] = rt; p.host[1] = st; p.host[2] = p.flags[0]; p.host[3] = p.totals[3]; __threadfence_system(); }
            }
            if (p.clr_counters) {
                wsync();
                if (lane < 16) p.clr_counters[lane] = 0u;
                if (lane < 4) p.totals[lane] = 0u;
                if (p.clr_hist) for (int b = lane; b < SPAN_BUCKETS; b += 64) p.clr_hist[b] = 0u;
            }
        }
        wsync();
    }
    const uint32_t so = p.clip_seg_off[clip];
    const int32_t* sg = p.seg_i + (uint64_t)clip * p.seg_cap * 8;
    for (uint32_t i = lane; i < nseg; i += 64) {
        int32_t* o = p.seg_out + (uint64_t)(so + i) * 4;
        o[0] = (int32_t)clip; o[1] = sg[8 * i + SEG_START]; o[2] = sg[8 * i + SEG_LEN]; o[3] = sg[8 * i + SEG_FLAG];
    }
    uint32_t ro = p.clip_row_off[clip];
    int si = 0;
    int32_t* cy = p.carry ? p.carry + (uint64_t)clip * CARRY_WORDS : nullptr;
    const int seg_before = cy ? cy[0] : 0, res_before = cy ? cy[1] : 0;
    bool lost = false;
    for (uint32_t k = 0; k < nseg; k++) {
        const int flag = sg[8 * k + SEG_FLAG];
        if (flag < 0) continue;
        const int nr = sg[8 * k + SEG_NROWS];
        const uint32_t r0 = (uint32_t)sg[8 * k + SEG_ROW0];
        const int gsi = res_before + si;
        int32_t ts, tl;
        if (gsi >= seg_before) { ts = sg[8 * (gsi - seg_before) + SEG_START]; tl = sg[8 * (gsi - seg_before) + SEG_LEN]; }
        else {
            if (seg_before - gsi > CARRY_HIST) lost = true;
            ts = cy[2 + 2 * (gsi % CARRY_HIST)]; tl = cy[3 + 2 * (gsi % CARRY_HIST)];
        }
        for (int i = lane; i < nr; i += 64) {
            const int32_t* m = p.row_meta_in + (uint64_t)(r0 + i) * 8;
            int32_t* o = p.row_meta_out + (uint64_t)(ro + i) * 8;
            o[0] = m[0]; o[1] = gsi; o[4] = seg_before + m[4]; o[5] = m[5]; o[6] = m[6]; o[7] = m[7];
            if (p.level == 10 || p.level == 13) { o[2] = ts + m[2]; o[3] = m[3]; }
            else { o[2] = ts; o[3] = tl; }
        }
        for (int i = lane; i < nr * WSA_NFEAT; i += 64) p.row_feat_out[(uint64_t)ro * WSA_NFEAT + i] = p.row_feat_in[(uint64_t)r0 * WSA_NFEAT + i];
        ro += (uint32_t)nr;
        si++;
    }
    if (cy) {
        wsync();
        if (lane == 0) {
            for (uint32_t k = 0; k < nseg; k++) {
                const int g = seg_before + (int)k;
                cy[2 + 2 * (g % CARRY_HIST)] = sg[8 * k + SEG_START]; cy[3 + 2 * (g % CARRY_HIST)] = sg[8 * k + SEG_LEN];
            }
            cy[0] = seg_before + (int)nseg; cy[1] = res_before + si;
            if (lost) atomicOr(&p.totals[2], 1u);
        }
    }
}

void launch_compact(const CompactParams& p, hipStream_t s) {
    if (p.n_clips == 0) return;
    if (p.fused && !p.carry && p.clip_rows && p.n_clips <= 4096) { hipLaunchKernelGGL(compact_gather_kernel<true>, dim3(p.n_clips), dim3(64), 0, s, p); return; }
    if (p.n_clips <= 2 * CSCAN_T) hipLaunchKernelGGL(compact_scan_kernel<true>, dim3(1), dim3(CSCAN_T), 0, s, p);
    else {
        hipLaunchKernelGGL(compact_count_kernel, dim3((p.n_clips + 255) / 256), dim3(256), 0, s, p);
        hipLaunchKernelGGL(compact_scan_kernel<false>, dim3(1), dim3(CSCAN_T), 0, s, p);
    }
    hipLaunchKernelGGL(compact_gather_kernel<false>, dim3(p.n_clips), dim3(64), 0, s, p);
}
bool compact_is_fused(const CompactParams& p) { return p.fused && !p.carry && p.clip_rows && p.n_clips <= 4096 && p.n_clips > 0; }

}
```

webspeechanalyzer_amd/csrc/wsa_internal.hpp:

```cpp
#pragma once
#include <hip/hip_runtime.h>
#include <stdint.h>
#include <string>
#include <vector>
#include "../../include/wsa.h"

namespace wsa {

struct FePlanHost {
    int win = 0, hop = 0, nfft = 0, n2 = 0, R = 0, kmax = 0, bands = 0, spec_type = 1;
    int three = 0, M = 0;
    std::vector<float> window;
    std::vector<float> tw_n2;
    std::vector<float> tw_m;
    std::vector<float> tw_64;
    std::vector<float> tw_nfft;
    std::vector<int32_t> mel_k0, mel_cnt, mel_off;
    std::vector<float> mel_w;
    std::vector<float> emph;
    float gain = 0;
    std::vector<double> bins_hz;
};
bool build_fe_plan(const wsa_config& cfg, double fs, FePlanHost& out, std::string& err);

struct Tuning {
    int dbg = 0;
    bool no_pair = false, no_split = false, fe_fat = false, peaks_lanes = false;
    bool no_quad = false, quad = false;
    bool no_fuse = false;
    int full_table = -1;
    int tracker_wpc = 0, fin_wpc = 0;
    int fpw = 0;
    int fe_wg_per_cu = 0;
    bool fe_no_queue = false;
    int peaks_wpc = 0;
    int peaks_w = 0;
    int upload_threads = 0;
    int rs_s = 0, rs_j = 0, rs_c = 0;
    bool rs_one_launch = false;
    static Tuning from_env();
};

struct FeParams {
    const float* pcm = nullptr; uint64_t clip_stride = 0;
    const uint32_t* n_frames = nullptr;
    const uint32_t* frame_off = nullptr;
    uint32_t* spec = nullptr;
    int win = 0, hop = 0, kmax = 0, bands = 0, spec_type = 0, frames_per_wave = 0, mel_total = 0, mel_max_taps = 0;
    int mel_max_taps_lo = 0;
    const float* window = nullptr; const float2* tw_n2 = nullptr; const float2* tw_64 = nullptr; const float2* tw_nfft = nullptr;
    const float2* tw_m = nullptr;
    const int32_t* mel_k0 = nullptr; const int32_t* mel_cnt = nullptr; const int32_t* mel_off = nullptr; const float* mel_w = nullptr;
    const float* emph = nullptr; float gain = 0;
    const uint32_t* pcm_off = nullptr;
    int fat = 0, wg_per_cu = 0;
    uint32_t* queue = nullptr; uint32_t chunks_per_clip = 0, n_chunks = 0; int n_cu = 0;
};

constexpr int CAND_CAP = 64;
struct RecPtrs { uint4* hdr = nullptr; uint32_t* amp = nullptr; uint4* ent = nullptr; };
struct PkParams {
    const uint32_t* spec = nullptr; RecPtrs rec; uint32_t frame0 = 0, total_frames = 0; int bands = 0;
    const double* stream_state = nullptr; const uint32_t* n_frames = nullptr; uint32_t step_frames = 0, ring = 0;
    uint32_t* flags = nullptr;
    int dbg = 0;
    int lanes_only = 0, wpc = 0;
    int round_bins = 0;
};

struct GateParams {
    RecPtrs rec;
    const uint32_t* n_frames = nullptr; const uint32_t* frame_off = nullptr; uint32_t clip0 = 0, n_clips = 0;
    int level = 0, max_voiced_bin = 0; double breaker = 0, min_frames = 0; int auto_gate = 0; double ctx_max0 = 0, floor0 = 0;
    int32_t* fr_info = nullptr;
    double* fr_v = nullptr;
    double* fr_fl = nullptr;
    int32_t* seg_i = nullptr; double* seg_d = nullptr; int seg_cap = 0;
    uint32_t* seg_count = nullptr;
    uint32_t* clip_rows = nullptr;
    uint32_t* counters = nullptr;
    uint32_t* shared = nullptr;
    double* trace = nullptr; int dbg = 0;
    uint32_t* span_hist = nullptr; uint2* span_key = nullptr;
    int strided = 1;
    double* state = nullptr;
    const uint32_t* ctl = nullptr;
    uint32_t ring = 0, step_frames = 0;
    int32_t* fr_span = nullptr;
    int prio = 0;
};
enum { GATE_STATE = 16 };
enum { SEG_START = 0, SEG_LEN = 1, SEG_FBEGIN = 2, SEG_FEND = 3, SEG_CCI = 4, SEG_FLAG = 5, SEG_NROWS = 6, SEG_ROW0 = 7 };

struct TrParams {
    RecPtrs rec;
    const uint32_t* frame_off = nullptr;
    int level = 0;
    const int32_t* fr_info = nullptr; const double* fr_v = nullptr; const double* fr_fl = nullptr;
    int32_t* seg_i = nullptr; const double* seg_d = nullptr; int seg_cap = 0;
    const uint32_t* seg_count = nullptr; uint32_t n_clips = 0; const uint32_t* counters = nullptr; uint32_t* shared = nullptr;
    char* ws = nullptr; uint64_t ws_stride = 0; int tcap = 0, pcap = 0, fcap = 0;
    int32_t* row_meta = nullptr; double* row_feat = nullptr; uint32_t row_cap = 0; uint32_t* clip_rows = nullptr;
    double* trace = nullptr;
    int dbg = 0;
    uint32_t ring_mask = 0xffffffffu;
    float* formants = nullptr;
    int32_t* st_state = nullptr; char* st_act = nullptr;
    const int32_t* fr_span = nullptr; const uint32_t* n_frames_step = nullptr; const double* gate_state = nullptr;
    int4* trk_pts = nullptr; int32_t* trk_rank = nullptr; int32_t* trk_seg = nullptr;
    const uint2* order = nullptr;
    float* sums = nullptr;
    uint2* redo = nullptr; uint32_t* redo_count = nullptr;
    int order_cnt = 1;
    char* pool = nullptr; uint32_t pool_bpf = 0; double* span_hdr = nullptr;
    int fin_waves = 0;
    int quad = 0, quad_waves = 0;
};

struct CompactParams {
    uint32_t n_clips = 0; int seg_cap = 0, level = 0;
    const int32_t* seg_i = nullptr; const uint32_t* seg_count = nullptr;
    const int32_t* row_meta_in = nullptr; const double* row_feat_in = nullptr;
    int32_t* seg_out = nullptr; int32_t* row_meta_out = nullptr; double* row_feat_out = nullptr;
    uint32_t* clip_row_off = nullptr; uint32_t* clip_seg_off = nullptr; uint32_t* totals = nullptr;
    int32_t* carry = nullptr;
    const uint32_t* ctl = nullptr;
    const uint32_t* clip_rows = nullptr; const uint32_t* flags = nullptr; uint32_t* host = nullptr; int fused = 0;
    uint32_t* clr_counters = nullptr; uint32_t* clr_hist = nullptr;
};
bool compact_is_fused(const CompactParams& p);
enum { CARRY_HIST = 32, CARRY_WORDS = 2 + 2 * CARRY_HIST };

struct UttParams {
    uint32_t n_clips = 0;
    const int32_t* segments = nullptr; const int32_t* row_meta = nullptr;
    const uint32_t* clip_seg_off = nullptr; const uint32_t* clip_row_off = nullptr; const uint32_t* frame_off = nullptr;
    const float* formants = nullptr;
    uint32_t* clip_utt_off = nullptr;
    int32_t* utt_meta = nullptr; double* utt_feat = nullptr;
    uint32_t* totals = nullptr;
    uint32_t* state = nullptr; const int32_t* carry = nullptr; const uint32_t* ctl = nullptr; uint32_t ring_mask = 0xffffffffu;
};
enum { UTT_STATE_WORDS = 288 };

constexpr int RS_TAPS = 32, RS_OFFS = 32;
struct RsParams {
    const float* in; uint64_t stride_in; float* out; uint64_t stride_out;
    const uint32_t* n_in; const uint32_t* n_out;
    int chunks;
    const float* table; double ratio; int span, S, J;
};
void build_resample_table(double fs_in, double fs_out, std::vector<float>& K);
void resample_table_image(const std::vector<float>& K, std::vector<float>& img);
uint64_t resample_length(uint64_t n_in, double fs_in, double fs_out);
int resample_stride(double fs_in, double fs_out);
int resample_span(double ratio, int S, int J);
int resample_outputs_per_lane(int S, double ratio);
void launch_resample(const RsParams& p, uint32_t n_clips, uint64_t max_out, hipStream_t s);
struct RsClass { double ratio; uint32_t table_off; int span, S, J, copy, pad; };
struct RsWork { uint32_t clip, blk; };
struct RsMixedParams {
    const float* in; uint64_t stride_in; float* out; uint64_t stride_out;
    const uint32_t* n_in; const uint32_t* n_out;
    const float* tables; const RsClass* cls; const uint32_t* clip_class; const RsWork* work;
};
struct RsMixedPlan {
    std::vector<float> tables; std::vector<RsClass> cls; std::vector<uint32_t> clip_class; std::vector<RsWork> work;
    std::vector<uint32_t> first, block, lds;
    uint32_t max_block = 64, max_lds = 0, n_work = 0;
};
bool plan_resample_mixed(uint32_t n_clips, const uint32_t* n_out, const double* fs_in, double fs_out, RsMixedPlan& P, std::string& err);
void launch_resample_mixed(const RsMixedParams& p, const RsMixedPlan& P, bool per_class, hipStream_t s);

enum { RS_CTL_NFR = 0, RS_CTL_OFF = 1, RS_CTL_BITS = 2,
       RS_CTL_NIN = 3, RS_CTL_NOUT = 4,
       RS_CTL_DST = 5,
       RS_CTL_SHIFT = 6, RS_CTL_CARRY = 7,
       RS_CTL_Y_LO = 8, RS_CTL_Y_HI = 9,
       RS_CTL_IN0_LO = 10, RS_CTL_IN0_HI = 11,
       RS_CTL_WORDS = 12 };
constexpr int RS_HIST = 48;
struct RsStreamParams {
    float* stage; uint32_t stage_stride;
    float* conv; uint32_t conv_stride;
    const float* in; uint64_t in_stride;
    float* hist;
    const uint32_t* ctl; uint32_t n;
    const float* tables; const RsClass* cls; const uint32_t* stream_class;
    uint32_t xcap;
};
void launch_resample_stream(const RsStreamParams& p, hipStream_t s);
size_t resample_stream_lds(uint32_t xcap);
uint64_t resample_ready(uint64_t n_in, double fs_in, double fs_out);
uint32_t resample_step_frames_bound(uint32_t frames_per_step, uint32_t hop, double min_ratio);
uint32_t resample_step_outputs_bound(uint32_t frames_per_step, uint32_t hop, double min_ratio);

void launch_frontend(const FeParams& p, int n_clips, int max_frames, int R, int three, hipStream_t s);
bool fe_supported_R(int R, int three);
size_t fe_lds_required(const FePlanHost& P, bool fat);
void launch_peaks(const PkParams& p, hipStream_t s);
void launch_peaks_mode(const PkParams& p, int mode, hipStream_t s);
void launch_gate(const GateParams& p, hipStream_t s);
void launch_gate_stream(const GateParams& p, hipStream_t s);
void launch_stream_prepare(double* state, int32_t* carry, int32_t* tr_state, const uint32_t* ctl, uint32_t n, double ctx_max0, double floor0, hipStream_t s);
void launch_tracker(const TrParams& p, int n_waves, bool full_table, bool pair, hipStream_t s);
enum { SPAN_BUCKETS = 2048 };
void launch_span_order(const TrParams& p, uint32_t* span_hist, const uint2* span_key, uint2* order, uint32_t* counters, hipStream_t s);
void launch_tracker_stream(const TrParams& p, uint32_t n_streams, hipStream_t s);
enum { TR_STATE_WORDS = 16, TR_ACT_MAX = 320, TR_ACT_BYTES = TR_ACT_MAX * 44 };
void launch_compact(const CompactParams& p, hipStream_t s);
void launch_utterance(const UttParams& p, hipStream_t s);

struct CoefParams {
    const int32_t* row_meta = nullptr; double* row_feat = nullptr;
    const uint32_t* frame_off = nullptr; const uint32_t* totals = nullptr;
    const float* formants = nullptr; const float* sums = nullptr;
    double* ws = nullptr; uint32_t total_frames = 0;
    uint32_t* shared = nullptr;
    uint32_t ring_mask = 0xffffffffu, scratch_stride = 0;
};
void launch_coeffs(const CoefParams& p, uint32_t rows_cap, hipStream_t s);
size_t tracker_ws_bytes(int tcap, int pcap, int fcap, bool raw_tracks);
size_t tracker_pool_bpf();

}
```

Baseline: 778.1 million frames/s.

## Route spans to pair or quad tracker roles by width and length in one hybrid launch

The gate now marks each span as wide when any frame carries more than a threshold of peaks, and keeps a separate histogram for wide spans. The span-order kernel builds two lists: list A holds wide spans plus long narrow ones, and list B holds short narrow spans below a ratio cut. A new hybrid accumulate kernel processes list A with 32-lane pair workers and list B with 16-lane quad workers in the same launch. This targets load imbalance between the single pair and quad modes, at the cost of extra gate ballots, a larger histogram and more tracker waves.

```diff
diff --git a/webspeechanalyzer_amd/csrc/api.hip b/webspeechanalyzer_amd/csrc/api.hip
--- a/webspeechanalyzer_amd/csrc/api.hip
+++ b/webspeechanalyzer_amd/csrc/api.hip
@@ -66,6 +66,7 @@
     auto num = [](const char* name, int dflt) { const char* e = std::getenv(name); return e && *e ? std::atoi(e) : dflt; };
     t.dbg = num("WSA_DBG", 0);
     t.no_pair = std::getenv("WSA_NO_PAIR") != nullptr; t.no_split = std::getenv("WSA_NO_SPLIT") != nullptr; t.no_quad = std::getenv("WSA_NO_QUAD") != nullptr; t.quad = std::getenv("WSA_QUAD") != nullptr; t.no_fuse = std::getenv("WSA_NO_FUSE") != nullptr;
+    t.no_hybrid = std::getenv("WSA_NO_HYBRID") != nullptr; t.hybrid = std::getenv("WSA_HYBRID") != nullptr; t.hybrid_ratio = num("WSA_HYBRID_RATIO", 0);
     t.fe_fat = std::getenv("WSA_FE_FAT") != nullptr; t.peaks_lanes = std::getenv("WSA_PEAKS_LANES") != nullptr;
     t.full_table = num("WSA_FULL_TABLE", -1);
     t.tracker_wpc = num("WSA_TRACKER_WPC", 0); t.fin_wpc = num("WSA_FIN_WPC", 0); t.fpw = num("WSA_FPW", 0);
@@ -89,7 +90,7 @@
 __global__ void batch_clear_kernel(uint32_t* counters, uint32_t* totals, uint32_t* span_hist) {
     if (threadIdx.x < 16) counters[threadIdx.x] = 0;
     if (threadIdx.x < 4) totals[threadIdx.x] = 0;
-    if (span_hist) for (int b = threadIdx.x; b < SPAN_BUCKETS; b += blockDim.x) span_hist[b] = 0;
+    if (span_hist) for (int b = threadIdx.x; b < 2 * SPAN_BUCKETS; b += blockDim.x) span_hist[b] = 0;
 }
 }
 
@@ -218,7 +219,7 @@
     ok = ok && B.alloc(A, D, b->total_frames, false) && A.alloc(&B.d_counters, 16);
     if (D.level > 2)
         ok = ok && A.alloc(&B.d_ws, B.ws_stride * (size_t)b->n_waves * (b->pair && !b->split ? 2 : 1)) && A.alloc(&b->d_redo, spans) && A.alloc(&b->d_order, spans)
-                && A.alloc(&b->d_span_hist, (size_t)SPAN_BUCKETS) && A.alloc(&b->d_span_key, spans)
+                && A.alloc(&b->d_span_hist, (size_t)SPAN_HIST_WORDS) && A.alloc(&b->d_span_key, spans)
                 && (!D.raw_tracks || (A.alloc(&B.d_trk_pts, ((size_t)b->total_frames + 1) * 64 * 2) && A.alloc(&B.d_trk_rank, ((size_t)b->total_frames + 1) * 64)))
                 && (D.level != 12 || A.alloc(&B.d_coef_ws, (size_t)b->total_frames * 8));
     ok = ok && A.pin(&b->h_totals, &b->h_totals_dev, 8);
@@ -313,8 +314,11 @@
         t.fin_waves = b->tune.fin_wpc >= 1 && b->tune.fin_wpc <= 32 ? ctx->n_cu * b->tune.fin_wpc : 0;
         t.quad = b->split && !b->tune.no_quad && (b->tune.quad || b->total_frames >= 1200000u) ? 1 : 0;
         t.quad_waves = (int)std::min<size_t>((size_t)b->n_waves, ((size_t)b->n_clips * (size_t)B.seg_cap + 3) / 4 + 1);
+        const bool hybrid = b->split && !b->tune.no_hybrid && !b->tune.quad && !b->tune.no_quad && (b->tune.hybrid || b->total_frames >= 1200000u);
+        if (hybrid) t.quad = 2;
+        const int ratio = b->tune.hybrid_ratio >= 1 && b->tune.hybrid_ratio <= 1000 ? b->tune.hybrid_ratio : HYBRID_RATIO_DEFAULT;
         t.pool = b->split ? b->d_pool : nullptr; t.pool_bpf = (uint32_t)b->pool_bpf; t.span_hdr = b->split ? b->d_span_hdr : nullptr;
-        if (t.order) launch_span_order(t, b->d_span_hist, b->d_span_key, b->d_order, counters, cs);
+        if (t.order) launch_span_order(t, b->d_span_hist, b->d_span_key, b->d_order, counters, hybrid ? ratio : -1, cs);
         if (b->timing) HIP_TRY(ctx, hipEventRecord(b->ev[2], s));
         launch_tracker(t, b->n_waves, b->full_table, b->pair, cs);
     }
@@ -398,6 +402,11 @@
     return hipMemcpy(out16, b->be.d_counters, 16 * sizeof(uint32_t), hipMemcpyDeviceToHost) == hipSuccess ? WSA_OK : WSA_ERR_HIP;
 }
 
+int wsa_debug_batch_routing(wsa_batch* b, uint32_t* out3) {
+    if (!b || !out3 || !b->d_span_hist) return WSA_ERR_INVALID;
+    return hipMemcpy(out3, b->d_span_hist + 2 * SPAN_BUCKETS, 3 * sizeof(uint32_t), hipMemcpyDeviceToHost) == hipSuccess ? WSA_OK : WSA_ERR_HIP;
+}
+
 wsa_status wsa_batch_run(wsa_batch* b, const float* d_pcm, uint64_t clip_stride, void* stream) {
     if (!b) return WSA_ERR_INVALID;
     return run_impl(b, d_pcm, clip_stride, nullptr, true, true, reinterpret_cast<hipStream_t>(stream));
diff --git a/webspeechanalyzer_amd/csrc/gate.hip b/webspeechanalyzer_amd/csrc/gate.hip
--- a/webspeechanalyzer_amd/csrc/gate.hip
+++ b/webspeechanalyzer_amd/csrc/gate.hip
@@ -23,6 +23,7 @@
         double gw = 0, gT = 0, gk = 0;
         int nseg = 0, span_begin = 0, cuts = 0;
         bool overflow = false;
+        bool wide = false;
         double* st = ST ? p.state + (uint64_t)clip * GATE_STATE : nullptr;
         if (ST) {
             cur_frame = (int)st[0]; no_fm = (int)st[1]; c_ci = (int)st[2]; c_started = (int)st[3];
@@ -42,7 +43,7 @@
                 seg_d[2 * nseg] = ctx_max; seg_d[2 * nseg + 1] = floor_;
                 if (!ST && p.span_hist) {
                     const uint32_t bkt = (uint32_t)(SPAN_BUCKETS - 1) - min((uint32_t)(f_end - span_begin), (uint32_t)(SPAN_BUCKETS - 1));
-                    p.span_key[(uint64_t)clip * p.seg_cap + nseg] = make_uint2(bkt, atomicAdd(&p.span_hist[bkt], 1u));
+                    p.span_key[(uint64_t)clip * p.seg_cap + nseg] = make_uint2(bkt | (wide ? SPAN_WIDE_BIT : 0u), atomicAdd(&p.span_hist[bkt + (wide ? (uint32_t)SPAN_BUCKETS : 0u)], 1u));
                 }
             }
             nseg++;
@@ -122,7 +123,7 @@
             if (c_started < 0) {
                 const bool r_gt4 = p.auto_gate ? (d > h && h * (n - 1) > 4 * (d - h)) : ((d > h ? h * (n - 1) / (d - h) : 0) > 4);
                 if (n > 0 && pbin > 7 && pbin < p.max_voiced_bin && n > 4 && r_gt4) {
-                    c_ci = 0; c_started = 0; no_fm = 0; reset_before_acc = true; span_begin = (int)f;
+                    c_ci = 0; c_started = 0; no_fm = 0; reset_before_acc = true; span_begin = (int)f; wide = false;
                 } else no_fm++;
             }
             bool do_reset = false;
@@ -132,10 +133,11 @@
                     no_fm++;
                     if (c_started < 2) c_started--;
                     else if ((double)no_fm >= p.breaker) { finalize(c_ci + 1, (int)f + 1); do_reset = true; }
-                    else if (p.auto_gate) { gate_reset = false; noise_gate(h); if (gate_reset) span_begin = (int)f + 1; }
+                    else if (p.auto_gate) { gate_reset = false; noise_gate(h); if (gate_reset) { span_begin = (int)f + 1; wide = false; } }
                 } else {
-                    if (p.auto_gate) { gate_reset = false; noise_gate(h); if (gate_reset) { reset_before_acc = true; span_begin = (int)f; } }
+                    if (p.auto_gate) { gate_reset = false; noise_gate(h); if (gate_reset) { reset_before_acc = true; span_begin = (int)f; wide = false; } }
                     info = t_idx | (reset_before_acc ? (1 << 30) : 0);
+                    if (n > SPAN_NARROW_PEAKS) wide = true;
                     if (c_started < 2) c_started++; else no_fm = 0;
                 }
             }
@@ -148,7 +150,7 @@
                 }
             }
             c_ci++;
-            if (do_reset) { c_ci = 0; c_started = -1; no_fm = 0; span_begin = (int)f + 1; }
+            if (do_reset) { c_ci = 0; c_started = -1; no_fm = 0; span_begin = (int)f + 1; wide = false; }
             if (ST && c_started >= 0 && f + 1 - (uint32_t)span_begin + p.step_frames > p.ring) {
                 finalize(c_ci, (int)f + 1);
                 c_ci = 0; c_started = 1; no_fm = 0; span_begin = (int)f + 1; cuts++;
@@ -202,6 +204,7 @@
         uint64_t gT = 0; uint32_t gk = 0;
         int nseg = 0, span_begin = 0;
         bool overflow = false;
+        bool wide = false;
 
         auto finalize = [&](int e_arg, int f_end, int cur_frame) __attribute__((always_inline)) {
             const int len = e_arg - no_fm;
@@ -214,7 +217,7 @@
                 seg_d[2 * nseg] = (double)ctx_max; seg_d[2 * nseg + 1] = (double)floor_;
                 if (p.span_hist) {
                     const uint32_t bkt = (uint32_t)(SPAN_BUCKETS - 1) - min((uint32_t)(f_end - span_begin), (uint32_t)(SPAN_BUCKETS - 1));
-                    p.span_key[(uint64_t)clip * p.seg_cap + nseg] = make_uint2(bkt, atomicAdd(&p.span_hist[bkt], 1u));
+                    p.span_key[(uint64_t)clip * p.seg_cap + nseg] = make_uint2(bkt | (wide ? SPAN_WIDE_BIT : 0u), atomicAdd(&p.span_hist[bkt + (wide ? (uint32_t)SPAN_BUCKETS : 0u)], 1u));
                 }
             }
             nseg++;
@@ -250,7 +253,8 @@
             const int mxbin_l = (int)((hd.y >> 16) & 0xffu);
             const uint32_t flags_l = ((mxbin_l < 7 || mxbin_l >= maxvb) ? 1u : 0u)
                                    | (11ull * (uint64_t)hd.z < (((uint64_t)(hd.y & 0xffu) << 32) | hd.x) ? 2u : 0u)
-                                   | ((mxbin_l > 7 && mxbin_l < maxvb) ? 4u : 0u);
+                                   | ((mxbin_l > 7 && mxbin_l < maxvb) ? 4u : 0u)
+                                   | (((hd.y >> 8) & 0xffu) > (uint32_t)SPAN_NARROW_PEAKS ? 8u : 0u);
             int o_info = -1; uint32_t o_fl = 0;
             const uint32_t floor_in = floor_;
             const int nblk = (int)min(64u, nfr - blk);
@@ -293,6 +297,11 @@
                                 const uint64_t exm = __ballot(ex) & run_m;
                                 const int E = min(exm ? __ffsll((long long)exm) - 1 : 64, nblk);
                                 if (E > j) {
+                                    uint64_t wm = wide ? 0ull : __ballot(k >= 0 && lane < E && voiced && (flags_l & 8u));
+                                    while (wm) {
+                                        const int jw = __ffsll((long long)wm) - 1; wm &= wm - 1ull;
+                                        if (__popcll(__ballot(amp_row(jw) > (uint32_t)read_lane_i32((int)fk, jw))) > SPAN_NARROW_PEAKS) { wide = true; break; }
+                                    }
                                     if (k >= 0 && lane < E) { o_info = voiced ? c_ci + k : -1; o_fl = fk1; }
                                     floor_ = (uint32_t)read_lane_i32((int)fk1, E - 1);
                                     no_fm = read_lane_i32(voiced ? 0 : nofm_b + 1, E - 1);
@@ -306,6 +315,7 @@
                             bool unv_;
                             if (strong_ && !(fl_ & 1u)) {
                                 if ((fl_ & 2u) && count_accepted(j) > 3) break;
+                                if ((fl_ & 8u) && !wide && count_accepted(j) > SPAN_NARROW_PEAKS) wide = true;
                                 unv_ = false;
                             } else {
                                 if (no_fm + 1 >= br_i) break;
@@ -372,7 +382,7 @@
                     if (c_started < 0) {
                         bool start = false;
                         if (n > 4 && pbin > 7 && pbin < maxvb) { exact_d(); start = d > (uint64_t)h && (uint64_t)h * (uint64_t)(n - 1) > 4ull * (d - (uint64_t)h); }
-                        if (start) { c_ci = 0; c_started = 0; no_fm = 0; reset_before_acc = true; span_begin = (int)f; }
+                        if (start) { c_ci = 0; c_started = 0; no_fm = 0; reset_before_acc = true; span_begin = (int)f; wide = false; }
                         else no_fm++;
                     }
                     bool do_reset = false, gate_reset = false;
@@ -397,11 +407,12 @@
                             no_fm++;
                             if (c_started < 2) c_started--;
                             else if (no_fm >= br_i) { finalize(c_ci + 1, (int)f + 1, (int)f + 1); do_reset = true; }
-                            else { noise_gate(); if (gate_reset) span_begin = (int)f + 1; }
+                            else { noise_gate(); if (gate_reset) { span_begin = (int)f + 1; wide = false; } }
                         } else {
                             noise_gate();
-                            if (gate_reset) { reset_before_acc = true; span_begin = (int)f; }
+                            if (gate_reset) { reset_before_acc = true; span_begin = (int)f; wide = false; }
                             info = t_idx | (reset_before_acc ? (1 << 30) : 0);
+                            if (n > SPAN_NARROW_PEAKS) wide = true;
                             if (c_started < 2) c_started++; else no_fm = 0;
                         }
                     }
@@ -411,7 +422,7 @@
                         tr[7] = (double)h; tr[8] = (double)d; tr[9] = (double)g; tr[10] = 0; tr[11] = 0;
                     }
                     c_ci++;
-                    if (do_reset) { c_ci = 0; c_started = -1; no_fm = 0; span_begin = (int)f + 1; }
+                    if (do_reset) { c_ci = 0; c_started = -1; no_fm = 0; span_begin = (int)f + 1; wide = false; }
                 }
                 put(j, info);
             }
diff --git a/webspeechanalyzer_amd/csrc/tracker.hip b/webspeechanalyzer_amd/csrc/tracker.hip
--- a/webspeechanalyzer_amd/csrc/tracker.hip
+++ b/webspeechanalyzer_amd/csrc/tracker.hip
@@ -57,12 +57,21 @@
 size_t tracker_pool_bpf() { size_t b = 0; (void)carve_ws(nullptr, MAXC, MAXC, 1, 0, &b); return align16(b) + 256; }
 size_t tracker_ws_bytes(int tcap, int pcap, int fcap, bool raw_tracks) { size_t b = 0; (void)carve_ws(nullptr, tcap, pcap, fcap, raw_tracks ? pcap : 0, &b); return align16(b) + 256; }
 
-template <int AC, bool RAW, bool ST, bool PAIR = false, int SPLIT = 0, int GW = 32>
-__device__ __forceinline__ void tracker_body(const TrParams& p) {
+template <int AC, bool PAIR, int GW>
+constexpr int tracker_lds_bytes() {
     constexpr int SCRATCH = MAXC * (4 + 4 + 8 + 8) + 64 * 8 + MAXC * 8 + MAXC * 4;
     constexpr int LDS_ONE = AC * 52 + SCRATCH;
-    constexpr int LDS_ALL = (PAIR && GW == 16 && 4 * QUAD_GSZ > LDS_ONE) ? 4 * QUAD_GSZ : LDS_ONE;
-    __shared__ __attribute__((aligned(16))) unsigned char s_big[LDS_ALL];
+    return (PAIR && GW == 16 && 4 * QUAD_GSZ > LDS_ONE) ? 4 * QUAD_GSZ : LDS_ONE;
+}
+template <int N>
+__device__ __forceinline__ unsigned char* tracker_role_block() { __shared__ __attribute__((aligned(16))) unsigned char s_role[N]; return s_role; }
+template <int AC, bool RAW, bool ST, bool PAIR = false, int SPLIT = 0, int GW = 32, int ROLE = 0>
+__device__ __forceinline__ void tracker_body(const TrParams& p, const uint32_t role_wid = 0u, const uint32_t role_nw = 0u) {
+    static_assert(ROLE == 0 || (PAIR && SPLIT == 1), "roles share a launch only in the accumulate half of the split tracker");
+    constexpr int LDS_ALL = tracker_lds_bytes<AC, PAIR, GW>();
+    unsigned char* s_big;
+    if constexpr (ROLE == 0) { __shared__ __attribute__((aligned(16))) unsigned char s_own[LDS_ALL]; s_big = s_own; }
+    else s_big = tracker_role_block<LDS_ALL>();
     static_assert((AC * 52) % 16 == 0, "the scratch arrays start 16-byte aligned");
     double* const s_plo = reinterpret_cast<double*>(s_big + AC * 52);
     double* const s_phi = s_plo + MAXC;
@@ -114,10 +123,11 @@
         }
         else if (PAIR) {
             pair_total = p.counters[p.order_cnt];
-            const uint32_t npairs = (pair_total + (uint32_t)(64 / GW) - 1u) / (uint32_t)(64 / GW), W_ = gridDim.x, r = item;
+            const uint32_t npairs = (pair_total + (uint32_t)(64 / GW) - 1u) / (uint32_t)(64 / GW), W_ = ROLE ? role_nw : gridDim.x, r = item;
             if ((uint64_t)r * W_ >= npairs) break;
             item++;
-            pair_idx = (uint64_t)r * W_ + ((r & 1u) ? W_ - 1u - blockIdx.x : blockIdx.x);
+            const uint32_t w_ = ROLE ? role_wid : blockIdx.x;
+            pair_idx = (uint64_t)r * W_ + ((r & 1u) ? W_ - 1u - w_ : w_);
             if (pair_idx >= npairs) continue;
         }
         else if (p.order) {
@@ -1291,6 +1301,18 @@
     __builtin_amdgcn_s_setprio(3);
     tracker_body<AC_FAST, false, false, true, 1, 16>(p);
 }
+__global__ __launch_bounds__(64) __attribute__((amdgpu_waves_per_eu(4, 4))) void tracker_kernel_hybrid_acc(TrParams p, uint32_t pair_waves) {
+    static_assert(tracker_lds_bytes<AC_FAST, true, 32>() == tracker_lds_bytes<AC_FAST, true, 16>(), "one LDS block serves both roles");
+    __builtin_amdgcn_s_setprio(3);
+    const uint32_t P = pair_waves;
+    if (blockIdx.x < P) {
+        TrParams a = p; a.order_cnt = CNT_LIST_A;
+        tracker_body<AC_FAST, false, false, true, 1, 32, 1>(a, blockIdx.x, P);
+    } else {
+        TrParams b = p; b.order = p.order + p.counters[CNT_LIST_A]; b.order_cnt = CNT_LIST_B;
+        tracker_body<AC_FAST, false, false, true, 1, 16, 2>(b, blockIdx.x - P, gridDim.x - P);
+    }
+}
 __global__ __launch_bounds__(64) __attribute__((amdgpu_waves_per_eu(4, 4))) void tracker_kernel_finalize(TrParams p) {
     __builtin_amdgcn_s_setprio(3);
     tracker_body<AC_FAST, false, false, false, 2>(p);
@@ -1301,38 +1323,57 @@
 __global__ __launch_bounds__(64) void tracker_kernel_stream_raw(TrParams p) { tracker_body<AC_MAX, true, true>(p); }
 
 constexpr int ORDER_T = 256;
-__global__ __launch_bounds__(ORDER_T) void span_order_kernel(const uint32_t* hist, const uint2* key, const uint32_t* seg_count, uint32_t n_clips, int seg_cap, uint2* order, uint32_t* counters) {
-    __shared__ uint32_t offs[SPAN_BUCKETS], part[ORDER_T];
+__global__ __launch_bounds__(ORDER_T) void span_order_kernel(uint32_t* hist, const uint2* key, const uint32_t* seg_count, uint32_t n_clips, int seg_cap, uint2* order, uint32_t* counters, int ratio) {
+    __shared__ uint32_t off_n[SPAN_BUCKETS], off_w[SPAN_BUCKETS], part_a[ORDER_T], part_b[ORDER_T], part_w[ORDER_T], first_b;
     const int tid = threadIdx.x;
     constexpr int PER = SPAN_BUCKETS / ORDER_T;
-    uint32_t mine[PER], sum = 0;
+    uint32_t nar[PER], wid[PER];
+    int first = SPAN_BUCKETS;
 #pragma unroll
-    for (int q = 0; q < PER; q++) { mine[q] = hist[tid * PER + q]; sum += mine[q]; }
-    part[tid] = sum;
+    for (int q = PER - 1; q >= 0; q--) { nar[q] = hist[tid * PER + q]; wid[q] = hist[SPAN_BUCKETS + tid * PER + q]; if (nar[q] + wid[q]) first = tid * PER + q; }
+    if (tid == 0) first_b = SPAN_BUCKETS;
+    __syncthreads();
+    if (first < SPAN_BUCKETS) atomicMin(&first_b, (uint32_t)first);
+    __syncthreads();
+    const uint32_t f_max = first_b < SPAN_BUCKETS ? (uint32_t)(SPAN_BUCKETS - 1) - first_b : 0u;
+    const int b_cut = ratio < 0 ? SPAN_BUCKETS : SPAN_BUCKETS - 1 - (int)((uint64_t)f_max * (uint32_t)min(ratio, 1000) / 1000u);
+    uint32_t sum_a = 0, sum_b = 0, sum_w = 0;
+#pragma unroll
+    for (int q = 0; q < PER; q++) { const bool inb = tid * PER + q >= b_cut; sum_a += wid[q] + (inb ? 0u : nar[q]); sum_b += inb ? nar[q] : 0u; sum_w += wid[q]; }
+    part_a[tid] = sum_a; part_b[tid] = sum_b; part_w[tid] = sum_w;
     __syncthreads();
     for (int d = 1; d < ORDER_T; d <<= 1) {
-        const uint32_t add = tid >= d ? part[tid - d] : 0u;
+        const uint32_t aa = tid >= d ? part_a[tid - d] : 0u, ab = tid >= d ? part_b[tid - d] : 0u, aw = tid >= d ? part_w[tid - d] : 0u;
         __syncthreads();
-        part[tid] += add;
+        part_a[tid] += aa; part_b[tid] += ab; part_w[tid] += aw;
         __syncthreads();
     }
-    uint32_t run = part[tid] - sum;
+    const uint32_t n_a = part_a[ORDER_T - 1], n_b = part_b[ORDER_T - 1];
+    uint32_t run_a = part_a[tid] - sum_a, run_b = n_a + part_b[tid] - sum_b;
 #pragma unroll
-    for (int q = 0; q < PER; q++) { offs[tid * PER + q] = run; run += mine[q]; }
-    if (blockIdx.x == 0 && tid == ORDER_T - 1) counters[1] = part[tid];
+    for (int q = 0; q < PER; q++) {
+        const int bk = tid * PER + q;
+        off_w[bk] = run_a; run_a += wid[q];
+        if (bk >= b_cut) { off_n[bk] = run_b; run_b += nar[q]; } else { off_n[bk] = run_a; run_a += nar[q]; }
+    }
+    if (blockIdx.x == 0 && tid == ORDER_T - 1) {
+        counters[1] = n_a + n_b; counters[CNT_LIST_A] = n_a; counters[CNT_LIST_B] = n_b;
+        hist[2 * SPAN_BUCKETS] = n_a; hist[2 * SPAN_BUCKETS + 1] = n_b; hist[2 * SPAN_BUCKETS + 2] = part_w[tid];
+    }
     __syncthreads();
     const uint32_t clip = blockIdx.x * ORDER_T + tid;
     if (clip >= n_clips) return;
     const uint32_t ns = seg_count[clip];
     for (uint32_t k = 0; k < ns; k++) {
         const uint2 e = key[(uint64_t)clip * seg_cap + k];
-        order[offs[e.x] + e.y] = make_uint2(clip, k);
+        const uint32_t bk = e.x & ~SPAN_WIDE_BIT;
+        order[((e.x & SPAN_WIDE_BIT) ? off_w[bk] : off_n[bk]) + e.y] = make_uint2(clip, k);
     }
 }
 
-void launch_span_order(const TrParams& p, uint32_t* span_hist, const uint2* span_key, uint2* order, uint32_t* counters, hipStream_t s) {
+void launch_span_order(const TrParams& p, uint32_t* span_hist, const uint2* span_key, uint2* order, uint32_t* counters, int ratio, hipStream_t s) {
     if (p.n_clips == 0) return;
-    hipLaunchKernelGGL(span_order_kernel, dim3((p.n_clips + ORDER_T - 1) / ORDER_T), dim3(ORDER_T), 0, s, span_hist, span_key, p.seg_count, p.n_clips, p.seg_cap, order, counters);
+    hipLaunchKernelGGL(span_order_kernel, dim3((p.n_clips + ORDER_T - 1) / ORDER_T), dim3(ORDER_T), 0, s, span_hist, span_key, p.seg_count, p.n_clips, p.seg_cap, order, counters, ratio);
 }
 
 void launch_tracker_stream(const TrParams& p, uint32_t n_streams, hipStream_t s) {
@@ -1348,13 +1389,14 @@
     else if (full_table) hipLaunchKernelGGL(tracker_kernel_full, dim3(n_waves), dim3(64), 0, s, p);
     else if (pair && p.order && p.redo && (!p.trace || (p.dbg & 16))) {
         if (p.pool && p.span_hdr) {
-            if (p.quad) hipLaunchKernelGGL(tracker_kernel_quad_acc, dim3(p.quad_waves > 0 ? p.quad_waves : n_waves), dim3(64), 0, s, p);
+            if (p.quad == 2) hipLaunchKernelGGL(tracker_kernel_hybrid_acc, dim3(n_waves + (p.quad_waves > 0 ? p.quad_waves : n_waves)), dim3(64), 0, s, p, (uint32_t)n_waves);
+            else if (p.quad) hipLaunchKernelGGL(tracker_kernel_quad_acc, dim3(p.quad_waves > 0 ? p.quad_waves : n_waves), dim3(64), 0, s, p);
             else hipLaunchKernelGGL(tracker_kernel_pair_acc, dim3(n_waves), dim3(64), 0, s, p);
             hipLaunchKernelGGL(tracker_kernel_finalize, dim3(p.fin_waves > 0 ? p.fin_waves : 2 * n_waves), dim3(64), 0, s, p);
         }
         else hipLaunchKernelGGL(tracker_kernel_pair, dim3(n_waves), dim3(64), 0, s, p);
         TrParams r = p; r.order = p.redo; r.order_cnt = 2; r.pool = nullptr; r.span_hdr = nullptr;
-        const int redo_waves = p.quad ? 1024 : 128;
+        const int redo_waves = p.quad == 1 ? 1024 : 128;
         hipLaunchKernelGGL(tracker_kernel_fast, dim3(n_waves < redo_waves ? n_waves : redo_waves), dim3(64), 0, s, r);
     }
     else hipLaunchKernelGGL(tracker_kernel_fast, dim3(n_waves), dim3(64), 0, s, p);
@@ -1428,7 +1470,7 @@
                 wsync();
                 if (lane < 16) p.clr_counters[lane] = 0u;
                 if (lane < 4) p.totals[lane] = 0u;
-                if (p.clr_hist) for (int b = lane; b < SPAN_BUCKETS; b += 64) p.clr_hist[b] = 0u;
+                if (p.clr_hist) for (int b = lane; b < 2 * SPAN_BUCKETS; b += 64) p.clr_hist[b] = 0u;
             }
         }
         wsync();
diff --git a/webspeechanalyzer_amd/csrc/wsa_internal.hpp b/webspeechanalyzer_amd/csrc/wsa_internal.hpp
--- a/webspeechanalyzer_amd/csrc/wsa_internal.hpp
+++ b/webspeechanalyzer_amd/csrc/wsa_internal.hpp
@@ -27,6 +27,8 @@
     int dbg = 0;
     bool no_pair = false, no_split = false, fe_fat = false, peaks_lanes = false;
     bool no_quad = false, quad = false;
+    bool no_hybrid = false, hybrid = false;
+    int hybrid_ratio = 0;
     bool no_fuse = false;
     int full_table = -1;
     int tracker_wpc = 0, fin_wpc = 0;
@@ -205,7 +207,9 @@
 void launch_stream_prepare(double* state, int32_t* carry, int32_t* tr_state, const uint32_t* ctl, uint32_t n, double ctx_max0, double floor0, hipStream_t s);
 void launch_tracker(const TrParams& p, int n_waves, bool full_table, bool pair, hipStream_t s);
 enum { SPAN_BUCKETS = 2048 };
-void launch_span_order(const TrParams& p, uint32_t* span_hist, const uint2* span_key, uint2* order, uint32_t* counters, hipStream_t s);
+enum { SPAN_NARROW_PEAKS = 16, SPAN_STATS = 4, SPAN_HIST_WORDS = 2 * SPAN_BUCKETS + SPAN_STATS, CNT_LIST_A = 3, CNT_LIST_B = 5, HYBRID_RATIO_DEFAULT = 720 };
+constexpr uint32_t SPAN_WIDE_BIT = 0x80000000u;
+void launch_span_order(const TrParams& p, uint32_t* span_hist, const uint2* span_key, uint2* order, uint32_t* counters, int ratio, hipStream_t s);
 void launch_tracker_stream(const TrParams& p, uint32_t n_streams, hipStream_t s);
 enum { TR_STATE_WORDS = 16, TR_ACT_MAX = 320, TR_ACT_BYTES = TR_ACT_MAX * 44 };
 void launch_compact(const CompactParams& p, hipStream_t s);
```

New measurement: 769.3 million frames/s. -1.1%, worse.
